# JuliaLinearAlgebra/ArnoldiMethod.jl

Hardware: AMD Instinct MI355X
Metric: arnoldi_iters_per_sec (higher is better)
Workload: dtype f64

## Files before the change

arnoldimethod.jl_amd/_lib.py:

```python
from __future__ import annotations

import ctypes as C
import os

_HERE = os.path.dirname(os.path.abspath(__file__))
LIB_PATH = os.path.join(_HERE, "libkschur_hip.so")

KS_OK, KS_ERR_ARGUMENT, KS_ERR_DIMENSION, KS_ERR_HIP, KS_ERR_RCCL, KS_ERR_QR, KS_ERR_INTERNAL, KS_ERR_NO_DEVICE, KS_ERR_OPERATOR, KS_ERR_COMM = range(10)
KS_F64, KS_C64 = 0, 1
KS_I32, KS_I64 = 0, 1
KS_CSR, KS_CSC = 0, 1
LAYOUTS = {-1: "none", 0: "csr", 1: "csr-vi", 2: "csr-dvi", 3: "sell", 4: "sell-vi", 5: "stencil", 6: "csr-cb"}
PLAN_FACTS = ("ptr64", "ni", "nblk", "nlong", "row_gather", "nslices", "sell_entries", "ncolblocks", "cb_rpt", "cb_ni", "nstencil",
              "nstencil_local", "stencil_mask_bytes", "ndvi", "dvi_unroll")
WHICH = {"LM": 0, "LR": 1, "SR": 2, "LI": 3, "SI": 4}


class ArgumentError(ValueError):
    """Julia's ArgumentError (src/run.jl:111-116,123-124,165-174,185; src/ArnoldiMethod.jl:62-63,87-90)."""


class DimensionMismatch(ValueError):
    """Julia's DimensionMismatch (checksquare, src/run.jl:110)."""


class QRDidNotConverge(RuntimeError):
    """"QR algorithm did not converge" (src/schurfact.jl:406)."""


class HipError(RuntimeError):
    pass


class CommTimeout(HipError):
    """A peer rank did not take part in an exchange within KS_P2P_TIMEOUT_S (peer-to-peer transport)."""


class ks_params(C.Structure):
    _fields_ = [
        ("nev", C.c_int32), ("which", C.c_int32), ("tol", C.c_double), ("mindim", C.c_int32), ("maxdim", C.c_int32),
        ("restarts", C.c_int32), ("start_from", C.c_int32), ("initialize", C.c_int32), ("reserved", C.c_int32),
    ]


class ks_history(C.Structure):
    _fields_ = [
        ("mvproducts", C.c_int32), ("nconverged", C.c_int32), ("converged", C.c_int32), ("nev", C.c_int32),
        ("restarts", C.c_int32), ("reorth", C.c_int32), ("breakdowns", C.c_int32), ("explicit_steps", C.c_int32),
        ("seconds_expand", C.c_double), ("seconds_host", C.c_double), ("seconds_rotate", C.c_double),
    ]


class ks_expand_stats(C.Structure):
    _fields_ = [("steps", C.c_int32), ("reorth", C.c_int32), ("breakdowns", C.c_int32), ("explicit_steps", C.c_int32)]


HOST_APPLY_FN = C.CFUNCTYPE(C.c_int, C.c_void_p, C.c_void_p, C.c_void_p)
DEVICE_APPLY_FN = C.CFUNCTYPE(C.c_int, C.c_void_p, C.c_void_p, C.c_void_p, C.c_void_p)
HOST_ALLREDUCE_FN = C.CFUNCTYPE(C.c_int, C.c_void_p, C.POINTER(C.c_double), C.c_int)
HOST_EXCHANGE_FN = C.CFUNCTYPE(C.c_int, C.c_void_p, C.c_int, C.POINTER(C.c_int32), C.POINTER(C.c_void_p), C.POINTER(C.c_int64),
                               C.POINTER(C.c_void_p), C.POINTER(C.c_int64))

vp, i32, i64, u64, dbl = C.c_void_p, C.c_int, C.c_int64, C.c_uint64, C.c_double
P = C.POINTER
PROTOTYPES = {
    "ks_version": [P(C.c_int), P(C.c_int)],
    "ks_ctx_create": [i32, P(vp)],
    "ks_comm_unique_id": [vp],
    "ks_ctx_create_dist": [i32, i32, i32, vp, P(vp)],
    "ks_ctx_create_hostcomm": [i32, i32, i32, HOST_ALLREDUCE_FN, HOST_EXCHANGE_FN, vp, P(vp)],
    "ks_ctx_create_p2p": [i32, i32, i32, P(vp)],
    "ks_ctx_p2p_handle": [vp, vp],
    "ks_ctx_p2p_attach": [vp, vp],
    "ks_ctx_destroy": [vp],
    "ks_ctx_synchronize": [vp],
    "ks_ctx_rank": [vp, P(C.c_int), P(C.c_int)],
    "ks_ctx_stream": [vp, P(vp)],
    "ks_operator_csr": [vp, i64, i64, i64, vp, vp, vp, i32, i32, i32, i32, P(vp)],
    "ks_operator_csr_dist": [vp, i64, i64, i64, vp, vp, vp, i32, i32, vp, vp, vp, vp, P(vp)],
    "ks_operator_dense": [vp, i64, vp, i64, i32, i32, P(vp)],
    "ks_operator_host_callback": [vp, i64, i32, HOST_APPLY_FN, vp, P(vp)],
    "ks_operator_device_callback": [vp, i64, i32, DEVICE_APPLY_FN, vp, P(vp)],
    "ks_operator_lu": [vp, i64, i32, vp, vp, vp, vp, vp, vp, vp, vp, vp, P(vp)],
    "ks_operator_lu_info": [vp, P(i64), P(i64), P(i64), P(i64)],
    "ks_operator_lu_layout": [vp, i32, P(i64), P(i64), P(i64), P(C.c_int)],
    "ks_operator_destroy": [vp],
    "ks_operator_size": [vp, P(i64), P(i64), P(C.c_int)],
    "ks_operator_format": [vp, P(C.c_double), P(C.c_int), P(C.c_int)],
    "ks_operator_apply_raw": [vp, vp, vp],
    "ks_workspace_create": [vp, i64, i64, i64, i32, i32, P(vp)],
    "ks_workspace_placement": [vp, P(C.c_int), P(C.c_double), P(C.c_double), P(C.c_int)],
    "ks_workspace_passes": [vp, P(C.c_int)],
    "ks_workspace_set_passes": [vp, i32, dbl],
    "ks_workspace_set_sstep": [vp, i32, dbl, dbl],
    "ks_debug_blk_time": [vp, i32, i32, i32, i32, i32, P(C.c_double), P(C.c_int)],
    "ks_workspace_sstep_info": [vp, P(C.c_int), P(C.c_int), P(C.c_int), P(C.c_double)],
    "ks_workspace_relation_info": [vp, P(C.c_int), P(C.c_double)],
    "ks_workspace_relation_probes": [vp, P(C.c_int)],
    "ks_workspace_fused_rotations": [vp, P(C.c_int), P(C.c_int), P(C.c_int)],
    "ks_workspace_split_rotations": [vp, P(C.c_int)],
    "ks_workspace_deflated_blocks": [vp, P(C.c_int), P(C.c_int)],
    "ks_sstep_partition": [C.c_int, C.c_int, C.c_int, C.c_int, P(C.c_int), C.c_int, P(C.c_int)],
    "ks_workspace_assert_arnoldi": [vp, i32],
    "ks_workspace_provenance": [vp, P(C.c_int)],
    "ks_workspace_check_guard": [vp, P(C.c_int)],
    "ks_workspace_destroy": [vp],
    "ks_workspace_dims": [vp, P(i64), P(C.c_int), P(C.c_int), P(i64)],
    "ks_workspace_H": [vp, P(vp), P(C.c_int)],
    "ks_workspace_Q": [vp, P(vp), P(C.c_int)],
    "ks_workspace_col_ptr": [vp, i32, P(vp)],
    "ks_workspace_set_seed": [vp, u64],
    "ks_col_upload": [vp, i32, vp],
    "ks_col_download": [vp, i32, vp],
    "ks_cols_download": [vp, i32, i32, vp, i64],
    "ks_cols_upload": [vp, i32, i32, vp, i64],
    "ks_col_fill_uniform": [vp, i32, u64],
    "ks_col_norm": [vp, i32, P(dbl)],
    "ks_col_div": [vp, i32, dbl],
    "ks_col_copy": [vp, i32, i32],
    "ks_apply": [vp, vp, i32, i32],
    "ks_gemv_t": [vp, i32, i32, vp],
    "ks_gemv_n_sub": [vp, i32, i32, vp],
    "ks_rotate": [vp, i32, i32, i32, vp, i32],
    "ks_basis_times": [vp, i32, i32, vp, i32, i32, vp, i64],
    "ks_orthogonalize": [vp, i32, P(C.c_int)],
    "ks_reinitialize": [vp, i32, vp, P(C.c_int)],
    "ks_iterate_arnoldi": [vp, vp, i32, i32, P(ks_expand_stats)],
    "ks_params_default": [i64, P(ks_params)],
    "ks_partialschur": [vp, vp, P(ks_params), vp, vp, P(ks_history)],
    "ks_restart": [vp, P(ks_params), i32, P(C.c_int), P(C.c_int), P(C.c_int), vp, vp, vp],
    "ks_expand_restart": [vp, vp, P(ks_params), i32, i32, P(C.c_int), P(C.c_int), P(C.c_int), vp, vp, vp, P(ks_expand_stats), vp],
    "ks_profile_enable": [vp, i32],
    "ks_profile_reset": [vp],
    "ks_profile_get": [vp, i32, vp, vp, vp],
    "ks_residual_norms": [vp, vp, i32, P(dbl), P(dbl)],
    "ks_arnoldi_relation": [vp, vp, i32, P(dbl), P(dbl)],
    "ks_host_schurfact": [i32, vp, i32, i32, i32, i32, i32, vp, i32, i32],
    "ks_host_restart_step": [i32, vp, i32, vp, i32, i32, i32, i32, i32, dbl, i32, P(C.c_int), P(C.c_int), P(C.c_int), vp, vp, vp],
    "ks_host_sortschur": [i32, vp, i32, i32, i32, vp, i32, i32, i32, i32],
    "ks_host_givens": [i32, vp, vp, P(dbl), vp, vp],
    "ks_host_csr_plan": [i64, i64, i64, vp, vp, vp, i32, i32, i32, i32, i32, i64, i64, P(C.c_int), P(C.c_int), P(dbl), P(dbl), vp, vp, vp, vp, i64, vp, i32],
    "ks_last_words": [C.c_char_p, i32],
}

_lib = None


def load():
    global _lib
    if _lib is not None:
        return _lib
    if not os.path.exists(LIB_PATH):
        raise ImportError(
            f"{LIB_PATH} is missing: the MI355X HIP library has not been built (run `python __graft_entry__.py build`). "
            "There is no CPU fallback for the product path."
        )
    L = C.CDLL(LIB_PATH)
    L.ks_last_error_string.restype = C.c_char_p
    L.ks_last_error_string.argtypes = []
    for name, args in PROTOTYPES.items():
        fn = getattr(L, name)
        fn.argtypes = args
        fn.restype = C.c_int
    _lib = L
    return L


def check(rc: int):
    if rc == KS_OK:
        return
    msg = load().ks_last_error_string().decode(errors="replace")
    if rc == KS_ERR_ARGUMENT:
        raise ArgumentError(msg)
    if rc == KS_ERR_DIMENSION:
        raise DimensionMismatch(msg)
    if rc == KS_ERR_QR:
        raise QRDidNotConverge(msg)
    if rc == KS_ERR_COMM:
        raise CommTimeout(msg)
    raise HipError(f"libkschur_hip error {rc}: {msg}")
```

arnoldimethod.jl_amd/api.py:

```python
from __future__ import annotations

import ctypes as C
import math
from dataclasses import dataclass

import numpy as np

from . import _lib
from ._lib import ArgumentError, DimensionMismatch, check

EPS = float(np.finfo(np.float64).eps)
DEFAULT_SEED = 20240917


class Target:
    name = "LM"

    def __repr__(self):
        return f"{self.name}()"


class LM(Target):
    name = "LM"

# ... 455 lines not shown
        out = np.empty((self.n, Yf.shape[1]), dtype=ydt, order="F")
        check(_lib.load().ks_basis_times(self._h, c, Yf.shape[1], Yf.ctypes.data, Yf.shape[0], _dtype_code(ydt), out.ctypes.data, self.n))
        return out

    def orthogonalize(self, j: int) -> bool:
        ok = C.c_int()
        check(_lib.load().ks_orthogonalize(self._h, j, C.byref(ok)))
        return bool(ok.value)

    def reinitialize(self, j: int = 0, v1=None) -> bool:
        ok = C.c_int()
        p = None
        if v1 is not None:
            v1 = np.ascontiguousarray(np.asarray(v1, dtype=self.dtype))
            p = v1.ctypes.data
        check(_lib.load().ks_reinitialize(self._h, j, p, C.byref(ok)))
        return bool(ok.value)

    def iterate_arnoldi(self, A: Operator, frm: int, to: int):
        st = _lib.ks_expand_stats()
        _check_op(_lib.load().ks_iterate_arnoldi(A._h, self._h, frm, to, C.byref(st)), A)
        return dict(steps=st.steps, reorth=st.reorth, breakdowns=st.breakdowns, explicit_steps=st.explicit_steps)

    def restart(self, active: int, nev: int, which="LM", tol=None, mindim=None, maxdim=None):
        maxdim = self.maxdim if maxdim is None else maxdim
        mindim = min(max(10, nev), self.n_global) if mindim is None else mindim
        tol = math.sqrt(EPS) if tol is None else tol
        p = _lib.ks_params(nev, _which_code(which), float(tol), mindim, maxdim, 1, 1, 0, 0)
        k, nlock, purge = C.c_int(), C.c_int(), C.c_int()
        lams, rs, groups = np.zeros(2 * maxdim), np.zeros(maxdim), np.zeros(maxdim, dtype=np.int32)
        check(_lib.load().ks_restart(self._h, C.byref(p), active, C.byref(k), C.byref(nlock), C.byref(purge),
                                     lams.ctypes.data, rs.ctypes.data, groups.ctypes.data))
        return dict(k=k.value, nlock=nlock.value, purge=purge.value, eigenvalues=lams[0::2] + 1j * lams[1::2],
                    residuals=rs, groups=groups)

    def expand_restart(self, A: Operator, k: int, active: int, nev: int, which="LM", tol=None, mindim=None, maxdim=None):
        maxdim = self.maxdim if maxdim is None else maxdim
        mindim = min(max(10, nev), self.n_global) if mindim is None else mindim
        tol = math.sqrt(EPS) if tol is None else tol
        p = _lib.ks_params(nev, _which_code(which), float(tol), mindim, maxdim, 1, 1, 0, 0)
        ko, nlock, purge = C.c_int(), C.c_int(), C.c_int()
        lams, rs, groups = np.zeros(2 * maxdim), np.zeros(maxdim), np.zeros(maxdim, dtype=np.int32)
        st = _lib.ks_expand_stats()
        sec = np.zeros(3)
        _check_op(_lib.load().ks_expand_restart(A._h, self._h, C.byref(p), active, k, C.byref(ko), C.byref(nlock), C.byref(purge),
                                                lams.ctypes.data, rs.ctypes.data, groups.ctypes.data, C.byref(st), sec.ctypes.data), A)
        return dict(k=ko.value, nlock=nlock.value, purge=purge.value, eigenvalues=lams[0::2] + 1j * lams[1::2], residuals=rs,
                    groups=groups, steps=st.steps, reorth=st.reorth, breakdowns=st.breakdowns, explicit_steps=st.explicit_steps,
                    seconds=tuple(sec))

    def residual_norms(self, A: Operator, ncols: int):
        r, o = C.c_double(), C.c_double()
        _check_op(_lib.load().ks_residual_norms(A._h, self._h, ncols, C.byref(r), C.byref(o)), A)
        return r.value, o.value

    def arnoldi_relation(self, A: Operator, k: int):
        r, o = C.c_double(), C.c_double()
        _check_op(_lib.load().ks_arnoldi_relation(A._h, self._h, k, C.byref(r), C.byref(o)), A)
        return r.value, o.value

    @property
    def passes(self) -> int:
        k = C.c_int()
        check(_lib.load().ks_workspace_passes(self._h, C.byref(k)))
        return k.value

    def set_passes(self, passes: int, max_ratio: float = float("nan")):
        check(_lib.load().ks_workspace_set_passes(self._h, int(passes), float(max_ratio)))

    def set_sstep(self, s: int, pivot_min: float = float("nan"), gram_dev_max: float = float("nan")):
        check(_lib.load().ks_workspace_set_sstep(self._h, int(s), float(pivot_min), float(gram_dev_max)))

    @property
    def sstep_info(self) -> dict:
        s, b, a = C.c_int(), C.c_int(), C.c_int()
        d = (C.c_double * 3)()
        check(_lib.load().ks_workspace_sstep_info(self._h, C.byref(s), C.byref(b), C.byref(a), d))
        fr, sa, sd = C.c_int(), C.c_int(), C.c_int()
        check(_lib.load().ks_workspace_fused_rotations(self._h, C.byref(fr), C.byref(sa), C.byref(sd)))
        sr = C.c_int()
        check(_lib.load().ks_workspace_split_rotations(self._h, C.byref(sr)))
        db, dc = C.c_int(), C.c_int()
        check(_lib.load().ks_workspace_deflated_blocks(self._h, C.byref(db), C.byref(dc)))
        return dict(s=s.value, blocks=b.value, abandoned=a.value, pivot_stage1=d[0], pivot_stage2=d[1], gram_dev=d[2], fused_rotations=fr.value,
                    split_rotations=sr.value, chains_adopted=sa.value, chains_dropped=sd.value, deflated_blocks=db.value, deflated_columns=dc.value)

    @property
    def relation_info(self) -> dict:
        b, w = C.c_int(), C.c_double()
        check(_lib.load().ks_workspace_relation_info(self._h, C.byref(b), C.byref(w)))
        pr = C.c_int()
        check(_lib.load().ks_workspace_relation_probes(self._h, C.byref(pr)))
        return dict(breaks=b.value, worst_leak=w.value, probes=pr.value)

    def assert_arnoldi(self, k: int):
        check(_lib.load().ks_workspace_assert_arnoldi(self._h, int(k)))

    @property
    def provenance(self) -> int:
        k = C.c_int()
        check(_lib.load().ks_workspace_provenance(self._h, C.byref(k)))
        return k.value

    @property
    def placement(self) -> dict:
        k, b, w, r = C.c_int(), C.c_double(), C.c_double(), C.c_int()
        check(_lib.load().ks_workspace_placement(self._h, C.byref(k), C.byref(b), C.byref(w), C.byref(r)))
        return dict(candidates=k.value, kept_ms=b.value, slowest_ms=w.value, refused=r.value)

    def guard_intact(self) -> bool:
        ok = C.c_int()
        check(_lib.load().ks_workspace_check_guard(self._h, C.byref(ok)))
        return bool(ok.value)

    def close(self):
        if getattr(self, "_h", None) and getattr(self.ctx, "_h", None):
            _lib.load().ks_workspace_destroy(self._h)
        self._h = None

    def __del__(self):
        try:
            self.close()
        except Exception:
            pass


def sstep_partition(dtype, k0: int, count: int, smax: int) -> list:
    if k0 < 1 or count < 1 or smax < 1:
        return []
    cap = 64
    out = (C.c_int * cap)()
    nb = C.c_int(0)
    check(_lib.load().ks_sstep_partition(_dtype_code(dtype), int(k0), int(count), int(smax), out, cap, C.byref(nb)))
    return [int(out[i]) for i in range(min(nb.value, cap))]


class PartialSchur:

    def __init__(self, ws: ArnoldiWorkspace, nconv: int, eigenvalues: np.ndarray):
        self.workspace = ws
        self.nconverged = nconv
        self.R = ws.H[:nconv, :nconv]
        self.eigenvalues = eigenvalues
        self._Q = None

    @property
    def Q(self) -> np.ndarray:
        if self._Q is None:
            self._Q = self.workspace.cols(0, self.nconverged)
        return self._Q

    def __repr__(self):
        return (
            f"PartialSchur decomposition ({'ComplexF64' if self.workspace.dtype.kind == 'c' else 'Float64'}) "
            f"of dimension {self.nconverged}\neigenvalues:\n{self.eigenvalues!r}"
        )


@dataclass
class History:

    mvproducts: int
    nconverged: int
    converged: bool
    nev: int
    restarts: int = 0
    reorth: int = 0
    breakdowns: int = 0
# ... 101 lines not shown
```

arnoldimethod.jl_amd/csrc/ks_backend.hpp:

```cpp
#pragma once
template <class T> struct HipBackend : ks::Backend<T> {
  using D = typename DevT<T>::type;
  ks_operator* op;
  ks_workspace* ws;
  HipBackend(ks_operator* o, ks_workspace* w) : op(o), ws(w) {}

  int64_t n_global() const override { return ws->n_global; }

  void iterate_arnoldi(int from, int to, const ks::Mat<T>& H, ks::ExpandStats& stats) override {
    guarded_expand([&] { iterate_arnoldi_impl(from, to, H, stats, nullptr); });
  }

  bool iterate_arnoldi_early(int from, int to, const ks::Mat<T>& H, ks::ExpandStats& stats, const std::function<void()>& early) override {
    const char* e = std::getenv("KS_EARLY_RESTART");
    const bool on = !(e && e[0] == '0');
    bool done = false;
    guarded_expand([&] { done = iterate_arnoldi_impl(from, to, H, stats, on ? &early : nullptr); });
    return done;
  }

  template <class F> void guarded_expand(F&& f) {
    try {
      f();
    } catch (...) {
      gate_cancel(ws);
      (void)hipStreamSynchronize(ws->ctx->stream);
      try { reset_lazy(ws); } catch (...) {}
      prov_drop(ws);
      ws->rot_pending = ws->rot_fuse = ws->rot_split = false;
      ws->rot_true_start = ws->chain_true = ws->ztrue_valid = false;
      ws->spec_valid = false;
      ws->spec_adopt = 0;
      ws->rp_inflight = false;
      throw;
    }
  }

  bool iterate_arnoldi_impl(int from, int to, const ks::Mat<T>& H, ks::ExpandStats& stats, const std::function<void()>* early) {
    ws->ctx->use();
    bool early_stands = false;
    int j0 = from;
    int explicit_step = -1;
    const bool trusted = prov_ok(ws, from);
    bool no_block = false;
    drift_probe_collect();
    if (trusted && ws->prov_vouched && !ws->t_lazy && ws->sstep_eff >= 2 && op->async_capable && from >= 2 && to - from + 1 >= 2) relation_probe(from, H);
    blk_shifts_from_saved_H();
    while (j0 <= to) {
      const double tb0 = ks::now_s();
      int jend = to;
      if (!op->async_capable) jend = j0;
      if (explicit_step >= 0) jend = j0;
      const bool lazy = use_deferred(ws, jend);
      const bool tpath = lazy && ws->passes == 2 && trusted && explicit_step < 0;
      std::vector<int> blk_sizes;
      ksd::BlkShifts<D> blk_sh{};
      std::vector<std::complex<double>> defl_ex;
      int ndefl = 0;
      if (tpath && !no_block && ws->sstep >= 2 && ws->sstep_eff >= 1 && op->async_capable && jend - j0 + 1 >= 2) {
        ndefl = defl_plan(H, j0, defl_ex, std::min(std::min(ws->sstep, ksd::kBlkSMax), jend - j0 + 1));
        if (ndefl > ws->defl_last && ws->sstep_eff < ws->sstep) { ws->sstep_eff = ws->sstep; ws->blk_clean = 0; }
        ws->defl_last = ndefl;
      }
      if (tpath && !no_block && ws->sstep_eff >= 2 && op->async_capable && jend - j0 + 1 >= 2 &&
          blk_make_shifts<D>(ws, std::min(ws->sstep_eff, ksd::kBlkSMax), blk_sh, ndefl > 0 ? &defl_ex : nullptr))
        blk_sizes = blk_partition(ws->dtype, j0, jend - j0 + 1, std::min(ws->sstep_eff, ksd::kBlkSMax));
      const bool bpath = !blk_sizes.empty();
      if (bpath) {
        int covered = 0;
        for (int sz : blk_sizes) covered += sz;
        jend = std::min(jend, j0 + covered - 1);
      }
      if (ws->rot_pending) {
        const bool fused_ok = bpath && ks_blk_rot_ok(ws->dtype == KS_F64 ? 0 : 1, ws->rot_cin, j0, blk_sizes[0]);
        const bool split_ok = bpath && ws->spec_on && ks_blk_zsrc_ok(ws->dtype == KS_F64 ? 0 : 1, j0, blk_sizes[0]);
        static const int defer_dbg = env_int("KS_DEFER_DEBUG", 0);
        if (defer_dbg)
          std::fprintf(stderr, "[adopt] bpath %d j0 %d out0+rr %d fused_ok %d split_ok %d spec_valid %d blk0 %d spec_ne %d backoff %d\n", (int)bpath, j0, ws->rot_out0 + ws->rot_rr,
                       (int)fused_ok, (int)split_ok, (int)ws->spec_valid, bpath ? blk_sizes[0] : 0, ws->spec_ne, ws->spec_backoff);
        const bool need_true = ws->rot_true_start;
        const bool spec_fits = ws->spec_valid && bpath && blk_sizes[0] >= ws->spec_ne && ws->spec_sh.size() == sizeof(blk_sh) && (!need_true || ws->spec_true);
        if (bpath && ndefl == 0 && j0 == ws->rot_out0 + ws->rot_rr && (fused_ok || split_ok) && ensure_zscratch<D>(ws) &&
            (!need_true || spec_fits || true_start_enqueue<D>(ws))) {
          ws->rot_pending = false;
          ws->rot_true_start = false;
          ws->rot_fuse = true;
          ws->rot_split = !fused_ok;
          ws->chain_true = spec_fits ? ws->spec_true : need_true;
          ws->t_lazy = false;
          ws->t_hi = -1;
          if (spec_fits) {
            std::memcpy(&blk_sh, ws->spec_sh.data(), sizeof(blk_sh));
            ws->spec_adopt = ws->spec_ne;
            ws->spec_used++;
            ws->spec_backoff_len = 1;
            ws->spec_valid = false;
          }
          spec_drop(ws);
        } else {
          rot_flush(ws);
        }
      }
      spec_drop(ws);
      ws->ztrue_valid = false;
      if (tpath && (bpath || ws->blk_tail || !(ws->t_lazy && j0 == ws->t_hi + 1))) {
        materialize(ws);
        ws->ntrue = j0;
      }
      double sigma0 = 1.0;
      if (tpath && ws->t_lazy && j0 - 1 >= ws->ntrue && j0 - 1 <= ws->t_hi) {
        const double binv = reinterpret_cast<const double*>(static_cast<const char*>(ws->Th) + ((size_t)(j0 - 1) + (size_t)(j0 - 1) * ws->ldt) * ws->esz)[0];
        if (binv > 0.0 && std::isfinite(binv)) sigma0 = std::ldexp(1.0, std::ilogb(binv));
      }
      reset_state(ws, tpath, sigma0);
      const bool mb = lazy && ws->use_mbox;
      const bool do_early = early && mb && !tpath && jend == to;
      const uint64_t seq = ++ws->mbox_seq;
      if (bpath) {
        blk_ensure_buffers(ws);
        enqueue_steps_blk<D>(ws, op, j0, blk_sizes, blk_sh, ndefl);
      } else if (tpath) {
        enqueue_steps_t<D>(ws, op, j0, jend);
      } else if (lazy) {
        if (ws->t_lazy) materialize(ws);
        enqueue_steps_deferred<D>(ws, op, j0, jend, do_early ? seq : 0);
      } else {
        materialize(ws);
        for (int j = j0; j <= jend; ++j) {
          op->in_scale = 1.0;
          op->apply(ws->col(j - 1), ws->col(j), ws->st);
          enqueue_orthogonalize<D>(ws, j);
        }
      }
      bool early_ran = false;
      struct EarlyGuard {
        ks_workspace* w; void* Hp; bool armed;
        ~EarlyGuard() { if (armed && !w->Hbackup.empty()) std::memcpy(Hp, w->Hbackup.data(), w->Hbackup.size()); }
      } early_guard{ws, H.p, false};
      static const int dbg = env_int("KS_EARLY_DEBUG", 0);
      double tq0 = dbg ? ks::now_s() : 0.0, tq1 = 0, tq2 = 0;
      if (mb) publish_control(ws, j0, ws->Hstage_dev, 1, seq, tpath);
      else fetch_state_enqueue(ws, j0, tpath);
      if (bpath && jend == to && to == ws->maxdim && j0 >= 2 && !ws->rp_inflight && ++ws->rp_count >= ws->rp_every) {
        ws->rp_count = 0;
        drift_probe_enqueue(j0, H);
      }
      if (bpath && ndefl == 0 && jend == to && to == ws->maxdim &&
          (ks_blk_rot_ok(ws->dtype == KS_F64 ? 0 : 1, ws->maxdim + 1, j0, blk_sizes[0]) || ks_blk_zsrc_ok(ws->dtype == KS_F64 ? 0 : 1, j0, blk_sizes[0]))) {
        static const int defer_dbg2 = env_int("KS_DEFER_DEBUG", 0);
        if (defer_dbg2) std::fprintf(stderr, "[spec] enqueue? backoff %d j0 %d blk0 %d\n", ws->spec_backoff, j0, blk_sizes[0]);
        const bool start_stored = ws->blk_count == 0 || ws->blk_diag[2] <= 1e-12;
        if (ws->spec_backoff > 0) --ws->spec_backoff;
        else spec_enqueue(blk_sh, j0, !start_stored);
      }
      const bool will_defer = ws->rot_defer_on && bpath && ws->sstep_eff >= 8 && to == ws->maxdim;
      if (early && tpath && mb && jend == to && !will_defer) gate_arm(ws);
      if (do_early) {
        mbox_wait(ws, 0, seq);
        if (dbg) tq1 = ks::now_s();
        const DevState* se = reinterpret_cast<const DevState*>(static_cast<const char*>(ws->Hstage_early) + ws->hd_bytes);
        if (se->breakdown < 0) {
          const size_t hb = (size_t)H.ld * H.n * sizeof(T);
          ws->Hbackup.resize(hb);
          std::memcpy(ws->Hbackup.data(), H.p, hb);
          early_guard.armed = true;
          fetch_H_columns<T>(ws, j0, jend, H, false, ws->Hstage_early);
          (*early)();
          early_ran = true;
        }
        if (dbg) tq2 = ks::now_s();
      }
      if (mb) {
        mbox_wait(ws, 1, seq);
        if (ws->ctx->profiling) {
          KS_HIP(hipStreamSynchronize(ws->ctx->stream));
          prof_collect(ws->ctx);
        }
        ws->ctx->check_comm();
      } else {
        fetch_state_wait(ws);
      }
      if (dbg && do_early) {
        const double tq3 = ks::now_s();
        std::fprintf(stderr, "[early] enqueue %.1f us | wait H %.1f us | early host part %.1f us | final wait %.1f us | batch %.1f us\n", 1e6 * (tq0 - tb0), 1e6 * (tq1 - tq0), 1e6 * (tq2 - tq1), 1e6 * (tq3 - tq2), 1e6 * (tq3 - tb0));
      } else if (dbg) {
        const double tq3 = ks::now_s();
        std::fprintf(stderr, "[early off] enqueue %.1f us | wait %.1f us | batch %.1f us\n", 1e6 * (tq0 - tb0), 1e6 * (tq3 - tq0), 1e6 * (tq3 - tb0));
      }
      if (ws->gate_armed && (ws->st_h->breakdown >= 0 || ws->st_h->bail >= 0 || ws->st_h->blk_bail >= 0))
        gate_cancel(ws);
      const int blk_bail = bpath ? ws->st_h->blk_bail : -1;
      const int bail = (tpath && !bpath) ? ws->st_h->bail : -1;
      const int bd = (bail >= 0 || blk_bail >= 0) ? -1 : ws->st_h->breakdown;
      const int last_done = blk_bail >= 0 ? blk_bail - 1 : (bail >= 0 ? bail - 1 : (bd >= 0 ? bd : jend));
      if (bpath) {
        ws->blk_diag[0] = ws->st_h->blk_piv1;
        ws->blk_diag[1] = ws->st_h->blk_piv2;
        ws->blk_diag[2] = ws->st_h->blk_gdev;
        int done = 0, done_blocks = 0;
        for (int sz : blk_sizes) { if (j0 + done + sz - 1 <= last_done) { done += sz; ws->blk_count++; ++done_blocks; } }
        if (blk_bail >= 0) {
          ws->blk_bails++; stats.blk_bails++; no_block = true;
          ws->sstep_eff = ws->sstep_eff >= 4 ? ws->sstep_eff / 2 : (ws->sstep_eff > 2 ? 2 : 1);
          ws->blk_clean = 0;
        } else if (++ws->blk_clean >= 16 && ws->sstep_eff < ws->sstep) {
          int nxt = ws->sstep_eff + 1;
          for (int cand : {2, 3, 4, 5, 8, 10, 20}) if (cand > ws->sstep_eff) { nxt = cand; break; }
          ws->sstep_eff = std::min(ws->sstep, std::max(2, nxt));
          ws->blk_clean = 0;
        }
        stats.blocks += done_blocks;
      } else if (tpath && ws->sstep_eff == 1 && ws->sstep >= 2 && blk_bail < 0 && bail < 0 && bd < 0) {
        if (++ws->blk_clean >= 16) { ws->sstep_eff = 2; ws->blk_clean = 0; }
      }
      if (early_ran && bd >= 0) {
        std::memcpy(H.p, ws->Hbackup.data(), ws->Hbackup.size());
        early_ran = false;
      }
      early_guard.armed = false;
      if (early_ran) {
        const T* hs = static_cast<const T*>(ws->Hstage);
        H(jend, jend - 1) = hs[(size_t)(jend - 1) * (ws->maxdim + 1) + jend];
        lazy_factors_from_stage<T>(ws, j0, jend, ws->Hstage);
        early_stands = true;
      } else {
        fetch_H_columns<T>(ws, j0, last_done, H, lazy && !tpath);
      }
      if (tpath) {
        const int good = blk_bail >= 0 ? blk_bail - 1 : (bail >= 0 ? bail - 1 : (bd >= 0 ? bd - 1 : jend));
        if (good >= ws->ntrue) {
          ws->t_lazy = true;
          ws->t_hi = good;
          ws->blk_tail = bpath;
        }
      }
      stats.steps += last_done - j0 + 1;
      stats.reorth += ws->st_h->n_reorth;
      if (explicit_step >= 0) explicit_step = -1;
      if (bail >= 0) {
        explicit_step = bail;
        stats.explicit_steps++;
      }
      if (lazy && jend > j0) ws->oop_full = 10 * ws->st_h->n_reorth >= 9 * (last_done - j0 + 1);
      if (bd >= 0) {
        if ((int64_t)bd != ws->n_global) {
          reinit_column<D>(ws, bd, nullptr);
          stats.breakdowns++;
        }
      }
      j0 = last_done + 1;
    }
    if (trusted) prov_set(ws, to);
    else prov_drop(ws);
    if (ws->sstep_eff >= 2 && to == ws->maxdim && !early_stands) {
      ws->Hfull.assign(static_cast<const char*>(ws->H), static_cast<const char*>(ws->H) + h_bytes(ws));
      ws->hfull_valid = true;
      ws->ritz_valid = false;
    }
    return early_stands;
  }

  int defl_plan(const ks::Mat<T>& H, int j0, std::vector<std::complex<double>>& ex, int steps) {
    ex.clear();
    static const int dbg = env_int("KS_DEFLATE_DEBUG", 0);
    if (dbg) std::fprintf(stderr, "[deflate] j0 %d on %d dist %d ritz_valid %d nritz %d sstep_eff %d steps %d\n", j0, (int)ws->defl_on, (int)ws->ctx->distributed(), (int)ws->ritz_valid, (int)ws->ritz.size(), ws->sstep_eff, steps);
    if (!ws->defl_on || !ws->ritz_valid || ws->ritz.empty()) return 0;
    static const double ratio = [] { const char* e = std::getenv("KS_DEFLATE_RATIO"); const double v = e ? std::atof(e) : 1.5; return v > 1.0 ? v : 1.5; }();
    int nl = 0;
    for (int j = 1; j <= j0 - 2; ++j)
      if (H(j, j - 1) == T(0)) nl = j;
    if (nl == 0) return 0;
    using C = std::complex<double>;
    std::vector<C> lam(nl);
    std::vector<int> width(nl, 1);
    for (int j = 0; j < nl;) {
      if (j + 1 < nl && H(j + 1, j) != T(0)) {
        const C a = C(H(j, j)), b = C(H(j, j + 1)), c = C(H(j + 1, j)), d = C(H(j + 1, j + 1));
        const C tr2 = 0.5 * (a + d), disc = std::sqrt(tr2 * tr2 - (a * d - b * c));
        lam[j] = tr2 + disc; lam[j + 1] = tr2 - disc;
        width[j] = 2; width[j + 1] = 0;
        j += 2;
      } else {
        lam[j] = C(H(j, j));
        ++j;
      }
    }
    double rest = 0.0;
    for (auto z : ws->ritz) {
      if (!std::isfinite(std::abs(z))) continue;
      bool locked = false;
      for (int j = 0; j < nl; ++j) locked = locked || std::abs(z - lam[j]) <= 1e-6 * std::max(1.0, std::abs(lam[j]));
      if (!locked) rest = std::max(rest, std::abs(z));
    }
    if (dbg) std::fprintf(stderr, "[deflate] locked columns %d, largest other Ritz value %.3g, |lambda_0| %.3g\n", nl, rest, std::abs(lam[0]));
    if (!(rest > 0.0)) return 0;
    int nd = 0;
    for (int j = 0; j < nl;) {
      const int w = width[j] == 2 ? 2 : 1;
      const double mag = w == 2 ? std::max(std::abs(lam[j]), std::abs(lam[j + 1])) : std::abs(lam[j]);
      const double growth = std::pow(mag / rest, std::max(1, steps - 1));
      if (!(mag > ratio * rest) || !(growth > 1e3) || nd + w > ksd::kDeflMax) break;
      for (int q = 0; q < w; ++q) ex.push_back(lam[j + q]);
      nd += w;
      j += w;
    }
    return nd;
  }

  void spec_enqueue(const ksd::BlkShifts<D>& sh, int k_now, bool from_true) {
    if (!ws->spec_on || !ws->rot_defer_on || !ws->gate_allowed || ws->sstep_eff < 8 || !op->async_capable || ws->ctx->hc.allreduce != nullptr) return;
    if (from_true && (!ws->true_start_on || ws->maxdim + 1 > 40)) return;
    const int ne = std::min(10, ws->maxdim - k_now - (sizeof(D) == 8 ? 1 : 0));
    if (ne < 2) return;
    if (!ensure_zscratch<D>(ws)) return;
    if (from_true && !true_start_enqueue<D>(ws)) return;
    char* zs = static_cast<char*>(ws->zscratch);
    op->shift_store_cacheable = true;
    for (int i = 0; i < ne; ++i) {
      op->in_scale = 1.0;
      const void* src = i == 0 ? (from_true ? static_cast<const void*>(ws->ztrue) : ws->col(ws->maxdim)) : static_cast<const void*>(zs + (size_t)(i - 1) * ws->ld * sizeof(D));
      double tre, tim;
      if constexpr (sizeof(D) == 8) { tre = sh.theta[i]; tim = 0.0; }
      else { tre = sh.theta[i].x; tim = sh.theta[i].y; }
      op->apply_shifted(src, zs + (size_t)i * ws->ld * sizeof(D), tre, tim, sh.sigma[i], ws->ld, ws->st);
    }
    ws->spec_sh.assign(reinterpret_cast<const char*>(&sh), reinterpret_cast<const char*>(&sh) + sizeof(sh));
    ws->spec_ne = ne;
    ws->spec_true = from_true;
    ws->spec_valid = true;
  }

  void relation_probe(int from, const ks::Mat<T>& H) {
    const int c = from - 2, nc = from;
    hipStream_t s_ = ws->ctx->stream;
    D* scratch = static_cast<D*>(ws->col(from));
    op->in_scale = 1.0;
    op->apply(ws->col(c), ws->col(from), nullptr);
    if (!ws->probe_dev) {
      KS_HIP(hipMalloc(&ws->probe_dev, 16 + (size_t)(ws->maxdim + 2) * 16));
      KS_HIP(hipHostMalloc(&ws->probe_host, 16 + (size_t)(ws->maxdim + 2) * 16, hipHostMallocCoherent | hipHostMallocMapped));
    }
    double* out = static_cast<double*>(ws->probe_dev);
    D* coef_d = reinterpret_cast<D*>(static_cast<char*>(ws->probe_dev) + 16);
    D* coef_h = reinterpret_cast<D*>(static_cast<char*>(ws->probe_host) + 16);
    double fro2 = 0.0;
    for (int j = 0; j < from - 1; ++j)
      for (int i = 0; i < from; ++i) fro2 += std::norm(std::complex<double>(H(i, j)));
    for (int i = 0; i < nc; ++i) std::memcpy(&coef_h[i], &H(i, c), sizeof(D));
    KS_HIP(hipMemcpyAsync(coef_d, coef_h, (size_t)nc * sizeof(D), hipMemcpyHostToDevice, s_));
    KS_HIP(hipMemsetAsync(out, 0, 2 * sizeof(double), s_));
    const int64_t nchunks = (ws->n + 15) / 16;
    const int64_t stride = std::max<int64_t>(1, std::min<int64_t>(64, nchunks / 16384));
    const int64_t sampled = (nchunks + stride - 1) / stride * 16;
    const int grid = (int)((sampled + kBlock - 1) / kBlock);
    ksd::k_relation_probe<D><<<grid, kBlock, 0, s_>>>(static_cast<const D*>(ws->V), ws->ld, nc, scratch, coef_d, ws->n, stride, out);
    KS_HIP(hipGetLastError());
    if (ws->ctx->distributed()) ws->ctx->allreduce(out, 2);
    double* res = static_cast<double*>(ws->probe_host);
    KS_HIP(hipMemcpyAsync(res, out, 2 * sizeof(double), hipMemcpyDeviceToHost, s_));
    KS_HIP(hipStreamSynchronize(s_));
    ws->ctx->check_comm();
    ws->relation_probes++;
    const double fro = std::sqrt(fro2);
    const double leak = res[1] > 0.0 ? std::sqrt(res[0] * ((double)ws->n_global / res[1])) : 0.0;
    if (!(leak <= 10.0 * ws->relation_tol * fro)) {
      ws->relation_breaks++;
      ws->relation_leak = std::max(ws->relation_leak, fro > 0.0 ? leak / fro : leak);
      ws->sstep_eff = 0;
    }
  }

  void drift_probe_enqueue(int from, const ks::Mat<T>& H) {
    const int c = from - 2, nc = from;
    hipStream_t s_ = ws->ctx->stream;
    if (!ws->probe_dev) {
      KS_HIP(hipMalloc(&ws->probe_dev, 16 + (size_t)(ws->maxdim + 2) * 16));
      KS_HIP(hipHostMalloc(&ws->probe_host, 16 + (size_t)(ws->maxdim + 2) * 16, hipHostMallocCoherent | hipHostMallocMapped));
    }
    if (!ws->probe_col) {
      if (hipMalloc(&ws->probe_col, (size_t)ws->ld * sizeof(D)) != hipSuccess) {
        (void)hipGetLastError();
        ws->probe_col = nullptr;
        return;
      }
      KS_HIP(hipMemsetAsync(ws->probe_col, 0, (size_t)ws->ld * sizeof(D), s_));
    }
    D* scratch = static_cast<D*>(ws->probe_col);
    op->in_scale = 1.0;
    op->apply(ws->col(c), scratch, ws->st);
    if (!ws->ctx->distributed()) {
      if (!ws->watch_acc) {
        KS_HIP(hipMalloc(&ws->watch_acc, 32));
        KS_HIP(hipMemsetAsync(ws->watch_acc, 0, 32, s_));
        KS_HIP(hipHostGetDevicePointer(&ws->probe_host_dev, ws->probe_host, 0));
      }
      ksd::ProbeCoef<D> pc;
      double fro2w = 0.0;
      for (int j = 0; j < from - 1; ++j)
        for (int i = 0; i < from; ++i) fro2w += std::norm(std::complex<double>(H(i, j)));
// ... 328 lines not shown
```

arnoldimethod.jl_amd/csrc/ks_block.hpp:

```cpp
#pragma once



inline bool blk_shape_ok(int dtype, int k, int s) { return ks_blk_shape_ok(dtype == KS_F64 ? 0 : 1, k, s); }
inline std::vector<int> blk_partition(int dtype, int k0, int count, int smax) {
  std::vector<int> out;
  int k = k0;
  while (count > 0) {
    int s = std::min(count, smax);
    while (s > 1 && !blk_shape_ok(dtype, k, s)) --s;
    if (!blk_shape_ok(dtype, k, s)) break;
    out.push_back(s);
    k += s;
    count -= s;
  }
  return out;
}

inline std::vector<std::complex<double>> leja_shifts(const std::vector<std::complex<double>>& ritz, int s, bool real) {
  std::vector<std::complex<double>> pts;
  for (auto z : ritz) {
    if (real) z = std::complex<double>(z.real(), 0.0);
    if (!std::isfinite(z.real()) || !std::isfinite(z.imag())) continue;
    bool dup = false;
    for (auto& q : pts) dup = dup || std::abs(q - z) <= 1e-14 * std::max(1.0, std::abs(z));
    if (!dup) pts.push_back(z);
  }
  std::vector<std::complex<double>> out;
  if (pts.empty()) { out.assign(s, 0.0); return out; }
  std::vector<double> logprod(pts.size(), 0.0);
  std::vector<bool> used(pts.size(), false);
  size_t cur = 0;
  for (size_t i = 1; i < pts.size(); ++i) if (std::abs(pts[i]) > std::abs(pts[cur])) cur = i;
  while (out.size() < pts.size() && (int)out.size() < s) {
    used[cur] = true;
    out.push_back(pts[cur]);
    size_t best = pts.size();
    for (size_t i = 0; i < pts.size(); ++i) {
      if (used[i]) continue;
      logprod[i] += std::log(std::max(std::abs(pts[i] - pts[cur]), 1e-300));
      if (best == pts.size() || logprod[i] > logprod[best]) best = i;
    }
    if (best == pts.size()) break;
    cur = best;
  }
  const size_t have = out.size();
  while ((int)out.size() < s) out.push_back(out[out.size() % have]);
  return out;
}

inline void blk_ensure_buffers(ks_workspace* ws) {
  if (ws->bpart) return;
  const size_t entries = (size_t)ksd::kBlkKMax * ksd::kBlkSMax + ksd::kBlkGram;
  KS_HIP(hipMalloc(&ws->bpart, entries * (size_t)ws->pnb * ws->esz));
  KS_HIP(hipMalloc(&ws->bred, entries * ws->esz));
  const size_t sb = ws->dtype == KS_F64 ? sizeof(ksd::BlkScratch<double>) : sizeof(ksd::BlkScratch<cd>);
  KS_HIP(hipMalloc(&ws->bscr, sb));
  KS_HIP(hipMemset(ws->bscr, 0, sb));
  KS_HIP(hipMalloc(&ws->bzero, 256));
  KS_HIP(hipMemset(ws->bzero, 0, 256));
}

inline int& blk_dbg() { static int v = env_int("KS_BLK_DBG", 0); return v; }
template <class D> int launch_blk(ks_workspace* ws, int which, int k, int s, bool zscratch = false) {
  auto* bs = static_cast<ksd::BlkScratch<D>*>(ws->bscr);
  BlkLaunchArgs a{};
  a.V = ws->V; a.ld = ws->ld; a.dtype = sizeof(D) == 8 ? 0 : 1; a.k = k; a.s = s;
  if (zscratch) { a.zsrc = ws->zscratch; a.ldz = ws->ld; }
  if (which == 2) { a.cin = ws->rot_cin; a.out0 = ws->rot_out0; a.rotm = ws->Qd; }
  a.partial = ws->bpart; a.pnb = ws->pnb; a.coefp = bs->coefp; a.r1inv = bs->r1inv; a.zeros = ws->bzero; a.st = ws->st;
  a.dbg = blk_dbg(); a.nt = ws->v_nt ? 1 : 0; a.num_cu = ws->ctx->num_cu; a.bpc = ws->ctx->bpc; a.stream = ws->ctx->stream;
  try {
    return ks_blk_launch(which, a);
  } catch (const std::runtime_error& e) {
    throw KsError{KS_ERR_INTERNAL, e.what()};
  }
}

template <class D> bool ensure_zscratch(ks_workspace* ws) {
  if (ws->zscratch) return true;
  const size_t zbytes = (size_t)ws->ld * ksd::blk_smax<D>() * sizeof(D);
  if (hipMalloc(&ws->zscratch, zbytes) != hipSuccess) {
    (void)hipGetLastError();
    ws->zscratch = nullptr;
    ws->spec_on = false;
    ws->rot_defer_on = false;
    return false;
  }
  KS_HIP(hipMemsetAsync(ws->zscratch, 0, zbytes, ws->ctx->stream));
  if (env_int("KS_ADDR_DEBUG", 0)) std::fprintf(stderr, "[addr] V %p zscratch %p ld %lld bytes/col %lld\n", ws->V, ws->zscratch, (long long)ws->ld, (long long)(ws->ld * sizeof(D)));
  return true;
}

template <class D> bool true_start_enqueue(ks_workspace* ws) {
  if (ws->ztrue_valid) return true;
  const int cin = ws->maxdim + 1;
  if (cin > 40) return false;
  if (!ws->ztrue) {
    if (hipMalloc(&ws->ztrue, (size_t)ws->ld * sizeof(D)) != hipSuccess) { (void)hipGetLastError(); ws->ztrue = nullptr; return false; }
    KS_HIP(hipMemsetAsync(ws->ztrue, 0, (size_t)ws->ld * sizeof(D), ws->ctx->stream));
  }
  ks_ctx* cx = ws->ctx;
  ProfScope ps(cx, KSP_ROTATE, (double)ws->n * sizeof(D) * (cin + 1));
  const D* Vc = static_cast<const D*>(ws->col(0));
  const D* tcol = static_cast<const D*>(ws->Td) + (size_t)ws->maxdim * ws->ldt;
  D* out = static_cast<D*>(ws->ztrue);
  const size_t smem = (size_t)cin * sizeof(D);
  const int nb = cap_blocks(ws, cx->num_cu * 4, kBlock);
  if (cin <= 8) ksd::k_rotate_valu<D, 8><<<nb, kBlock, smem, cx->stream>>>(Vc, ws->ld, cin, 1, tcol, ws->ldt, out, ws->ld, -1);
  else if (cin <= 16) ksd::k_rotate_valu<D, 16><<<nb, kBlock, smem, cx->stream>>>(Vc, ws->ld, cin, 1, tcol, ws->ldt, out, ws->ld, -1);
  else if (cin <= 24) ksd::k_rotate_valu<D, 24><<<nb, kBlock, smem, cx->stream>>>(Vc, ws->ld, cin, 1, tcol, ws->ldt, out, ws->ld, -1);
  else ksd::k_rotate_valu<D, 40><<<nb, kBlock, smem, cx->stream>>>(Vc, ws->ld, cin, 1, tcol, ws->ldt, out, ws->ld, -1);
  KS_HIP(hipGetLastError());
  ws->ztrue_valid = true;
  ws->true_starts++;
  return true;
}

template <class D>
void enqueue_steps_blk(ks_workspace* ws, ks_operator* op, int from, const std::vector<int>& sizes, const ksd::BlkShifts<D>& sh, int ndefl = 0) {
  ks_ctx* cx = ws->ctx;
  hipStream_t s_ = cx->stream;
  const int ldh = ws->maxdim + 1;
  const double nb8 = (double)ws->n * sizeof(D);
  D* Hd = static_cast<D*>(ws->Hd);
  D* Tm = static_cast<D*>(ws->Td);
  auto* bs = static_cast<ksd::BlkScratch<D>*>(ws->bscr);
  int k = from;
  int first = 1;
  for (int s : sizes) {
    const bool fuse = first && ws->rot_fuse;
    const bool split = fuse && ws->rot_split;
    const bool chain_true = fuse && ws->chain_true;
    ws->rot_fuse = false;
    ws->rot_split = false;
    ws->chain_true = false;
    char* zs = nullptr;
    if (fuse) {
      KS_REQUIRE(ws->zscratch != nullptr, KS_ERR_INTERNAL, "fused rotation without scratch columns (the adoption allocates them)");
      zs = static_cast<char*>(ws->zscratch);
    }
    if (split) {
      rotate_device<D>(ws, 0, ws->rot_cin, ws->rot_rr, ws->rot_out0, -1);
      ws->rot_split_count++;
    }
    auto zcol = [&](int i) -> void* { return fuse ? static_cast<void*>(zs + (size_t)i * ws->ld * sizeof(D)) : ws->col(k + i); };
    op->shift_store_cacheable = s >= 10;
    const int adopted = fuse ? ws->spec_adopt : 0;
    ws->spec_adopt = 0;
    for (int i = adopted; i < s; ++i) {
      double tre, tim;
      if constexpr (sizeof(D) == 8) { tre = sh.theta[i]; tim = 0.0; }
      else { tre = sh.theta[i].x; tim = sh.theta[i].y; }
      op->in_scale = 1.0;
      const void* src = i == 0 ? (fuse ? (chain_true ? static_cast<const void*>(ws->ztrue) : ws->col(ws->maxdim)) : ws->col(k - 1)) : zcol(i - 1);
      op->apply_shifted(src, zcol(i), tre, tim, sh.sigma[i], ws->ld, ws->st);
      if (ndefl > 0) {
        ProfScope ps(cx, KSP_AXPY, nb8 * 2.0 * (ndefl + 1) + nb8);
        if (!ws->defl_part) KS_HIP(hipMalloc(&ws->defl_part, (size_t)ksd::kDeflMax * (1024 + 1) * sizeof(D)));
        const int nbd = (int)std::max<int64_t>(1, std::min<int64_t>(std::min(1024, cx->num_cu * 4), (ws->n + kBlock - 1) / kBlock));
        D* zc = static_cast<D*>(zcol(i));
        const D* U = static_cast<const D*>(ws->col(0));
        D* part = static_cast<D*>(ws->defl_part);
        ksd::k_defl_dots<D><<<nbd, kBlock, 0, s_>>>(U, ws->ld, ndefl, zc, ws->n, part);
        if (!cx->distributed()) {
          ksd::k_defl_apply<D><<<nbd, kBlock, 0, s_>>>(U, ws->ld, ndefl, zc, ws->n, part, nbd, bs->cdefl + (size_t)i * ksd::kDeflMax);
        } else {
          D* red = part + (size_t)ksd::kDeflMax * 1024;
          ksd::k_defl_reduce<D><<<1, kBlock, 0, s_>>>(part, nbd, ndefl, red);
          cx->allreduce(reinterpret_cast<double*>(red), ndefl * (int)(sizeof(D) / 8));
          ksd::k_defl_apply<D><<<nbd, kBlock, 0, s_>>>(U, ws->ld, ndefl, zc, ws->n, red, 1, bs->cdefl + (size_t)i * ksd::kDeflMax);
        }
      }
    }
    if (ndefl > 0) ws->defl_blocks++;
    const int ne = k * s + s * (s + 1) / 2;
    int nb1, nb2;
    auto fin = [&](int stage, int nbp) {
      ProfScope ps(cx, KSP_FIN, 0.0);
      const D* part = static_cast<const D*>(ws->bpart);
      D* red = static_cast<D*>(ws->bred);
      if (!cx->distributed()) {
        ksd::k_fin_blk<D><<<(ne + 3) / 4, kBlock, 0, s_>>>(stage, 0, part, nbp, ws->pnb, k, s, red, Hd, ldh, Tm, ws->ldt, ws->ntrue, bs, sh, first, ws->blk_pivmin,
                                                 ws->blk_gdevmax, ws->st, ws->ctr, ndefl);
      } else {
        ksd::k_fin_blk<D><<<(ne + 3) / 4, kBlock, 0, s_>>>(stage, 1, part, nbp, ws->pnb, k, s, red, Hd, ldh, Tm, ws->ldt, ws->ntrue, bs, sh, first, ws->blk_pivmin,
                                                 ws->blk_gdevmax, ws->st, ws->ctr, ndefl);
        cx->allreduce(reinterpret_cast<double*>(red), ne * (int)(sizeof(D) / 8));
        ksd::k_fin_blk<D><<<1, kBlock, 0, s_>>>(stage, 2, part, nbp, ws->pnb, k, s, red, Hd, ldh, Tm, ws->ldt, ws->ntrue, bs, sh, first, ws->blk_pivmin,
                                                ws->blk_gdevmax, ws->st, ws->ctr, ndefl);
      }
    };
    if (fuse && !split) {
      ProfScope ps(cx, KSP_ROTATE, nb8 * (ws->rot_cin + s + ws->rot_rr));
      nb1 = launch_blk<D>(ws, 2, k, s, true);
      ws->rot_fused_count++;
    } else {
      ProfScope ps(cx, KSP_DOTS, nb8 * (k + s));
      nb1 = launch_blk<D>(ws, 0, k, s, fuse);
    }
    fin(1, nb1);
    {
      ProfScope ps(cx, KSP_FUSED, nb8 * (k + 2 * s));
      nb2 = launch_blk<D>(ws, 1, k, s, fuse);
    }
    fin(2, nb2);
    k += s;
    first = 0;
  }
  KS_HIP(hipGetLastError());
}

template <class D> bool blk_make_shifts(ks_workspace* ws, int smax, ksd::BlkShifts<D>& sh, const std::vector<std::complex<double>>* excluded = nullptr) {
  if (!ws->ritz_valid || ws->ritz.empty()) return false;
  const bool real = sizeof(D) == 8;
  std::vector<std::complex<double>> pool;
  if (excluded && !excluded->empty()) {
    for (auto z : ws->ritz) {
      bool ex = false;
      for (auto q : *excluded) ex = ex || std::abs(z - q) <= 1e-6 * std::max(1.0, std::abs(q));
      if (!ex) pool.push_back(z);
    }
  }
  const std::vector<std::complex<double>>& src = pool.empty() ? ws->ritz : pool;
  const auto th = leja_shifts(src, smax, real);
  double rho = 0.0;
  for (auto z : src)
    if (std::isfinite(std::abs(z))) rho = std::max(rho, std::abs(z));
  if (!(rho > 0.0) || !std::isfinite(rho)) return false;
  const double sigma = std::ldexp(1.0, -(int)std::lround(std::log2(rho)));
  for (int i = 0; i < ksd::kBlkSMax; ++i) {
    const auto z = th[i < (int)th.size() ? i : 0];
    if constexpr (sizeof(D) == 8) sh.theta[i] = z.real();
    else sh.theta[i] = cd{z.real(), z.imag()};
    sh.sigma[i] = sigma;
  }
  return true;
}
```

arnoldimethod.jl_amd/csrc/ks_block_inst.hip:

```cpp
#include <hip/hip_runtime.h>

#include <algorithm>
#include <cstdlib>
#include <stdexcept>
#include <string>

#include "ks_block_kernels.hpp"
#include "ks_block_mfma.hpp"
#include "ks_block_launch.hpp"

#ifndef KS_BLK_PART
#error "compile with -DKS_BLK_PART=0|1|2"
#endif

namespace {
using ksd::cd;
using ksd::kBlock;

inline void hipcheck(hipError_t e, const char* what) {
  if (e != hipSuccess) throw std::runtime_error(std::string("HIP error in ") + what + ": " + hipGetErrorString(e));
}
template <class K> int resident(const BlkLaunchArgs& a, K kernel, int& cache, int threads = kBlock) {
  if (cache < 0) {
    int occ = 0;
// ... 17 lines not shown
  if (stages < 2) throw std::runtime_error("block kernels: ring does not fit the LDS");
  const size_t smem = (size_t)stages * ncol * 1024;
  auto kern = ksd::k_bdots_ring<NCW, S, NW, WB>;
  static bool attr = false;
  if (!attr) {
    hipcheck(hipFuncSetAttribute(reinterpret_cast<const void*>(kern), hipFuncAttributeMaxDynamicSharedMemorySize, 160 * 1024), "dynamic LDS size");
    attr = true;
  }
  const int nb = cap(a, a.num_cu, 64, sizeof(double));
  kern<<<nb, 64 * NW, smem, a.stream>>>(static_cast<const double*>(a.V), a.ld, a.k, stages, static_cast<double*>(a.partial), a.pnb,
                                        static_cast<const ksd::DevState*>(a.st), a.dbg | (a.nt ? 64 : 0), static_cast<const double*>(a.zeros));
  return nb;
}

template <int NCW, int S, int NW, int WB> int go_ring1(const BlkLaunchArgs& a) {
  constexpr int WA = NW / WB, SP = ((S + WB - 1) / WB) * WB;
  const int ncol = a.k + S;
  const size_t fixed = (size_t)(WA * S + S) * 1024 + (size_t)(WA * NCW * SP + S * SP) * 8;
  int stages = (int)std::min<size_t>(3, (158 * 1024 - fixed) / ((size_t)ncol * 1024));
  static const int st_env = [] { const char* e = std::getenv("KS_BLK_RING_STAGES"); return e ? std::atoi(e) : 0; }();
  if (st_env >= 2) stages = (int)std::min<size_t>(st_env, (158 * 1024 - fixed) / ((size_t)ncol * 1024));
  if (stages < 2) throw std::runtime_error("block kernels: ring does not fit the LDS");
  const size_t smem = (size_t)stages * ncol * 1024 + fixed;
  auto kern = ksd::k_bupdate_ring<NCW, S, NW, WB>;
  static bool attr = false;
  if (!attr) {
    hipcheck(hipFuncSetAttribute(reinterpret_cast<const void*>(kern), hipFuncAttributeMaxDynamicSharedMemorySize, 160 * 1024), "dynamic LDS size");
    attr = true;
  }
  const int nb = cap(a, a.num_cu, 64, sizeof(double));
  kern<<<nb, 64 * NW, smem, a.stream>>>(static_cast<double*>(a.V), a.ld, a.k, stages, static_cast<const double*>(a.coefp), a.k,
                                        static_cast<const double*>(a.r1inv), static_cast<double*>(a.partial), a.pnb,
                                        static_cast<const ksd::DevState*>(a.st), a.dbg | (a.nt ? 64 : 0), static_cast<const double*>(a.zeros));
  return nb;
}

template <int NCW4> int go_ringL0(const BlkLaunchArgs& a) {
  const int ncol = a.k + ksd::kBlkL;
  const int stages = std::min(3, (150 * 1024) / (ncol * 1024));
  if (stages < 2) throw std::runtime_error("block kernels: ring does not fit the LDS");
  const size_t smem = (size_t)stages * ncol * 1024;
  auto kern = ksd::k_bdots_ringL<NCW4>;
  static bool attr = false;
  if (!attr) {
    hipcheck(hipFuncSetAttribute(reinterpret_cast<const void*>(kern), hipFuncAttributeMaxDynamicSharedMemorySize, 160 * 1024), "dynamic LDS size");
    attr = true;
  }
  const int nb = cap(a, a.num_cu, 64, sizeof(double));
  kern<<<nb, 512, smem, a.stream>>>(static_cast<const double*>(a.V), a.ld, a.k, stages, static_cast<double*>(a.partial), a.pnb,
                                   static_cast<const ksd::DevState*>(a.st), a.dbg | (a.nt ? 64 : 0), static_cast<const double*>(a.zeros));
  return nb;
}
template <int NCW2> int go_ringL1(const BlkLaunchArgs& a) {
  constexpr int S = ksd::kBlkL;
  const int ncol = a.k + S;
  const size_t fixed = (size_t)(2 * S + S) * 1024 + (size_t)(2 * NCW2 * S + S * S) * 8;
  const int stages = 2;
  const size_t smem = (size_t)stages * ncol * 1024 + fixed;
  if (smem > 160 * 1024) throw std::runtime_error("block kernels: ring does not fit the LDS");
  auto kern = ksd::k_bupdate_ringL<NCW2>;
  static bool attr = false;
  if (!attr) {
    hipcheck(hipFuncSetAttribute(reinterpret_cast<const void*>(kern), hipFuncAttributeMaxDynamicSharedMemorySize, 160 * 1024), "dynamic LDS size");
    attr = true;
  }
  const int nb = cap(a, a.num_cu, 64, sizeof(double));
  kern<<<nb, 512, smem, a.stream>>>(static_cast<double*>(a.V), a.ld, a.k, stages, static_cast<const double*>(a.coefp), a.k,
                                   static_cast<const double*>(a.r1inv), static_cast<double*>(a.partial), a.pnb,
                                   static_cast<const ksd::DevState*>(a.st), a.dbg | (a.nt ? 64 : 0), static_cast<const double*>(a.zeros));
  return nb;
}


inline int mfma_env() { static const int v = [] { const char* e = std::getenv("KS_BLK_MFMA"); return e ? std::atoi(e) : 255; }(); return v; }
inline int mfma_ring_env() { static const int v = [] { const char* e = std::getenv("KS_BLK_MFMA_RING"); return e ? std::atoi(e) : 3; }(); return v; }
template <int NGS, int NT, bool CX = false> int go_mfma(int which, const BlkLaunchArgs& a) {
  using C = ksd::BlkMfma<NGS, NT>;
  int ring = mfma_ring_env();
  while (ring > 2 && C::lds_bytes(ring, CX) > 160 * 1024) --ring;
  const size_t smem = C::lds_bytes(ring, CX);
  if (ring < 2 || smem > 160 * 1024) throw std::runtime_error("block kernels: slab ring does not fit the LDS");
  constexpr int RV = CX ? 2 : 1;
  const int nb = cap(a, a.num_cu, 64, CX ? 16 : 8);
  const int dbg = a.dbg | (a.nt ? 64 : 0);
  double* Vr = static_cast<double*>(a.V);
  const int64_t ldr = a.ld * RV;
  if (which == 0) {
    auto kern = ksd::k_bdots_mfma<NGS, NT, CX>;
    static bool attr = false;
    if (!attr) {
      hipcheck(hipFuncSetAttribute(reinterpret_cast<const void*>(kern), hipFuncAttributeMaxDynamicSharedMemorySize, 160 * 1024), "dynamic LDS size");
      attr = true;
    }
    const double* zb = a.zsrc ? static_cast<const double*>(a.zsrc) : Vr + (int64_t)a.k * ldr;
    kern<<<nb, 512, smem, a.stream>>>(Vr, ldr, a.k, zb, a.zsrc ? a.ldz * RV : ldr, a.s, ring, static_cast<double*>(a.partial), a.pnb,
                                     static_cast<const ksd::DevState*>(a.st), dbg, static_cast<const double*>(a.zeros));
  } else {
    auto kern = ksd::k_bupdate_mfma<NGS, NT, CX>;
    static bool attr = false;
    if (!attr) {
      hipcheck(hipFuncSetAttribute(reinterpret_cast<const void*>(kern), hipFuncAttributeMaxDynamicSharedMemorySize, 160 * 1024), "dynamic LDS size");
      attr = true;
    }
    const double* zb = a.zsrc ? static_cast<const double*>(a.zsrc) : Vr + (int64_t)a.k * ldr;
    kern<<<nb, 512, smem, a.stream>>>(Vr, ldr, a.k, zb, a.zsrc ? a.ldz * RV : ldr, a.s, ring, static_cast<const double*>(a.coefp), a.k,
                                     static_cast<const double*>(a.r1inv), static_cast<double*>(a.partial), a.pnb,
                                     static_cast<const ksd::DevState*>(a.st), dbg, static_cast<const double*>(a.zeros));
  }
  return nb;
}
template <int NT, int MAXG, int G = 1, bool CX = false> int go_mfma_by_k(int which, const BlkLaunchArgs& a) {
  if constexpr (G > MAXG) {
    throw std::runtime_error("block kernels: no matrix-instruction form for this many columns");
  } else {
    if ((a.k + 3) / 4 == G) return go_mfma<G, NT, CX>(which, a);
    return go_mfma_by_k<NT, MAXG, G + 1, CX>(which, a);
  }
}

#if KS_BLK_PART >= 1
template <int NGX, int NTK, int NT, bool CX> int go_rot(const BlkLaunchArgs& a) {
  using C = ksd::BlkRot<NGX, NTK, NT>;
  int ring = mfma_ring_env();
  while (ring > 2 && C::lds_bytes(ring, CX) > 160 * 1024) --ring;
  const size_t smem = C::lds_bytes(ring, CX);
  if (ring < 2 || smem > 160 * 1024) throw std::runtime_error("block kernels: slab ring of the fused rotation does not fit the LDS");
  constexpr int RV = CX ? 2 : 1;
  const int nb = cap(a, a.num_cu, 64, CX ? 16 : 8);
  auto kern = ksd::k_brotdots_mfma<NGX, NTK, NT, CX>;
  static bool attr = false;
  if (!attr) {
    hipcheck(hipFuncSetAttribute(reinterpret_cast<const void*>(kern), hipFuncAttributeMaxDynamicSharedMemorySize, 160 * 1024), "dynamic LDS size");
    attr = true;
  }
  kern<<<nb, 512, smem, a.stream>>>(static_cast<double*>(a.V), a.ld * RV, a.cin, static_cast<const double*>(a.rotm), a.out0, a.k,
                                   static_cast<const double*>(a.zsrc), a.ldz * RV, a.s, ring, static_cast<double*>(a.partial), a.pnb,
                                   a.dbg | (a.nt ? 64 : 0), static_cast<const double*>(a.zeros));
  return nb;
}
#if KS_BLK_PART == 1
#define KS_ROT_SHAPES(X) X(11, 6, 5) X(11, 7, 4) X(11, 7, 3) X(11, 8, 3) X(11, 8, 2) X(6, 3, 3) X(6, 4, 3) X(6, 4, 2)
constexpr bool kRotCX = false;
#else
#define KS_ROT_SHAPES(X) X(6, 3, 3) X(6, 4, 3) X(6, 4, 2) X(11, 6, 3)
constexpr bool kRotCX = true;
#endif
inline bool rot_shape(int cin, int k, int s, int& ngx, int& ntk, int& nt) {
  ngx = (cin + 3) / 4; ntk = (k + 3) / 4;
  const int need = (s + 3) / 4;
  nt = 0;
#define KS_ROT_HAS(A, B, C_) if (ngx == A && ntk == B && need <= C_ && (nt == 0 || C_ < nt)) nt = C_;
  KS_ROT_SHAPES(KS_ROT_HAS)
#undef KS_ROT_HAS
  return nt != 0;
}
inline int go_rot_by_shape(const BlkLaunchArgs& a) {
  int ngx, ntk, nt;
  if (!a.zsrc || !a.rotm || !rot_shape(a.cin, a.k, a.s, ngx, ntk, nt)) throw std::runtime_error("block kernels: no fused rotation for this shape");
#define KS_ROT_GO(A, B, C_) if (ngx == A && ntk == B && nt == C_) return go_rot<A, B, C_, kRotCX>(a);
  KS_ROT_SHAPES(KS_ROT_GO)
#undef KS_ROT_GO
  throw std::runtime_error("block kernels: no fused rotation for this shape");
}
#endif

template <class D, int NCW, int S, int NW = 4, int WB = 1> int go(int which, const BlkLaunchArgs& a) {
  if constexpr (sizeof(D) == 8 && S == 20) {
    if ((mfma_env() >> which) & 1) return go_mfma_by_k<5, 6>(which, a);
  }
  if constexpr (sizeof(D) == 8 && S == 10) {
    if ((mfma_env() >> (which + 2)) & 1) return go_mfma_by_k<3, 8>(which, a);
  }
  if constexpr (sizeof(D) == 8 && S == 8) {
    if ((mfma_env() >> (which + 4)) & 1) return go_mfma_by_k<2, 12>(which, a);
  }
  if constexpr (sizeof(D) == 8 && NW == 8 && S == 20) {
    if (which == 0 && (ring_env() & 1)) return go_ringL0<NCW>(a);
    if (which == 1 && (ring_env() & 2)) {
      if (a.k <= 20) return go_ringL1<10>(a);
      if (a.k <= 22) return go_ringL1<11>(a);
      return go_ringL1<12>(a);
    }
  }
  if constexpr (sizeof(D) == 8 && NW == 8 && S <= 10) {
    if (which == 0 && (ring_env() & 1)) return go_ring0<NCW, S, NW, WB>(a);
    if (which == 1 && (ring_env() & 2)) return go_ring1<NCW, S, NW, WB>(a);
  }
  constexpr int U = ksd::blk_u<D, NCW, S, NW>();
  constexpr int NT_ = 64 * NW;
  const ksd::DevState* st = static_cast<const ksd::DevState*>(a.st);
  D* V = static_cast<D*>(a.V);
  D* part = static_cast<D*>(a.partial);
  if (which == 0) {
    static int cache = -1;
    const int nb = cap(a, resident(a, ksd::k_bdots<D, NCW, S, U, true, NW, WB>, cache, NT_), 64 * U, sizeof(D));
    if (a.nt) ksd::k_bdots<D, NCW, S, U, true, NW, WB><<<nb, NT_, 0, a.stream>>>(V, a.ld, a.k, part, a.pnb, st);
    else ksd::k_bdots<D, NCW, S, U, false, NW, WB><<<nb, NT_, 0, a.stream>>>(V, a.ld, a.k, part, a.pnb, st);
    return nb;
  }
  static int cache = -1;
  const int nb = cap(a, resident(a, ksd::k_bupdate<D, NCW, S, U, true, NW, WB>, cache, NT_), 64 * U, sizeof(D));
  const D* cp = static_cast<const D*>(a.coefp);
  const D* ri = static_cast<const D*>(a.r1inv);
  if (a.nt) ksd::k_bupdate<D, NCW, S, U, true, NW, WB><<<nb, NT_, 0, a.stream>>>(V, a.ld, a.k, cp, a.k, ri, part, a.pnb, st, a.dbg);
  else ksd::k_bupdate<D, NCW, S, U, false, NW, WB><<<nb, NT_, 0, a.stream>>>(V, a.ld, a.k, cp, a.k, ri, part, a.pnb, st, a.dbg);
  return nb;
}

template <class D, int S> int by_ncw(int which, const BlkLaunchArgs& a) {
  const int need = (a.k + 3) / 4;
  if constexpr (sizeof(D) == 8 && S == 20) {
    if (need <= 6) return go<D, 6, S, 8, 2>(which, a);
  } else if constexpr (sizeof(D) == 8 && S == 10) {
    if (need <= 4) return go<D, 4, S, 8, 2>(which, a);
    if (need <= 5) return go<D, 5, S, 8, 2>(which, a);
    if (need <= 6) return go<D, 6, S, 8, 2>(which, a);
    if (need <= 7) return go<D, 7, S, 8, 2>(which, a);
    if (need <= 8) return go<D, 8, S, 8, 2>(which, a);
  } else if constexpr (sizeof(D) == 8) {
    if (need <= 4) return go<D, 4, S>(which, a);
    if (need <= 5) return go<D, 5, S>(which, a);
    if (need <= 6) return go<D, 6, S>(which, a);
    if (need <= 7) return go<D, 7, S>(which, a);
    if (need <= 8) return go<D, 8, S>(which, a);
    if (need <= 9) return go<D, 9, S>(which, a);
    if (need <= 10) return go<D, 10, S>(which, a);
    if (need <= 12) return go<D, 12, S>(which, a);
    if constexpr (S <= 5) return go<D, 16, S>(which, a);
  } else {
    if (need <= 4) return go<D, 4, S>(which, a);
    if (need <= 6) return go<D, 6, S>(which, a);
    if (need <= 8) return go<D, 8, S>(which, a);
  }
  throw std::runtime_error("block kernels: no instantiation for this many columns");
}
}

#if KS_BLK_PART == 0
int ks_blk_launch_part0(int which, const BlkLaunchArgs& a) {
  switch (a.s) {
    case 1: return by_ncw<double, 1>(which, a);
    case 2: return by_ncw<double, 2>(which, a);
    case 3: return by_ncw<double, 3>(which, a);
    case 4: return by_ncw<double, 4>(which, a);
    default: throw std::runtime_error("block kernels: block size not in this part");
  }
}
#elif KS_BLK_PART == 1
int ks_blk_mfma_nt_f64(int k, int s) {
  const int m = mfma_env();
  if (s < 1 || k < 1) return 0;
  if (s <= 8) return (k <= 64 && ((m >> 4) & 3) == 3) ? 2 : 0;
  if (s <= 12) return (k <= 48 && ((m >> 2) & 3) == 3) ? 3 : 0;
  if (s <= 16 && k <= 28 && k > 24) return (m & 3) == 3 ? 4 : 0;
  return (s <= 20 && k <= 24 && (m & 3) == 3) ? 5 : 0;
}
static bool pass2_mfma(int k, int s) {
  const int bit2 = s == 20 ? 1 : (s == 10 ? 3 : (s == 8 ? 5 : -1));
  if (bit2 >= 0 && (s == 20 ? k <= 24 : (s == 10 ? k <= 32 : k <= 48))) return ((mfma_env() >> bit2) & 1) != 0;
  return s > 5 && ks_blk_mfma_nt_f64(k, s) > 0;
}
bool ks_blk_rot_ok_f64(int cin, int k, int s) {
  int a, b, c;
  if (!pass2_mfma(k, s) || !((mfma_env() >> 6) & 1)) return false;
  return k >= 1 && cin >= k && rot_shape(cin, k, s, a, b, c);
}
int ks_blk_launch_part1(int which, const BlkLaunchArgs& a) {
  if (which == 2) return go_rot_by_shape(a);
  const bool wide = (a.s == 8 && a.k > 48) || (a.s == 10 && a.k > 32);
  switch (wide ? 0 : a.s) {
    case 5: return by_ncw<double, 5>(which, a);
    case 8: return by_ncw<double, 8>(which, a);
    case 10: return by_ncw<double, 10>(which, a);
    case 20: return by_ncw<double, 20>(which, a);
    default:
      switch (ks_blk_mfma_nt_f64(a.k, a.s)) {
        case 2: return go_mfma_by_k<2, 16>(which, a);
        case 3: return go_mfma_by_k<3, 12>(which, a);
        case 4: return go_mfma_by_k<4, 7, 7>(which, a);
        case 5: return go_mfma_by_k<5, 6>(which, a);
        default: throw std::runtime_error("block kernels: block size not in this part");
      }
  }
}
#else
int ks_blk_mfma_nt_c64(int k, int s) {
  if (!((mfma_env() >> 7) & 1) || k < 1 || k > 48 || s < 1) return 0;
  if (s <= 8) return 2;
  return (s <= 10 && k <= 32) ? 3 : 0;
}
bool ks_blk_rot_ok_c64(int cin, int k, int s) {
  int a, b, c;
  if (!(s > 5 && ks_blk_mfma_nt_c64(k, s) > 0) || !((mfma_env() >> 6) & 1)) return false;
  return k >= 1 && cin >= k && rot_shape(cin, k, s, a, b, c);
}
int ks_blk_launch_part2(int which, const BlkLaunchArgs& a) {
  if (which == 2) return go_rot_by_shape(a);
  if (a.s > 5 || a.k > 32) {
    const int nt = ks_blk_mfma_nt_c64(a.k, a.s);
    if (nt == 2) return go_mfma_by_k<2, 12, 1, true>(which, a);
    if (nt == 3) return go_mfma_by_k<3, 8, 1, true>(which, a);
  }
  switch (a.s) {
    case 1: return by_ncw<cd, 1>(which, a);
    case 2: return by_ncw<cd, 2>(which, a);
    case 3: return by_ncw<cd, 3>(which, a);
    case 4: return by_ncw<cd, 4>(which, a);
    case 5: return by_ncw<cd, 5>(which, a);
    default: throw std::runtime_error("block kernels: block size not instantiated for ComplexF64");
  }
}
#endif
```

arnoldimethod.jl_amd/csrc/ks_block_launch.hpp:

```cpp
#pragma once

#include <hip/hip_runtime.h>
#include <stdint.h>

struct BlkLaunchArgs {
  void* V;
  int64_t ld;
  int dtype;
  int k, s;
  void* partial;
  int pnb;
  const void* coefp;
  const void* r1inv;
  const void* zeros;
  const void* st;
  int dbg;
  int nt;
  int num_cu, bpc;
  hipStream_t stream;
  const void* zsrc = nullptr;
  int64_t ldz = 0;
  int cin = 0, out0 = 0;
  const void* rotm = nullptr;
};
int ks_blk_launch_part0(int which, const BlkLaunchArgs& a);
int ks_blk_launch_part1(int which, const BlkLaunchArgs& a);
int ks_blk_launch_part2(int which, const BlkLaunchArgs& a);
int ks_blk_mfma_nt_f64(int k, int s);
int ks_blk_mfma_nt_c64(int k, int s);
inline int ks_blk_mfma_nt(int dtype, int k, int s) { return dtype == 0 ? ks_blk_mfma_nt_f64(k, s) : ks_blk_mfma_nt_c64(k, s); }
inline bool ks_blk_zsrc_ok(int dtype, int k, int s) { return s > 5 && ks_blk_mfma_nt(dtype, k, s) > 0; }
bool ks_blk_rot_ok_f64(int cin, int k, int s);
bool ks_blk_rot_ok_c64(int cin, int k, int s);
inline bool ks_blk_rot_ok(int dtype, int cin, int k, int s) { return dtype == 0 ? ks_blk_rot_ok_f64(cin, k, s) : ks_blk_rot_ok_c64(cin, k, s); }
inline int ks_blk_launch(int which, const BlkLaunchArgs& a) {
  if (a.dtype != 0) return ks_blk_launch_part2(which, a);
  return a.s <= 4 ? ks_blk_launch_part0(which, a) : ks_blk_launch_part1(which, a);
}
inline bool ks_blk_shape_ok(int dtype, int k, int s) {
  if (k < 1 || s < 1 || k + s > 65) return false;
  if (dtype != 0) return (s <= 5 && k <= 32) || ks_blk_mfma_nt_c64(k, s) > 0;
  if (s <= 5) return true;
  if ((s == 8 && k <= 48) || (s == 10 && k <= 32) || (s == 20 && k <= 24)) return true;
  return ks_blk_mfma_nt_f64(k, s) > 0;
}
```

arnoldimethod.jl_amd/csrc/ks_block_mfma.hpp:

```cpp
#pragma once

#include "ks_block_kernels.hpp"

namespace ksd {

__device__ __forceinline__ double mfma4(double a, double b, double c) { return __builtin_amdgcn_mfma_f64_4x4x4f64(a, b, c, 0, 0, 0); }
__device__ __forceinline__ void wait_vm(int n) {
#define KS_VMW(N) case N: asm volatile("s_waitcnt vmcnt(" #N ") lgkmcnt(0)" ::: "memory"); break;
  switch (n) {
    KS_VMW(0) KS_VMW(1) KS_VMW(2) KS_VMW(3) KS_VMW(4) KS_VMW(5) KS_VMW(6) KS_VMW(7) KS_VMW(8) KS_VMW(9) KS_VMW(10) KS_VMW(11)
    KS_VMW(12) KS_VMW(13) KS_VMW(14) KS_VMW(15) KS_VMW(16) KS_VMW(17) KS_VMW(18) KS_VMW(19) KS_VMW(20) KS_VMW(21) KS_VMW(22)
    KS_VMW(23) KS_VMW(24) KS_VMW(25) KS_VMW(26) KS_VMW(27) KS_VMW(28) KS_VMW(29) KS_VMW(30) KS_VMW(31) KS_VMW(32) KS_VMW(33)
    KS_VMW(34) KS_VMW(35) KS_VMW(36) KS_VMW(37) KS_VMW(38) KS_VMW(39) KS_VMW(40)
    default: asm volatile("s_waitcnt vmcnt(0) lgkmcnt(0)" ::: "memory"); break;
  }
#undef KS_VMW
}
__device__ __forceinline__ void gst8_nt(double* p, double v) { asm volatile("global_store_dwordx2 %0, %1, off nt" :: "v"(p), "v"(v) : "memory"); }

template <int NGS, int NT> struct BlkMfma {
  static constexpr int NJS = (NGS + 1) / 2, NJZ = (NT + 1) / 2, NJ = NJS + NJZ;
  static constexpr int SLAB = NJ * 1024;
  static constexpr int NTS = NGS * NT, NTG = NT * (NT + 1) / 2, NTILE = NTS + NTG;
  static constexpr int MBYTES = NTILE * 128;
  __host__ __device__ static constexpr int s_off(int g) { return (g / 2) * 1024 + (g % 2) * 512; }
  __host__ __device__ static constexpr int z_off(int t) { return NJS * 1024 + (t / 2) * 1024 + (t % 2) * 512; }
  __host__ __device__ static constexpr int gt(int a, int t) { return t * (t + 1) / 2 + a; }
  static constexpr size_t lds_bytes(int ring, bool cx = false) { return (size_t)8 * ring * SLAB + (cx ? 2 : 1) * (size_t)MBYTES; }
};

template <int NGS, int NT, bool CX = false>
__device__ __forceinline__ void blkm_finish(double* acc, unsigned char* lds, int lane, int wave, int k, int s, double* __restrict__ partial, int pnb) {
  using C = BlkMfma<NGS, NT>;
  constexpr int NA = CX ? 2 * C::NTILE : C::NTILE;
  double* red = reinterpret_cast<double*>(lds);
  __syncthreads();
#pragma unroll
  for (int e = 0; e < NA; ++e) {
    double v = acc[e];
    v += __shfl_xor(v, 4, 64);
    v += __shfl_xor(v, 8, 64);
    if ((lane & 12) == 0) red[(wave * NA + e) * 16 + (lane >> 4) * 4 + (lane & 3)] = v;
  }
  __syncthreads();
  for (int e = threadIdx.x; e < NA * 16; e += 512) {
    double v = 0.0;
#pragma unroll
    for (int w = 0; w < 8; ++w) v += red[w * NA * 16 + e];
    const int part = (e >> 4) / C::NTILE;
    const int tile = (e >> 4) % C::NTILE, ii = (e >> 2) & 3, jj = e & 3;
    int entry = -1;
    if (tile < C::NTS) {
      const int g = tile / NT, t = tile % NT, c = 4 * g + ii, i = 4 * t + jj;
      if (c < k && i < s) entry = i * k + c;
    } else {
      int t = 0, rem = tile - C::NTS;
      while (rem > t) { rem -= t + 1; ++t; }
      const int a = rem, i = 4 * a + ii, i2 = 4 * t + jj;
      if (i <= i2 && i2 < s) entry = k * s + gram_idx(i, i2);
    }
    if (entry >= 0) partial[((int64_t)entry * pnb + blockIdx.x) * (CX ? 2 : 1) + part] = v;
  }
}


template <int NGS, int NT>
__device__ __forceinline__ void blkm_issue(const double* __restrict__ V, int64_t ldv, int k, const double* __restrict__ Zb, int64_t ldz, int s,
                                           int64_t pack0, int64_t pe, int lane, uint32_t slab_lds, const double* __restrict__ zeros, bool nt) {
  using C = BlkMfma<NGS, NT>;
  const int64_t p = pack0 + (lane & 7);
  const bool in = p < pe;
  const int cl = lane >> 3;
#pragma unroll
  for (int j = 0; j < C::NJ; ++j) {
    const int c = j < C::NJS ? 8 * j + cl : 8 * (j - C::NJS) + cl;
    const bool have = in && (j < C::NJS ? c < k : c < s);
    const double* src = have ? (j < C::NJS ? V + (int64_t)c * ldv : Zb + (int64_t)c * ldz) + p * 2 : zeros;
    if (nt) glds16_nt(src, slab_lds + (uint32_t)j * 1024u);
    else glds16(src, slab_lds + (uint32_t)j * 1024u);
  }
}

template <int NGS, int NT, bool CX = false>
__global__ void __launch_bounds__(512, 2)
    k_bdots_mfma(const double* __restrict__ V, int64_t ldv, int k, const double* __restrict__ Zb, int64_t ldz, int s, int ring,
                 double* __restrict__ partial, int pnb, const DevState* __restrict__ st, int dbg, const double* __restrict__ zeros) {
  if (st && st->breakdown >= 0) return;
  using C = BlkMfma<NGS, NT>;
  extern __shared__ __attribute__((aligned(16))) unsigned char lds_raw[];
  const int lane = threadIdx.x & 63;
  const int wave = __builtin_amdgcn_readfirstlane(threadIdx.x >> 6);
  unsigned char* myring = lds_raw + (size_t)wave * ring * C::SLAB;
  const uint32_t ring_lds = (uint32_t)(uintptr_t)myring;
  const int gat = (lane & 3) * 128 + (4 * ((lane >> 2) & 3) + (lane >> 4)) * 8;
  const double psign = ((lane >> 4) & 1) ? -1.0 : 1.0;
  constexpr int NA = CX ? 2 * C::NTILE : C::NTILE;
  double acc[NA];
#pragma unroll
  for (int e = 0; e < NA; ++e) acc[e] = 0.0;
  int64_t pb, pe;
  block_range(ldv / 2, blockIdx.x, gridDim.x, pb, pe);
  const int niter = (int)((pe - pb + 63) / 64);
  const bool nt = (dbg & 64) != 0;
  auto issue = [&](int it, int sl) {
    if (dbg & 32) return;
    blkm_issue<NGS, NT>(V, ldv, k, Zb, ldz, s, pb + (int64_t)it * 64 + wave * 8, pe, lane, ring_lds + (uint32_t)(sl * C::SLAB), zeros, nt);
  };
  for (int it = 0; it < ring - 1; ++it) issue(it, it);
  int sl_cur = 0, sl_new = ring - 1;
  for (int it = 0; it < niter; ++it) {
    wait_vm((ring - 2) * C::NJ);
    issue(it + ring - 1, sl_new);
    const unsigned char* slab = myring + (size_t)sl_cur * C::SLAB;
    sl_new = sl_cur;
    sl_cur = sl_cur + 1 == ring ? 0 : sl_cur + 1;
    if (dbg & 16) continue;
    double a[NGS], z[NT], zp[CX ? NT : 1];
#pragma unroll
    for (int t = 0; t < NT; ++t) z[t] = *reinterpret_cast<const double*>(slab + C::z_off(t) + gat);
    if constexpr (CX) {
#pragma unroll
      for (int t = 0; t < NT; ++t) zp[t] = psign * *reinterpret_cast<const double*>(slab + C::z_off(t) + (gat ^ 8));
    }
#pragma unroll
    for (int g = 0; g < NGS; ++g) a[g] = *reinterpret_cast<const double*>(slab + C::s_off(g) + gat);
#pragma unroll
    for (int t = 0; t < NT; ++t)
#pragma unroll
      for (int q = 0; q <= t; ++q) {
        acc[C::NTS + C::gt(q, t)] = mfma4(z[q], z[t], acc[C::NTS + C::gt(q, t)]);
        if constexpr (CX) acc[C::NTILE + C::NTS + C::gt(q, t)] = mfma4(z[q], zp[t], acc[C::NTILE + C::NTS + C::gt(q, t)]);
      }
#pragma unroll
    for (int g = 0; g < NGS; ++g)
#pragma unroll
      for (int t = 0; t < NT; ++t) {
        acc[g * NT + t] = mfma4(a[g], z[t], acc[g * NT + t]);
        if constexpr (CX) acc[C::NTILE + g * NT + t] = mfma4(a[g], zp[t], acc[C::NTILE + g * NT + t]);
      }
  }
  asm volatile("s_waitcnt vmcnt(0)" ::: "memory");
  blkm_finish<NGS, NT, CX>(acc, lds_raw, lane, wave, k, s, partial, pnb);
}

template <int NGS, int NT, bool CX = false>
__global__ void __launch_bounds__(512, 2)
    k_bupdate_mfma(double* __restrict__ V, int64_t ldv, int k, const double* __restrict__ Zb, int64_t ldz, int s, int ring,
                   const double* __restrict__ coefp, int ldc, const double* __restrict__ r1inv, double* __restrict__ partial, int pnb,
                   const DevState* __restrict__ st, int dbg, const double* __restrict__ zeros) {
  if (st && st->breakdown >= 0) return;
  using C = BlkMfma<NGS, NT>;
  extern __shared__ __attribute__((aligned(16))) unsigned char lds_raw[];
  const int lane = threadIdx.x & 63;
  const int wave = __builtin_amdgcn_readfirstlane(threadIdx.x >> 6);
  unsigned char* myring = lds_raw + (size_t)wave * ring * C::SLAB;
  const uint32_t ring_lds = (uint32_t)(uintptr_t)myring;
  constexpr int CD = CX ? 2 : 1;
  double* mt = reinterpret_cast<double*>(lds_raw + (size_t)8 * ring * C::SLAB);
  for (int e = threadIdx.x; e < CD * C::NTILE * 16; e += 512) {
    const int part = (e >> 4) / C::NTILE;
    const int tile = (e >> 4) % C::NTILE, kk = (e >> 2) & 3, jj = e & 3;
    double v = 0.0;
    if (tile < C::NTS) {
      const int g = tile / NT, t = tile % NT, c = 4 * g + kk, i = 4 * t + jj;
      if (c < k && i < s) v = -coefp[(c + (int64_t)i * ldc) * CD + part];
    } else {
      int t = 0, rem = tile - C::NTS;
      while (rem > t) { rem -= t + 1; ++t; }
      const int l = 4 * rem + kk, i = 4 * t + jj;
      if (l <= i && i < s) v = r1inv[(l + i * s) * CD + part];
    }
    mt[e] = v;
  }
  __syncthreads();
  const int lin = lane * 8;
  const int gat = (lane & 3) * 128 + (4 * ((lane >> 2) & 3) + (lane >> 4)) * 8;
  const double jsign = (lane & 1) ? 1.0 : -1.0;
  const double psign = ((lane >> 4) & 1) ? -1.0 : 1.0;
  const double* mrd = mt + (lane >> 4) * 4 + (lane & 3);
  const double* mri = mrd + C::NTILE * 16;
  constexpr int NA = CX ? 2 * C::NTILE : C::NTILE;
  double acc[NA];
#pragma unroll
  for (int e = 0; e < NA; ++e) acc[e] = 0.0;
  int64_t pb, pe;
  block_range(ldv / 2, blockIdx.x, gridDim.x, pb, pe);
  const int niter = (int)((pe - pb + 63) / 64);
  const bool nt = (dbg & 64) != 0;
  const int nst = (dbg & 1) ? 0 : (s + 3) / 4;
  auto issue = [&](int it, int sl) {
    blkm_issue<NGS, NT>(V, ldv, k, Zb, ldz, s, pb + (int64_t)it * 64 + wave * 8, pe, lane, ring_lds + (uint32_t)(sl * C::SLAB), zeros, nt);
  };
  const int row = 4 * ((lane >> 2) & 3) + (lane >> 4), cj = lane & 3;
  double* zst = V + (int64_t)(k + cj) * ldv + row;
  for (int it = 0; it < ring - 1; ++it) issue(it, it);
  int sl_cur = 0, sl_new = ring - 1;
  for (int it = 0; it < niter; ++it) {
    wait_vm((ring - 2) * C::NJ + (it < ring - 1 ? it : ring - 1) * nst);
    issue(it + ring - 1, sl_new);
    const unsigned char* slab = myring + (size_t)sl_cur * C::SLAB;
    sl_new = sl_cur;
    sl_cur = sl_cur + 1 == ring ? 0 : sl_cur + 1;
    const int64_t pack0 = pb + (int64_t)it * 64 + wave * 8;
    double x[NGS], zx[NT], d[NT];
#pragma unroll
    for (int g = 0; g < NGS; ++g) x[g] = *reinterpret_cast<const double*>(slab + C::s_off(g) + lin);
#pragma unroll
    for (int u = 0; u < NT; ++u) zx[u] = *reinterpret_cast<const double*>(slab + C::z_off(u) + lin);
#pragma unroll
    for (int t = 0; t < NT; ++t) d[t] = 0.0;
#pragma unroll
    for (int g = 0; g < NGS; ++g)
#pragma unroll
      for (int t = 0; t < NT; ++t) d[t] = mfma4(x[g], mrd[(g * NT + t) * 16], d[t]);
#pragma unroll
    for (int u = 0; u < NT; ++u)
#pragma unroll
      for (int t = u; t < NT; ++t) d[t] = mfma4(zx[u], mrd[(C::NTS + C::gt(u, t)) * 16], d[t]);
    if constexpr (CX) {
#pragma unroll
      for (int g = 0; g < NGS; ++g) {
        const double xj = jsign * *reinterpret_cast<const double*>(slab + C::s_off(g) + (lin ^ 8));
#pragma unroll
        for (int t = 0; t < NT; ++t) d[t] = mfma4(xj, mri[(g * NT + t) * 16], d[t]);
      }
#pragma unroll
      for (int u = 0; u < NT; ++u) {
        const double zj = jsign * *reinterpret_cast<const double*>(slab + C::z_off(u) + (lin ^ 8));
#pragma unroll
        for (int t = u; t < NT; ++t) d[t] = mfma4(zj, mri[(C::NTS + C::gt(u, t)) * 16], d[t]);
      }
    }
    if (nst) {
      const bool ok = pack0 + (row >> 1) < pe;
      double* dst = zst + pack0 * 2;
#pragma unroll
      for (int t = 0; t < NT; ++t) {
        if (4 * t < s) {
          if (ok && 4 * t + cj < s) gst8_nt(dst + (int64_t)(4 * t) * ldv, d[t]);
        }
      }
    }
    double a[NGS], dp[CX ? NT : 1];
#pragma unroll
    for (int g = 0; g < NGS; ++g) a[g] = *reinterpret_cast<const double*>(slab + C::s_off(g) + gat);
    if constexpr (CX) {
#pragma unroll
      for (int t = 0; t < NT; ++t) dp[t] = psign * __shfl_xor(d[t], 16, 64);
    }
#pragma unroll
    for (int t = 0; t < NT; ++t)
#pragma unroll
      for (int q = 0; q <= t; ++q) {
        acc[C::NTS + C::gt(q, t)] = mfma4(d[q], d[t], acc[C::NTS + C::gt(q, t)]);
        if constexpr (CX) acc[C::NTILE + C::NTS + C::gt(q, t)] = mfma4(d[q], dp[t], acc[C::NTILE + C::NTS + C::gt(q, t)]);
      }
#pragma unroll
    for (int g = 0; g < NGS; ++g)
#pragma unroll
      for (int t = 0; t < NT; ++t) {
        acc[g * NT + t] = mfma4(a[g], d[t], acc[g * NT + t]);
        if constexpr (CX) acc[C::NTILE + g * NT + t] = mfma4(a[g], dp[t], acc[C::NTILE + g * NT + t]);
      }
  }
  asm volatile("s_waitcnt vmcnt(0)" ::: "memory");
  blkm_finish<NGS, NT, CX>(acc, lds_raw, lane, wave, k, s, partial, pnb);
}


template <int NGX, int NTK, int NT> struct BlkRot {
  static constexpr int NJX = (NGX + 1) / 2, NJZ = (NT + 1) / 2, NJ = NJX + NJZ;
  static constexpr int SLAB = NJ * 1024;
  static constexpr int NTM = NGX * NTK;
  static constexpr int NTS = NTK * NT, NTG = NT * (NT + 1) / 2, NTILE = NTS + NTG;
  __host__ __device__ static constexpr int x_off(int g) { return (g / 2) * 1024 + (g % 2) * 512; }
  __host__ __device__ static constexpr int z_off(int t) { return NJX * 1024 + (t / 2) * 1024 + (t % 2) * 512; }
  __host__ __device__ static constexpr int gt(int a, int t) { return t * (t + 1) / 2 + a; }
  static constexpr size_t lds_bytes(int ring, bool cx = false) { return (size_t)8 * ring * SLAB + (cx ? 2 : 1) * (size_t)NTM * 128; }
};

template <int NGX, int NTK, int NT, bool CX = false>
__global__ void __launch_bounds__(512, 2)
    k_brotdots_mfma(double* __restrict__ V, int64_t ldv, int cin, const double* __restrict__ M, int out0, int knew,
                    const double* __restrict__ Zb, int64_t ldz, int s, int ring, double* __restrict__ partial, int pnb, int dbg,
                    const double* __restrict__ zeros) {
  using C = BlkRot<NGX, NTK, NT>;
  extern __shared__ __attribute__((aligned(16))) unsigned char lds_raw[];
  const int lane = threadIdx.x & 63;
  const int wave = __builtin_amdgcn_readfirstlane(threadIdx.x >> 6);
  unsigned char* myring = lds_raw + (size_t)wave * ring * C::SLAB;
  const uint32_t ring_lds = (uint32_t)(uintptr_t)myring;
  constexpr int CD = CX ? 2 : 1;
  double* mt = reinterpret_cast<double*>(lds_raw + (size_t)8 * ring * C::SLAB);
  for (int e = threadIdx.x; e < CD * C::NTM * 16; e += 512) {
    const int part = (e >> 4) / C::NTM;
    const int tile = (e >> 4) % C::NTM, kk = (e >> 2) & 3, jj = e & 3;
    const int g = tile / NTK, t = tile % NTK, c = 4 * g + kk, j = 4 * t + jj;
    double v = 0.0;
    if (c < cin && j < knew) v = j < out0 ? ((c == j && part == 0) ? 1.0 : 0.0) : M[(c + (int64_t)(j - out0) * cin) * CD + part];
    mt[e] = v;
  }
  __syncthreads();
  const int lin = lane * 8;
  const int gat = (lane & 3) * 128 + (4 * ((lane >> 2) & 3) + (lane >> 4)) * 8;
  const double jsign = (lane & 1) ? 1.0 : -1.0;
  const double psign = ((lane >> 4) & 1) ? -1.0 : 1.0;
  const double* mrd = mt + (lane >> 4) * 4 + (lane & 3);
  const double* mri = mrd + C::NTM * 16;
  constexpr int NA = CX ? 2 * C::NTILE : C::NTILE;
  double acc[NA];
#pragma unroll
  for (int e = 0; e < NA; ++e) acc[e] = 0.0;
  int64_t pb, pe;
  block_range(ldv / 2, blockIdx.x, gridDim.x, pb, pe);
  const int niter = (int)((pe - pb + 63) / 64);
  const bool nt = (dbg & 64) != 0;
  const int t_lo = out0 >> 2, t_hi = (knew - 1) >> 2;
  const int nst = (dbg & 1) ? 0 : (t_hi - t_lo + 1);
  auto issue = [&](int it, int sl) {
    const int64_t p = pb + (int64_t)it * 64 + wave * 8 + (lane & 7);
    const bool in = p < pe;
    const int cl = lane >> 3;
    const uint32_t slab_lds = ring_lds + (uint32_t)(sl * C::SLAB);
#pragma unroll
    for (int j = 0; j < C::NJ; ++j) {
      const int c = j < C::NJX ? 8 * j + cl : 8 * (j - C::NJX) + cl;
      const bool have = in && (j < C::NJX ? c < cin : c < s);
      const double* src = have ? (j < C::NJX ? V + (int64_t)c * ldv : Zb + (int64_t)c * ldz) + p * 2 : zeros;
      if (nt) glds16_nt(src, slab_lds + (uint32_t)j * 1024u);
      else glds16(src, slab_lds + (uint32_t)j * 1024u);
    }
  };
  const int row = 4 * ((lane >> 2) & 3) + (lane >> 4), cj = lane & 3;
  double* vst = V + (int64_t)cj * ldv + row;
  for (int it = 0; it < ring - 1; ++it) issue(it, it);
  int sl_cur = 0, sl_new = ring - 1;
  for (int it = 0; it < niter; ++it) {
    wait_vm((ring - 2) * C::NJ + (it < ring - 1 ? it : ring - 1) * nst);
    issue(it + ring - 1, sl_new);
    const unsigned char* slab = myring + (size_t)sl_cur * C::SLAB;
    sl_new = sl_cur;
    sl_cur = sl_cur + 1 == ring ? 0 : sl_cur + 1;
    const int64_t pack0 = pb + (int64_t)it * 64 + wave * 8;
    double x[NGX], d[NTK], z[NT], zp[CX ? NT : 1];
#pragma unroll
    for (int g = 0; g < NGX; ++g) x[g] = *reinterpret_cast<const double*>(slab + C::x_off(g) + lin);
#pragma unroll
    for (int u = 0; u < NT; ++u) z[u] = *reinterpret_cast<const double*>(slab + C::z_off(u) + gat);
    if constexpr (CX) {
#pragma unroll
      for (int u = 0; u < NT; ++u) zp[u] = psign * *reinterpret_cast<const double*>(slab + C::z_off(u) + (gat ^ 8));
    }
#pragma unroll
    for (int t = 0; t < NTK; ++t) d[t] = 0.0;
#pragma unroll
    for (int g = 0; g < NGX; ++g)
#pragma unroll
      for (int t = 0; t < NTK; ++t) d[t] = mfma4(x[g], mrd[(g * NTK + t) * 16], d[t]);
    if constexpr (CX) {
#pragma unroll
      for (int g = 0; g < NGX; ++g) {
        const double xj = jsign * *reinterpret_cast<const double*>(slab + C::x_off(g) + (lin ^ 8));
#pragma unroll
        for (int t = 0; t < NTK; ++t) d[t] = mfma4(xj, mri[(g * NTK + t) * 16], d[t]);
      }
    }
    if (nst) {
      const bool ok = pack0 + (row >> 1) < pe;
      double* dst = vst + pack0 * 2;
#pragma unroll
      for (int t = 0; t < NTK; ++t) {
        if (t >= t_lo && t <= t_hi) {
          const int j = 4 * t + cj;
          if (ok && j >= out0 && j < knew) gst8_nt(dst + (int64_t)(4 * t) * ldv, d[t]);
        }
      }
    }
#pragma unroll
    for (int u = 0; u < NT; ++u)
#pragma unroll
      for (int q = 0; q <= u; ++q) {
        acc[C::NTS + C::gt(q, u)] = mfma4(z[q], z[u], acc[C::NTS + C::gt(q, u)]);
        if constexpr (CX) acc[C::NTILE + C::NTS + C::gt(q, u)] = mfma4(z[q], zp[u], acc[C::NTILE + C::NTS + C::gt(q, u)]);
      }
#pragma unroll
    for (int t = 0; t < NTK; ++t)
#pragma unroll
      for (int u = 0; u < NT; ++u) {
        acc[t * NT + u] = mfma4(d[t], z[u], acc[t * NT + u]);
        if constexpr (CX) acc[C::NTILE + t * NT + u] = mfma4(d[t], zp[u], acc[C::NTILE + t * NT + u]);
      }
  }
  asm volatile("s_waitcnt vmcnt(0)" ::: "memory");
  blkm_finish<NTK, NT, CX>(acc, lds_raw, lane, wave, knew, s, partial, pnb);
}

}
```

arnoldimethod.jl_amd/csrc/ks_hip.hip:

```cpp
#include <hip/hip_runtime.h>
#include <rccl/rccl.h>

#include <signal.h>
#include <unistd.h>

#include <algorithm>
#include <chrono>
#include <cmath>
#include <cstdio>
#include <cstdlib>
#include <cstring>
#include <memory>
#include <stdexcept>
#include <string>
#include <thread>
#include <unordered_map>
#include <vector>

#include "../../include/kschur.h"
#include "ks_driver.hpp"
#include "ks_kernels.hpp"
#include "ks_spmv_march.hpp"
#include "ks_block_kernels.hpp"
#include "ks_block_launch.hpp"
// ... 497 lines not shown
    w->pstride = (int)round_up(maxdim + 2, 8);
    w->esz = dtype == KS_F64 ? 8 : 16;
    w->pnb = ctx->nblocks();
    w->nb = cap_blocks(w.get(), w->pnb, 2 * kBlock);
    const size_t esz = w->esz;
    const size_t vbytes = (size_t)w->ld * (maxdim + 1) * esz;
    w->vbytes = vbytes;
    {
      const int nt_env = env_int("KS_V_NT", -1);
      w->v_nt = nt_env >= 0 ? nt_env != 0 : vbytes > ((size_t)env_int("KS_V_NT_MB", 352) << 20);
    }
    if (env_int("KS_GUARD", 0)) {
      w->guard = (size_t)1 << 20;
      KS_HIP(hipMalloc(&w->Vbase, vbytes + 2 * w->guard));
      KS_HIP(hipMemsetAsync(w->Vbase, 0xA5, vbytes + 2 * w->guard, ctx->stream));
      w->V = static_cast<char*>(w->Vbase) + w->guard;
    } else {
      KS_HIP(hipMalloc(&w->V, vbytes));
      w->Vbase = w->V;
    }
    KS_HIP(hipMemsetAsync(w->V, 0, vbytes, ctx->stream));
    if (env_int("KS_ZS_EARLY", 0)) {
      const size_t zbytes = (size_t)w->ld * (dtype == KS_F64 ? ksd::kBlkSMax : 10) * esz;
      if (hipMalloc(&w->zscratch, zbytes) == hipSuccess) KS_HIP(hipMemsetAsync(w->zscratch, 0, zbytes, ctx->stream));
      else { (void)hipGetLastError(); w->zscratch = nullptr; }
    }
    const size_t hbytes = (size_t)(maxdim + 1) * maxdim * esz, qbytes = (size_t)maxdim * maxdim * esz;
    const size_t qxbytes = (size_t)(maxdim + 1) * (maxdim + 1) * esz;
    KS_HIP(hipHostMalloc(&w->H, hbytes));
    KS_HIP(hipHostMalloc(&w->Q, qbytes));
    w->hd_bytes = (size_t)round_up((int64_t)hbytes, 64);
    w->ldt = maxdim + 1;
    w->off_T = (size_t)round_up((int64_t)(w->hd_bytes + kCtlStateSlot + (size_t)(maxdim + 2) * 8), 64);
    w->off_g = w->off_T + (size_t)w->ldt * w->ldt * esz;
    w->ctl_bytes = (size_t)round_up((int64_t)(w->off_g + (size_t)w->ldt * esz), 64);
    const size_t ctl_bytes = w->ctl_bytes;
    static_assert(sizeof(DevState) <= kCtlStateSlot, "DevState must fit its slot of the control block");
    const unsigned coh = hipHostMallocCoherent | hipHostMallocMapped;
    KS_HIP(hipHostMalloc(&w->Hstage, ctl_bytes, coh));
    KS_HIP(hipHostMalloc(&w->Qstage, qxbytes, coh));
    KS_HIP(hipHostMalloc(&w->Hstage_early, ctl_bytes, coh));
    std::memset(w->Hstage_early, 0, ctl_bytes);
    KS_HIP(hipHostMalloc(reinterpret_cast<void**>(&w->mbox), 128, coh));
    std::memset(w->mbox, 0, 128);
    if (hipHostMalloc(reinterpret_cast<void**>(&w->gate_h), sizeof(ksd::RotGate), coh) == hipSuccess) {
      std::memset(w->gate_h, 0, sizeof(ksd::RotGate));
      if (hipHostGetDevicePointer(reinterpret_cast<void**>(&w->gate_hd), w->gate_h, 0) != hipSuccess ||
          hipHostGetDevicePointer(&w->Qstage_dev, w->Qstage, 0) != hipSuccess || hipMalloc(reinterpret_cast<void**>(&w->gate_d), sizeof(ksd::RotGate)) != hipSuccess) {
        (void)hipGetLastError();
        (void)hipHostFree(w->gate_h);
        w->gate_h = nullptr;
      } else {
        KS_HIP(hipMemset(w->gate_d, 0, sizeof(ksd::RotGate)));
      }
    } else {
      (void)hipGetLastError();
      w->gate_h = nullptr;
    }
    w->use_mbox = env_int("KS_MAILBOX", 1) != 0;
    if (hipHostGetDevicePointer(reinterpret_cast<void**>(&w->mbox_dev), w->mbox, 0) != hipSuccess ||
        hipHostGetDevicePointer(&w->Hstage_dev, w->Hstage, 0) != hipSuccess ||
        hipHostGetDevicePointer(&w->Hstage_early_dev, w->Hstage_early, 0) != hipSuccess) {
      (void)hipGetLastError();
      w->use_mbox = false;
    }
    std::memset(w->H, 0, hbytes);
    std::memset(w->Q, 0, qbytes);
    std::memset(w->Hstage, 0, ctl_bytes);
    KS_HIP(hipMalloc(&w->Hd, ctl_bytes));
    KS_HIP(hipMemsetAsync(w->Hd, 0, ctl_bytes, ctx->stream));
    w->st = reinterpret_cast<DevState*>(static_cast<char*>(w->Hd) + w->hd_bytes);
    w->st_h = reinterpret_cast<DevState*>(static_cast<char*>(w->Hstage) + w->hd_bytes);
    w->colscale = reinterpret_cast<double*>(static_cast<char*>(w->Hd) + w->hd_bytes + kCtlStateSlot);
    w->cs_h = reinterpret_cast<double*>(static_cast<char*>(w->Hstage) + w->hd_bytes + kCtlStateSlot);
    w->Td = static_cast<char*>(w->Hd) + w->off_T;
    w->gd = static_cast<char*>(w->Hd) + w->off_g;
    w->Th = static_cast<char*>(w->Hstage) + w->off_T;
    KS_HIP(hipMalloc(reinterpret_cast<void**>(&w->ctr), 64));
    KS_HIP(hipMemsetAsync(w->ctr, 0, 64, ctx->stream));
    w->passes = env_int("KS_PASSES", 2) == 3 ? 3 : 2;
    w->sstep = std::max(0, std::min(env_int("KS_SSTEP", 20), ksd::kBlkSMax));
    w->sstep_eff = w->sstep;
    w->rot_defer_on = env_int("KS_ROT_DEFER", 1) != 0;
    w->spec_on = env_int("KS_SPEC_CHAIN", 1) != 0;
    w->defl_on = env_int("KS_CHAIN_DEFLATE", 1) != 0;
    w->true_start_on = env_int("KS_TRUE_START", 0) != 0;
    if (const char* e = std::getenv("KS_SSTEP_GDEV_MAX")) w->blk_gdevmax = std::atof(e);
    if (const char* e = std::getenv("KS_SSTEP_PIVOT_MIN")) w->blk_pivmin = std::atof(e);
    if (const char* mr = std::getenv("KS_IMPLICIT_MAX_RATIO")) w->max_ratio = std::atof(mr);
    KS_HIP(hipMalloc(&w->Hscratch, (size_t)(maxdim + 2) * esz));
    KS_HIP(hipMalloc(&w->partial, (size_t)w->pnb * w->pstride * esz));
    KS_HIP(hipMalloc(&w->partial_s, (size_t)w->pnb * w->pstride * esz));
    KS_HIP(hipMalloc(&w->partial2, (size_t)std::max(w->pnb, ctx->num_cu * 8) * 8));
    KS_HIP(hipMalloc(&w->coef, (size_t)(w->pstride + 136) * esz));
    KS_HIP(hipMemsetAsync(w->coef, 0, (size_t)(w->pstride + 136) * esz, ctx->stream));
    KS_HIP(hipMalloc(&w->red, (size_t)(2 * w->pstride + 8) * esz));
    KS_HIP(hipMalloc(&w->scal, 64));
    KS_HIP(hipHostMalloc(&w->scal_h, 64));
    KS_HIP(hipHostMalloc(&w->coef_h, (size_t)w->pstride * esz));
    KS_HIP(hipMalloc(&w->Qd, std::max<size_t>(qxbytes, 16)));
    w->oop_mode = env_int("KS_OOP", 2);
    if (w->oop_mode == 1 || w->oop_mode == 2) {
      const size_t ob = (size_t)(w->oop_mode == 1 ? 2 : 1) * w->ld * esz;
      KS_HIP(hipMalloc(&w->oop, ob));
      KS_HIP(hipMemsetAsync(w->oop, 0, ob, ctx->stream));
    }
    w->hostscale.assign(maxdim + 2, 1.0);
    w->ones.assign(maxdim + 2, 1.0);
    w->colscale_dirty = true;
    reset_state(w.get());
    KS_HIP(hipStreamSynchronize(ctx->stream));
    if (dtype == KS_F64) tune_placement<double>(w.get(), vbytes);
    else tune_placement<cd>(w.get(), vbytes);
    reset_state(w.get());
    KS_HIP(hipStreamSynchronize(ctx->stream));
    *out = w.release();
  });
}

int ks_workspace_passes(const ks_workspace* ws, int* passes) {
  return guarded([&] {
    KS_REQUIRE(ws && passes, KS_ERR_ARGUMENT, "null argument");
    *passes = ws->passes;
  });
}

int ks_workspace_set_passes(ks_workspace* ws, int passes, double max_ratio) {
  return guarded([&] {
    KS_REQUIRE(ws, KS_ERR_ARGUMENT, "null workspace");
    KS_REQUIRE(passes == 2 || passes == 3, KS_ERR_ARGUMENT, "passes must be 2 (implicit second pass) or 3 (explicit)");
    ws->ctx->use();
    materialize(ws);
    ws->passes = passes;
    if (!std::isnan(max_ratio)) ws->max_ratio = max_ratio;
  });
}

int ks_workspace_set_sstep(ks_workspace* ws, int s, double pivot_min, double gram_dev_max) {
  return guarded([&] {
    KS_REQUIRE(ws, KS_ERR_ARGUMENT, "null workspace");
    KS_REQUIRE(s >= 0 && s <= ksd::kBlkSMax, KS_ERR_ARGUMENT, "block size must be 0 (off) .. 20");
    ws->ctx->use();
    materialize(ws);
    ws->sstep = s;
    ws->sstep_eff = s;
    ws->blk_clean = 0;
    if (!std::isnan(pivot_min)) ws->blk_pivmin = pivot_min;
    if (!std::isnan(gram_dev_max)) ws->blk_gdevmax = gram_dev_max;
  });
}

int ks_workspace_sstep_info(const ks_workspace* ws, int* s, int* blocks, int* abandoned, double* diag3) {
  return guarded([&] {
    KS_REQUIRE(ws, KS_ERR_ARGUMENT, "null workspace");
    if (s) *s = ws->sstep_eff;
    if (blocks) *blocks = ws->blk_count;
    if (abandoned) *abandoned = ws->blk_bails;
    if (diag3) { diag3[0] = ws->blk_diag[0]; diag3[1] = ws->blk_diag[1]; diag3[2] = ws->blk_diag[2]; }
  });
}

int ks_workspace_relation_info(const ks_workspace* ws, int* breaks, double* worst_leak) {
  return guarded([&] {
    KS_REQUIRE(ws, KS_ERR_ARGUMENT, "null workspace");
    if (breaks) *breaks = ws->relation_breaks;
    if (worst_leak) *worst_leak = ws->relation_leak;
  });
}

int ks_workspace_relation_probes(const ks_workspace* ws, int* probes) {
  return guarded([&] {
    KS_REQUIRE(ws && probes, KS_ERR_ARGUMENT, "null argument");
    *probes = ws->relation_probes;
  });
}

int ks_workspace_fused_rotations(const ks_workspace* ws, int* count, int* spec_adopted, int* spec_dropped) {
  return guarded([&] {
    KS_REQUIRE(ws, KS_ERR_ARGUMENT, "null workspace");
    if (count) *count = ws->rot_fused_count;
    if (spec_adopted) *spec_adopted = ws->spec_used;
    if (spec_dropped) *spec_dropped = ws->spec_wasted;
  });
}

int ks_workspace_split_rotations(const ks_workspace* ws, int* count) {
  return guarded([&] {
    KS_REQUIRE(ws && count, KS_ERR_ARGUMENT, "null argument");
    *count = ws->rot_split_count;
  });
}

int ks_workspace_deflated_blocks(const ks_workspace* ws, int* blocks, int* columns) {
  return guarded([&] {
    KS_REQUIRE(ws != nullptr, KS_ERR_ARGUMENT, "null argument");
    if (blocks) *blocks = ws->defl_blocks;
    if (columns) *columns = ws->defl_last;
  });
}

int ks_sstep_partition(int dtype, int k0, int count, int smax, int* out, int cap, int* nblocks) {
  return guarded([&] {
    KS_REQUIRE(nblocks && (out || cap == 0), KS_ERR_ARGUMENT, "null argument");
    KS_REQUIRE(dtype == KS_F64 || dtype == KS_C64, KS_ERR_ARGUMENT, "dtype");
    *nblocks = 0;
    if (k0 < 1 || count < 1 || smax < 1) return;
    const auto sizes = blk_partition(dtype, k0, count, std::min(smax, dtype == KS_F64 ? ksd::kBlkSMax : ksd::blk_smax<cd>()));
    *nblocks = (int)sizes.size();
    for (int i = 0; i < (int)sizes.size() && i < cap; ++i) out[i] = sizes[i];
  });
}

int ks_debug_blk_time(ks_workspace* ws, int k, int s, int which, int reps, int dbg, double* ms_per_launch, int* grid) {
  return guarded([&] {
    KS_REQUIRE(ws && ms_per_launch, KS_ERR_ARGUMENT, "null argument");
    KS_REQUIRE(blk_shape_ok(ws->dtype, k, s) && k + s <= ws->maxdim + 1, KS_ERR_ARGUMENT, "no block kernel for this shape");
    KS_REQUIRE(reps >= 1 && (which == 0 || which == 1), KS_ERR_ARGUMENT, "bad reps / which");
    ws->ctx->use();
    materialize(ws);
    prov_drop(ws);
    blk_ensure_buffers(ws);
    reset_state(ws);
    const bool zs = (dbg & 256) != 0, reroll = (dbg & 512) != 0;
    dbg &= 255;
    if (zs) {
      void* old = reroll ? ws->zscratch : nullptr;
      if (reroll) ws->zscratch = nullptr;
      bool ok = false;
      if (ws->dtype == KS_F64) ok = ensure_zscratch<double>(ws);
      else ok = ensure_zscratch<cd>(ws);
      if (old) { KS_HIP(hipStreamSynchronize(ws->ctx->stream)); (void)hipFree(old); }
      KS_REQUIRE(ok, KS_ERR_INTERNAL, "no room for the scratch columns");
    }
    const int saved = blk_dbg();
    blk_dbg() = dbg;
    hipEvent_t a, b;
    KS_HIP(hipEventCreate(&a));
    KS_HIP(hipEventCreate(&b));
    int nb = 0;
    auto run = [&](int n) {
      for (int i = 0; i < n; ++i) {
        if (ws->dtype == KS_F64) nb = launch_blk<double>(ws, which, k, s, zs);
        else nb = launch_blk<cd>(ws, which, k, s, zs);
      }
    };
    run(2);
    KS_HIP(hipEventRecord(a, ws->ctx->stream));
    run(reps);
    KS_HIP(hipEventRecord(b, ws->ctx->stream));
    KS_HIP(hipEventSynchronize(b));
    float ms = 0.f;
    KS_HIP(hipEventElapsedTime(&ms, a, b));
    (void)hipEventDestroy(a);
    (void)hipEventDestroy(b);
    blk_dbg() = saved;
    *ms_per_launch = (double)ms / reps;
    if (grid) *grid = nb;
  });
}

int ks_workspace_assert_arnoldi(ks_workspace* ws, int k) {
  return guarded([&] {
    KS_REQUIRE(ws, KS_ERR_ARGUMENT, "null workspace");
    KS_REQUIRE(k >= -1 && k <= ws->maxdim, KS_ERR_ARGUMENT, "k out of range");
    if (k < 0) prov_drop(ws);
    else { prov_set(ws, k); ws->prov_vouched = true; }
  });
}

int ks_workspace_provenance(const ks_workspace* ws, int* k) {
  return guarded([&] {
    KS_REQUIRE(ws && k, KS_ERR_ARGUMENT, "null argument");
    *k = ws->prov_k;
  });
}

int ks_workspace_placement(const ks_workspace* ws, int* candidates, double* best_ms, double* worst_ms, int* refused) {
  return guarded([&] {
    KS_REQUIRE(ws, KS_ERR_ARGUMENT, "null workspace");
    if (refused) *refused = ws->place_failed;
    if (candidates) *candidates = ws->place_candidates;
    if (best_ms) *best_ms = ws->place_best_ms;
    if (worst_ms) *worst_ms = ws->place_worst_ms;
  });
}

int ks_workspace_check_guard(ks_workspace* ws, int* intact) {
  return guarded([&] {
    KS_REQUIRE(ws && intact, KS_ERR_ARGUMENT, "null argument");
    *intact = 1;
    if (!ws->guard) return;
    ws->ctx->use();
    KS_HIP(hipStreamSynchronize(ws->ctx->stream));
    std::vector<unsigned char> h(ws->guard);
    for (int side = 0; side < 2; ++side) {
      const char* src = static_cast<const char*>(ws->Vbase) + (side ? ws->guard + ws->vbytes : 0);
      KS_HIP(hipMemcpy(h.data(), src, ws->guard, hipMemcpyDeviceToHost));
      for (unsigned char b : h)
        if (b != 0xA5) { *intact = 0; return; }
    }
  });
}

int ks_workspace_destroy(ks_workspace* ws) {
  return guarded([&] {
    if (!ws) return;
    (void)hipSetDevice(ws->ctx->device);
    gate_cancel(ws);
    (void)hipStreamSynchronize(ws->ctx->stream);
    delete ws;
  });
}

int ks_workspace_dims(const ks_workspace* ws, int64_t* n_local, int* maxdim, int* dtype, int64_t* ldv) {
  return guarded([&] {
    KS_REQUIRE(ws, KS_ERR_ARGUMENT, "null workspace");
    if (n_local) *n_local = ws->n;
    if (maxdim) *maxdim = ws->maxdim;
    if (dtype) *dtype = ws->dtype;
    if (ldv) *ldv = ws->ld;
  });
}

int ks_workspace_H(ks_workspace* ws, void** H, int* ldh) {
  return guarded([&] {
    KS_REQUIRE(ws && H, KS_ERR_ARGUMENT, "null argument");
// ... 610 lines not shown
```

arnoldimethod.jl_amd/csrc/ks_workspace.hpp:

```cpp
#pragma once
constexpr size_t kCtlStateSlot = 128;

struct ks_workspace {
  ks_ctx* ctx = nullptr;
  int dtype = KS_F64;
  int64_t n = 0, n_global = 0, row_begin = 0, ld = 0;
  int maxdim = 0;
  size_t esz = 8;
  void* V = nullptr;
  void* Vbase = nullptr;
  size_t guard = 0, vbytes = 0;
  bool v_nt = true;
  int place_failed = 0;
  int place_candidates = 0;
  double place_best_ms = 0.0, place_worst_ms = 0.0;
  void* H = nullptr;
  void* Q = nullptr;
  void* Hd = nullptr;
  void* Hstage = nullptr;
  void* Hscratch = nullptr;
  void* partial = nullptr;
  void* partial_s = nullptr;
  double* partial2 = nullptr;
  void* coef = nullptr;
  void* red = nullptr;
  double* scal = nullptr;
  double* scal_h = nullptr;
  void* coef_h = nullptr;
  size_t hd_bytes = 0;
  DevState* st = nullptr;
  DevState* st_h = nullptr;
  double* cs_h = nullptr;
  bool colscale_dirty = false;
  void* Hstage_early = nullptr;
  std::vector<char> Hbackup;
  uint64_t* mbox = nullptr;
  uint64_t* mbox_dev = nullptr;
  void* Hstage_dev = nullptr;
  void* Hstage_early_dev = nullptr;
  uint64_t mbox_seq = 0;
  bool use_mbox = true;
  int passes = 2;
  double max_ratio = 1e-3;
  int prov_k = -1;
  bool prov_vouched = false;
  int relation_probes = 0;
  bool rot_defer_on = true, spec_on = true;
  bool rot_pending = false, rot_fuse = false;
  bool rot_split = false;
  int rot_split_count = 0;
  int rot_cin = 0, rot_rr = 0, rot_out0 = 0;
  int rot_fused_count = 0;
  bool rot_defer_ok = false;
  void* zscratch = nullptr;
  bool defl_on = true;
  void* defl_part = nullptr;
  int defl_blocks = 0;
  int defl_last = 0;
  void* ztrue = nullptr;
  bool true_start_on = false;
  bool ztrue_valid = false;
  bool rot_true_start = false;
  bool spec_true = false;
  bool chain_true = false;
  int true_starts = 0;
  bool spec_valid = false;
  int spec_ne = 0;
  std::vector<char> spec_sh;
  int spec_backoff = 0;
  int spec_backoff_len = 1;
  int spec_adopt = 0;
  int spec_used = 0, spec_wasted = 0;
  int mindim_hint = 0;
  void* probe_dev = nullptr;
  void* probe_host = nullptr;
  void* probe_col = nullptr;
  void* watch_acc = nullptr;
  void* probe_host_dev = nullptr;
  int rp_every = 1, rp_count = 0, rp_done = 0;
  hipEvent_t qstage_evt = nullptr;
  bool qstage_marked = false;
  hipEvent_t rp_event = nullptr;
  bool rp_inflight = false;
  double rp_fro = 0.0, rp_last = 0.0, rp_seq = 0.0;
  double watch_tol = 0.0;
  std::vector<char> Hshadow;
  size_t off_T = 0, off_g = 0, ctl_bytes = 0;
  int ldt = 0;
  void* Td = nullptr;
  void* gd = nullptr;
  void* Th = nullptr;
  unsigned* ctr = nullptr;
  bool t_lazy = false;
  int ntrue = 0, t_hi = -1;
  void* Qd = nullptr;
  void* Qstage = nullptr;
  void* oop = nullptr;
  bool oop_full = false;
  int oop_mode = 2;
  void* tmp = nullptr;
  size_t tmp_bytes = 0;
  void* tmp2 = nullptr;
  size_t tmp2_bytes = 0;
  int pstride = 0;
  double* colscale = nullptr;
  std::vector<double> hostscale;
  std::vector<double> ones;
  int lazy_lo = 1 << 30, lazy_hi = -1;
  bool has_lazy() const { return lazy_hi >= lazy_lo || t_lazy; }
  int sstep = 0;
  double blk_pivmin = 1e-6;
  double blk_gdevmax = 1e-8;
  int sstep_eff = 0;
  int blk_clean = 0;
  std::vector<std::complex<double>> ritz;
  bool ritz_valid = false;
  std::vector<char> Hfull;
  bool hfull_valid = false;
  void* bpart = nullptr;
  void* bred = nullptr;
  void* bscr = nullptr;
  void* bzero = nullptr;
  bool blk_tail = false;
  double blk_diag[3] = {1.0, 1.0, 0.0};
  int blk_count = 0, blk_bails = 0;
  int relation_breaks = 0;
  double relation_leak = 0.0;
  double relation_tol = 1e-12;
  ksd::RotGate* gate_h = nullptr;
  ksd::RotGate* gate_hd = nullptr;
  ksd::RotGate* gate_d = nullptr;
  void* Qstage_dev = nullptr;
  bool gate_allowed = false;
  bool gate_armed = false;
  uint64_t gate_seq = 0;
  int gate_cin = 0, gate_rmax = 0;
  int nb = 0;
  int pnb = 0;
  uint64_t seed = 20240917ull;
  uint64_t rng_count = 0;

  void* col(int j) const { return static_cast<char*>(V) + (size_t)j * ld * esz; }
  void* ensure_tmp(size_t bytes) {
    if (bytes > tmp_bytes) {
      (void)hipFree(tmp);
      tmp = nullptr;
      KS_HIP(hipMalloc(&tmp, bytes));
      tmp_bytes = bytes;
    }
    return tmp;
  }
  void* ensure_tmp2(size_t bytes) {
    if (bytes > tmp2_bytes) {
      (void)hipFree(tmp2);
      tmp2 = nullptr;
      KS_HIP(hipMalloc(&tmp2, bytes));
      tmp2_bytes = bytes;
    }
    return tmp2;
  }
  ~ks_workspace() {
    if (gate_armed && gate_h) {
      __atomic_store_n(&gate_h->flag, (gate_seq << 1) | 1u, __ATOMIC_RELEASE);
      gate_armed = false;
      (void)hipStreamSynchronize(ctx->stream);
    }
    (void)hipFree(Vbase ? Vbase : V); (void)hipHostFree(H); (void)hipHostFree(Q); (void)hipFree(Hd); (void)hipHostFree(Hstage);
    (void)hipFree(Hscratch); (void)hipFree(partial); (void)hipFree(partial_s); (void)hipFree(partial2); (void)hipFree(coef); (void)hipFree(red);
    (void)hipFree(scal); (void)hipHostFree(scal_h); (void)hipHostFree(coef_h);
    if (zscratch) (void)hipFree(zscratch);
    if (ztrue) (void)hipFree(ztrue);
    if (defl_part) (void)hipFree(defl_part);
    if (rp_event) (void)hipEventDestroy(rp_event);
    if (qstage_evt) (void)hipEventDestroy(qstage_evt);
    if (probe_col) (void)hipFree(probe_col);
    if (watch_acc) (void)hipFree(watch_acc);
    if (probe_dev) (void)hipFree(probe_dev);
    if (probe_host) (void)hipHostFree(probe_host);
    (void)hipFree(Qd); (void)hipHostFree(Qstage); (void)hipFree(tmp); (void)hipFree(tmp2); (void)hipFree(oop);
    (void)hipHostFree(Hstage_early); (void)hipHostFree(mbox); (void)hipFree(ctr);
    (void)hipFree(bpart); (void)hipFree(bred); (void)hipFree(bscr); (void)hipFree(bzero);
    (void)hipHostFree(gate_h); (void)hipFree(gate_d);
  }
};

namespace {

inline void gate_cancel(ks_workspace* ws);

inline int cap_blocks(const ks_workspace* ws, int nb, int packs_per_iter) {
  const int64_t npacks = ws->ld * (int64_t)ws->esz / 16;
  const int64_t want = std::max<int64_t>(1, npacks / (2 * (int64_t)packs_per_iter));
  return (int)std::min<int64_t>(nb, want);
}

uint64_t next_seed(ks_workspace* ws) {
  const uint64_t s = ws->seed + ws->rng_count * 0x9E3779B97F4A7C15ull;
  ws->rng_count++;
  return s;
}

template <class K> int resident_blocks(ks_ctx* ctx, K kernel, size_t smem, int& cache) {
  if (cache < 0) {
    int occ = 0;
    KS_HIP(hipOccupancyMaxActiveBlocksPerMultiprocessor(&occ, kernel, kBlock, smem));
    cache = std::max(1, std::min(occ, ctx->bpc));
  }
  return ctx->num_cu * cache;
}

template <class D, int NC4> int dots_blocks(ks_workspace* ws) {
  static int cache = -1;
  return resident_blocks(ws->ctx, ksd::k_dots<D, NC4, 1, true>, 0, cache);
}

template <class D> int dots_blocks_for(ks_workspace* ws, int nc4) {
  switch (nc4) {
    case 1: return dots_blocks<D, 1>(ws);
    case 2: return dots_blocks<D, 2>(ws);
    case 3: return dots_blocks<D, 3>(ws);
    case 4: return dots_blocks<D, 4>(ws);
    case 5: return dots_blocks<D, 5>(ws);
    case 6: return dots_blocks<D, 6>(ws);
    case 7: return dots_blocks<D, 7>(ws);
    case 8: return dots_blocks<D, 8>(ws);
    case 9: return dots_blocks<D, 9>(ws);
    default: return dots_blocks<D, 10>(ws);
  }
}

template <class D, int NC4>
void launch_dots_nc(ks_workspace* ws, int nb, const D* V, int jc, const D* w, D* partial, int norm_slot, int pass,
                    const DevState* st) {
  if (ws->v_nt) ksd::k_dots<D, NC4, 1, true><<<nb, kBlock, 0, ws->ctx->stream>>>(V, ws->ld, jc, w, partial, ws->pnb, norm_slot, pass, st);
  else ksd::k_dots<D, NC4, 1, false><<<nb, kBlock, 0, ws->ctx->stream>>>(V, ws->ld, jc, w, partial, ws->pnb, norm_slot, pass, st);
}

template <class D> int launch_dots(ks_workspace* ws, int j, const D* w, int pass, const DevState* st, D* partial_out = nullptr) {
  const D* V = static_cast<const D*>(ws->V);
  D* partial = partial_out ? partial_out : static_cast<D*>(ws->partial);
  const int nb = cap_blocks(ws, dots_blocks_for<D>(ws, (std::min(j, 40) + 3) / 4), kBlock);
  for (int c0 = 0; c0 < j; c0 += 40) {
    const int jc = std::min(40, j - c0);
    const int norm_slot = (c0 + 40 >= j) ? (j - c0) : -1;
    const D* Vc = V + (size_t)c0 * ws->ld;
    D* pc = partial + (size_t)c0 * ws->pnb;
    switch ((jc + 3) / 4) {
      case 1: launch_dots_nc<D, 1>(ws, nb, Vc, jc, w, pc, norm_slot, pass, st); break;
      case 2: launch_dots_nc<D, 2>(ws, nb, Vc, jc, w, pc, norm_slot, pass, st); break;
      case 3: launch_dots_nc<D, 3>(ws, nb, Vc, jc, w, pc, norm_slot, pass, st); break;
      case 4: launch_dots_nc<D, 4>(ws, nb, Vc, jc, w, pc, norm_slot, pass, st); break;
      case 5: launch_dots_nc<D, 5>(ws, nb, Vc, jc, w, pc, norm_slot, pass, st); break;
      case 6: launch_dots_nc<D, 6>(ws, nb, Vc, jc, w, pc, norm_slot, pass, st); break;
// ... 64 lines not shown
      case 2: return launch_axpy_dots_nc<D, 2, 4, 8>(ws, j, w, defer, wdst);
      case 3: return launch_axpy_dots_nc<D, 3, 4, 8>(ws, j, w, defer, wdst);
      case 4: return launch_axpy_dots_nc<D, 4, 4, 8>(ws, j, w, defer, wdst);
      case 5: return launch_axpy_dots_nc<D, 5, 4, 8>(ws, j, w, defer, wdst);
      case 6: return launch_axpy_dots_nc<D, 6, 4, 8>(ws, j, w, defer, wdst);
      case 7: return launch_axpy_dots_nc<D, 7, 4, 8>(ws, j, w, defer, wdst);
      case 8: return launch_axpy_dots_nc<D, 8, 4, 8>(ws, j, w, defer, wdst);
      case 9: return launch_axpy_dots_nc<D, 9, 4, 8>(ws, j, w, defer, wdst);
      case 10: return launch_axpy_dots_nc<D, 10, 4, 8>(ws, j, w, defer, wdst);
      case 11: return launch_axpy_dots_nc<D, 11, 2, 8>(ws, j, w, defer, wdst);
      case 12: return launch_axpy_dots_nc<D, 12, 2, 8>(ws, j, w, defer, wdst);
      case 13: return launch_axpy_dots_nc<D, 13, 2, 8>(ws, j, w, defer, wdst);
      case 14: return launch_axpy_dots_nc<D, 14, 2, 8>(ws, j, w, defer, wdst);
      case 15: return launch_axpy_dots_nc<D, 15, 2, 8>(ws, j, w, defer, wdst);
      default: return launch_axpy_dots_nc<D, 16, 2, 8>(ws, j, w, defer, wdst);
    }
  }
  switch ((j + 3) / 4) {
    case 1: return launch_axpy_dots_nc<D, 1, 4, 24>(ws, j, w, defer, wdst);
    case 2: return launch_axpy_dots_nc<D, 2, 4, 24>(ws, j, w, defer, wdst);
    case 3: return launch_axpy_dots_nc<D, 3, 4, 24>(ws, j, w, defer, wdst);
    case 4: return launch_axpy_dots_nc<D, 4, 4, 24>(ws, j, w, defer, wdst);
    case 5: return launch_axpy_dots_nc<D, 5, 4, 24>(ws, j, w, defer, wdst);
    case 6: return launch_axpy_dots_nc<D, 6, 4, 24>(ws, j, w, defer, wdst);
    case 7: return launch_axpy_dots_nc<D, 7, 4, 24>(ws, j, w, defer, wdst);
    case 8: return launch_axpy_dots_nc<D, 8, 4, 24>(ws, j, w, defer, wdst);
    case 9: return launch_axpy_dots_nc<D, 9, 4, 24>(ws, j, w, defer, wdst);
    case 10: return launch_axpy_dots_nc<D, 10, 4, 24>(ws, j, w, defer, wdst);
    case 11: return launch_axpy_dots_nc<D, 11, 2, 48>(ws, j, w, defer, wdst);
    case 12: return launch_axpy_dots_nc<D, 12, 2, 48>(ws, j, w, defer, wdst);
    case 13: return launch_axpy_dots_nc<D, 13, 2, 48>(ws, j, w, defer, wdst);
    case 14: return launch_axpy_dots_nc<D, 14, 2, 48>(ws, j, w, defer, wdst);
    case 15: return launch_axpy_dots_nc<D, 15, 2, 48>(ws, j, w, defer, wdst);
    default: return launch_axpy_dots_nc<D, 16, 2, 48>(ws, j, w, defer, wdst);
  }
}

template <class D> void enqueue_orthogonalize(ks_workspace* ws, int j) {
  hipStream_t s = ws->ctx->stream;
  D* w = static_cast<D*>(ws->col(j));
  D* Hd = static_cast<D*>(ws->Hd);
  const int ldh = ws->maxdim + 1;
  D* Hcol = Hd + (size_t)(j - 1) * ldh;
  const D* V = static_cast<const D*>(ws->V);
  const double nb8 = (double)ws->n * sizeof(D);
  for (int pass = 1; pass <= 2; ++pass) {
    int nbd;
    {
      ProfScope ps(ws->ctx, KSP_DOTS, nb8 * (j + 1));
      nbd = launch_dots<D>(ws, j, w, pass, ws->st);
    }
    {
      ProfScope ps(ws->ctx, KSP_FIN, 0.0);
      launch_fin_dots<D>(ws, nbd, j, Hcol, pass, ws->st);
    }
    {
      ProfScope ps(ws->ctx, KSP_AXPY, nb8 * (j + 2));
      ksd::k_axpy<D><<<ws->nb, kBlock, 0, s>>>(V, ws->ld, j, w, static_cast<const D*>(ws->coef), ws->partial2, pass, ws->st);
    }
    {
      ProfScope ps(ws->ctx, KSP_FIN, 0.0);
      launch_fin_norm<D>(ws, ws->nb, j, Hcol + j, pass, ws->st);
    }
  }
  {
    ProfScope ps(ws->ctx, KSP_SCALE, nb8 * 2);
    ksd::k_scale<D><<<ws->nb, kBlock, 0, s>>>(w, ws->ld, 0.0, ws->st);
  }
  KS_HIP(hipGetLastError());
}

inline void reset_lazy(ks_workspace* ws) {
  ws->t_lazy = false;
  ws->t_hi = -1;
  ws->blk_tail = false;
  if (!(ws->lazy_hi >= ws->lazy_lo)) return;
  for (int c = ws->lazy_lo; c <= ws->lazy_hi; ++c) ws->hostscale[c] = 1.0;
  ws->colscale_dirty = true;
  ws->lazy_lo = 1 << 30;
  ws->lazy_hi = -1;
}
template <class D> void materialize_t(ks_workspace* ws);
inline void rot_flush(ks_workspace* ws);
inline void materialize(ks_workspace* ws) {
  gate_cancel(ws);
  rot_flush(ws);
  if (ws->t_lazy) {
    if (ws->dtype == KS_F64) materialize_t<double>(ws);
    else materialize_t<cd>(ws);
  }
  if (!(ws->lazy_hi >= ws->lazy_lo)) return;
  for (int c = ws->lazy_lo; c <= ws->lazy_hi; ++c)
    if (ws->hostscale[c] != 1.0) {
      if (ws->dtype == KS_F64) ksd::k_scale<double><<<ws->nb, kBlock, 0, ws->ctx->stream>>>(static_cast<double*>(ws->col(c)), ws->ld, ws->hostscale[c], nullptr);
      else ksd::k_scale<cd><<<ws->nb, kBlock, 0, ws->ctx->stream>>>(static_cast<cd*>(ws->col(c)), ws->ld, ws->hostscale[c], nullptr);
    }
  KS_HIP(hipGetLastError());
  reset_lazy(ws);
}

inline size_t control_end(const ks_workspace* ws, bool with_T) {
  return with_T ? ws->off_g : ws->hd_bytes + sizeof(DevState);
}
inline void publish_control(ks_workspace* ws, int from, void* image_dev, int slot, uint64_t seq, bool with_T = false) {
  const size_t off = from >= 1 ? (size_t)(from - 1) * (ws->maxdim + 1) * ws->esz : ws->hd_bytes;
  const int nwords = (int)((control_end(ws, with_T) - off) / 8);
  ksd::k_publish<<<1, kBlock, 0, ws->ctx->stream>>>(reinterpret_cast<const uint64_t*>(static_cast<const char*>(ws->Hd) + off),
                                                     reinterpret_cast<uint64_t*>(static_cast<char*>(image_dev) + off), nwords,
                                                     ws->mbox_dev + 8 * slot, seq);
  KS_HIP(hipGetLastError());
}
inline void mbox_wait(ks_workspace* ws, int slot, uint64_t seq) {
  const uint64_t* f = ws->mbox + 8 * slot;
  unsigned spins = 0;
  while (__atomic_load_n(f, __ATOMIC_ACQUIRE) != seq) {
#if defined(__x86_64__) || defined(__i386__)
    __builtin_ia32_pause();
#else
    std::this_thread::yield();
#endif
    if ((++spins & 0xFFFu) == 0) {
      const hipError_t q = hipStreamQuery(ws->ctx->stream);
      if (q == hipSuccess) {
        if (__atomic_load_n(f, __ATOMIC_ACQUIRE) == seq) break;
        throw KsError{KS_ERR_HIP, "the stream drained without publishing the control block"};
      }
      if (q != hipErrorNotReady) KS_HIP(q);
    }
  }
}

template <class D> void enqueue_steps_deferred(ks_workspace* ws, ks_operator* op, int from, int to, uint64_t early_seq = 0) {
  ks_ctx* cx = ws->ctx;
  hipStream_t s = cx->stream;
  const int ldh = ws->maxdim + 1;
  D* Hd = static_cast<D*>(ws->Hd);
  const D* V = static_cast<const D*>(ws->V);
  D* red = static_cast<D*>(ws->red);
  D* coef = static_cast<D*>(ws->coef);
  const D* part = static_cast<const D*>(ws->partial);
  double* redd = reinterpret_cast<double*>(ws->red);
  constexpr int dpe = (int)(sizeof(D) / 8);
  const double nb8 = (double)ws->n * sizeof(D);
  const bool dist = cx->distributed();
  static const int no_fold = env_int("KS_P2P_NO_FOLD", 0);
  const bool p2p = cx->p2p.attached && !no_fold;
  const ksd::P2pDev pd = cx->p2p.dev;
  D* S0 = (op && ws->oop) ? static_cast<D*>(ws->oop) : nullptr;
  D* S1 = (S0 && ws->oop_full && ws->oop_mode == 1) ? S0 + ws->ld : nullptr;
  for (int j = from; j <= to; ++j) {
    D* w = static_cast<D*>(ws->col(j));
    D* y = S0 ? S0 : w;
    D* w1 = S1 ? S1 : w;
    D* Hcol = Hd + (size_t)(j - 1) * ldh;
    D* Hsub_prev = (j >= 2) ? Hd + (size_t)(j - 2) * ldh + (j - 1) : Hcol;
    if (op) {
      op->in_scale = op->async_capable ? 1.0 : ws->hostscale[j - 1];
      op->apply(ws->col(j - 1), y, ws->st);
    }
    int nbd;
    {
      ProfScope ps(cx, KSP_DOTS, nb8 * (j + 1));
      nbd = launch_dots<D>(ws, j, y, 1, ws->st);
    }
    {
      ProfScope ps(cx, KSP_FIN, 0.0);
      if (!dist || p2p) {
        ksd::k_fin_dots_def<D><<<j + 1, kBlock, 0, s>>>(part, nbd, ws->pnb, ws->partial2, ws->nb, j, red, Hcol, Hsub_prev, coef, ws->colscale, p2p ? 3 : 0, ws->st, pd);
// ... 387 lines not shown
  ws->gate_cin = cin;
  ws->gate_rmax = cin;
  rotate_device<double>(ws, 0, cin, cin, 0, -1, true);
  KS_HIP(hipGetLastError());
  ws->gate_armed = true;
  return true;
}

inline void qstage_wait(ks_workspace* ws) {
  static const int evt_on = env_int("KS_QSTAGE_EVENT", 1);
  if (evt_on && ws->ctx->hc.allreduce == nullptr && ws->qstage_marked) {
    KS_HIP(hipEventSynchronize(ws->qstage_evt));
    return;
  }
  KS_HIP(hipStreamSynchronize(ws->ctx->stream));
}
inline void qstage_mark(ks_workspace* ws) {
  if (!ws->qstage_evt) KS_HIP(hipEventCreateWithFlags(&ws->qstage_evt, hipEventDisableTiming));
  KS_HIP(hipEventRecord(ws->qstage_evt, ws->ctx->stream));
  ws->qstage_marked = true;
}

template <class T> void rotate_tfold(ks_workspace* ws, int c0, int c, int r, const T* Qh, int ldq, int out0, int src, int dst) {
  using D = typename DevT<T>::type;
  ws->ctx->use();
  rot_flush(ws);
  const bool gated = ws->gate_armed;
  if (!gated) qstage_wait(ws);
  const int rr = r + (src >= 0 ? 1 : 0);
  const int cin = std::max(c0 + c, src + 1);
  KS_REQUIRE(cin <= ws->maxdim + 1 && rr <= ws->maxdim + 1, KS_ERR_INTERNAL, "T-folded rotation out of range");
  T* qs = static_cast<T*>(ws->Qstage);
  const bool tl = ws->t_lazy;
  const int tlo = ws->ntrue, thi = ws->t_hi;
  const T* Th = static_cast<const T*>(ws->Th);
  const size_t ldt = (size_t)ws->ldt;
  std::fill(qs, qs + (size_t)cin * rr, T(0));
  for (int jj = 0; jj < r; ++jj) {
    T* __restrict__ out = qs + (size_t)jj * cin;
    for (int i = c0; i < c0 + c; ++i) {
      const T q = Qh[(i - c0) + (size_t)jj * ldq];
      if (tl && i >= tlo && i <= thi) {
        const T* __restrict__ tc = Th + (size_t)i * ldt;
        for (int k = 0; k <= i; ++k) out[k] += tc[k] * q;
      } else {
        out[i] += q;
      }
    }
  }
  if (src >= 0) {
    T* __restrict__ out = qs + (size_t)r * cin;
    if (tl && src >= tlo && src <= thi) {
      const T* __restrict__ tc = Th + (size_t)src * ldt;
      for (int k = 0; k <= src; ++k) out[k] = tc[k];
    } else {
      out[src] = T(1);
    }
  }
  const bool extra_elsewhere = src >= 0 && dst != out0 + r;
  {
    const bool true_start_on = ws->true_start_on;
    const bool start_stored = ws->blk_diag[2] <= 1e-12;
    const bool start_true = !start_stored && true_start_on && cin <= 40 && ws->blk_diag[2] <= ws->blk_gdevmax;
    const bool start_ok = start_stored || start_true;
    static const int defer_dbg = env_int("KS_DEFER_DEBUG", 0);
    if (defer_dbg)
      std::fprintf(stderr, "[defer] on %d ok %d src %d extra %d cin %d sstep_eff %d blk_tail %d tl %d thi %d gdev %.2e\n", (int)ws->rot_defer_on, (int)ws->rot_defer_ok,
                   src, (int)extra_elsewhere, cin, ws->sstep_eff, (int)ws->blk_tail, (int)tl, thi, ws->blk_diag[2]);
    if (ws->rot_defer_on && ws->rot_defer_ok && src == ws->maxdim && !extra_elsewhere && cin == ws->maxdim + 1 && ws->sstep_eff >= 8 && ws->blk_tail && tl && thi == ws->maxdim &&
        start_ok && ws->defl_last == 0) {
      gate_cancel(ws);
      KS_HIP(hipMemcpyAsync(ws->Qd, qs, (size_t)cin * rr * sizeof(T), hipMemcpyHostToDevice, ws->ctx->stream));
      qstage_mark(ws);
      ws->rot_pending = true;
      ws->rot_true_start = start_true;
      ws->rot_cin = cin; ws->rot_rr = rr; ws->rot_out0 = out0;
      ws->t_lazy = true;
      ws->ntrue = out0 + rr;
      ws->t_hi = out0 + rr - 1;
      ws->blk_tail = false;
      return;
    }
  }
  if (gated) {
    if constexpr (sizeof(T) == 8) {
      if (cin == ws->gate_cin && rr <= ws->gate_rmax && __atomic_load_n(&ws->gate_h->timed_out, __ATOMIC_ACQUIRE) != ws->gate_seq) {
        ksd::RotGate* g = ws->gate_h;
        g->c = cin; g->r = rr; g->out0 = out0; g->extra_out = extra_elsewhere ? dst : -1; g->ldq = cin; g->nq = cin * rr; g->cancel = 0;
        __atomic_store_n(&g->flag, ws->gate_seq << 1, __ATOMIC_RELEASE);
        ws->gate_armed = false;
        bool took = true;
        const double t_ack = ks::now_s();
        for (;;) {
          const uint64_t a = __atomic_load_n(&g->taken, __ATOMIC_ACQUIRE);
          if ((a >> 1) == ws->gate_seq) { took = (a & 1u) == 0; break; }
          if (ks::now_s() - t_ack > 2e-3) break;
        }
        if (took) {
          ws->t_lazy = false;
          ws->t_hi = -1;
          ws->blk_tail = false;
          return;
        }
      }
    }
    gate_cancel(ws);
    KS_HIP(hipStreamSynchronize(ws->ctx->stream));
  }
  KS_HIP(hipMemcpyAsync(ws->Qd, qs, (size_t)cin * rr * sizeof(T), hipMemcpyHostToDevice, ws->ctx->stream));
  qstage_mark(ws);
  rotate_device<D>(ws, 0, cin, rr, out0, extra_elsewhere ? dst : -1);
  ws->t_lazy = false;
  ws->t_hi = -1;
  ws->blk_tail = false;
}

inline void spec_drop(ks_workspace* ws) {
  if (ws->spec_valid) { ws->spec_valid = false; ws->spec_wasted++; ws->spec_backoff = ws->spec_backoff_len; ws->spec_backoff_len = std::min(8, 2 * ws->spec_backoff_len); }
}
inline void rot_flush(ks_workspace* ws) {
  if (!ws->rot_pending) return;
  spec_drop(ws);
  ws->rot_pending = false;
  ws->rot_true_start = false;
  ws->ztrue_valid = false;
  ws->t_lazy = false;
  ws->t_hi = -1;
  if (ws->dtype == KS_F64) rotate_device<double>(ws, 0, ws->rot_cin, ws->rot_rr, ws->rot_out0, -1);
  else rotate_device<cd>(ws, 0, ws->rot_cin, ws->rot_rr, ws->rot_out0, -1);
}

template <class D> void materialize_t(ks_workspace* ws) {
  using T = typename HostT<D>::type;
  if (!ws->t_lazy) return;
  const int lo = ws->ntrue, hi = ws->t_hi;
  if (hi < lo) { ws->t_lazy = false; return; }
  const int c = hi - lo + 1;
  std::vector<T> I((size_t)c * c, T(0));
  for (int i = 0; i < c; ++i) I[i + (size_t)i * c] = T(1);
  rotate_tfold<T>(ws, lo, c, c, I.data(), c, lo, -1, -1);
}

template <class T> void rotate_lazy(ks_workspace* ws, int c0, int c, int r, const T* Qh, int ldq, bool update_device_factors = true) {
  using D = typename DevT<T>::type;
  if (c <= 0 || r <= 0) return;
  ws->ctx->use();
  gate_cancel(ws);
  if (ws->t_lazy) materialize(ws);
  KS_HIP(hipStreamSynchronize(ws->ctx->stream));
  if (ws->has_lazy() && ws->lazy_lo < c0) materialize(ws);
  T* qs = static_cast<T*>(ws->Qstage);
  for (int jj = 0; jj < r; ++jj)
    for (int ii = 0; ii < c; ++ii) qs[ii + (size_t)jj * c] = Qh[ii + (size_t)jj * ldq] * ws->hostscale[c0 + ii];
  KS_HIP(hipMemcpyAsync(ws->Qd, qs, (size_t)c * r * sizeof(T), hipMemcpyHostToDevice, ws->ctx->stream));
  qstage_mark(ws);
  rotate_device<D>(ws, c0, c, r);
  bool any = false;
  for (int ii = 0; ii < r; ++ii) {
    any = any || ws->hostscale[c0 + ii] != 1.0;
    ws->hostscale[c0 + ii] = 1.0;
  }
  if (any) ws->colscale_dirty = true;
  (void)update_device_factors;
}

template <class D> void col_copy_lazy(ks_workspace* ws, int dst, int src) {
  ws->ctx->use();
  if (ws->t_lazy) materialize(ws);
  const double f = ws->hostscale[src];
  if (dst == src) {
    if (f != 1.0) ksd::k_scale<D><<<ws->nb, kBlock, 0, ws->ctx->stream>>>(static_cast<D*>(ws->col(src)), ws->ld, f, nullptr);
  } else {
    ksd::k_copy<D><<<ws->nb, kBlock, 0, ws->ctx->stream>>>(static_cast<const D*>(ws->col(src)), static_cast<D*>(ws->col(dst)), ws->ld, f);
  }
  KS_HIP(hipGetLastError());
  if (ws->hostscale[dst] != 1.0 || (dst == src && f != 1.0)) {
    ws->hostscale[dst] = 1.0;
    ws->colscale_dirty = true;
  }
}
```

include/kschur.h:

```cpp
#ifndef KSCHUR_H
#define KSCHUR_H

#include <stddef.h>
#include <stdint.h>

#ifdef __cplusplus
extern "C" {
#endif

#define KS_VERSION_MAJOR 0
#define KS_VERSION_MINOR 1

enum {
  KS_OK = 0,
  KS_ERR_ARGUMENT = 1,
  KS_ERR_DIMENSION = 2,
  KS_ERR_HIP = 3,
  KS_ERR_RCCL = 4,
  KS_ERR_QR = 5,
  KS_ERR_INTERNAL = 6,
  KS_ERR_NO_DEVICE = 7,
  KS_ERR_OPERATOR = 8,
  KS_ERR_COMM = 9
};

enum { KS_F64 = 0, KS_C64 = 1 };
enum { KS_I32 = 0, KS_I64 = 1 };
enum { KS_CSR = 0, KS_CSC = 1 };
enum { KS_LM = 0, KS_LR = 1, KS_SR = 2, KS_LI = 3, KS_SI = 4 };

typedef struct ks_ctx ks_ctx;
typedef struct ks_operator ks_operator;
typedef struct ks_workspace ks_workspace;

const char* ks_last_error_string(void);
int ks_version(int* major, int* minor);

int ks_ctx_create(int device, ks_ctx** out);
int ks_comm_unique_id(void* out128);
int ks_ctx_create_dist(int device, int rank, int nranks, const void* unique_id128, ks_ctx** out);
int ks_ctx_create_p2p(int device, int rank, int nranks, ks_ctx** out);
int ks_ctx_p2p_handle(ks_ctx* ctx, void* out64);
int ks_ctx_p2p_attach(ks_ctx* ctx, const void* handles);
typedef int (*ks_host_allreduce_fn)(void* user, double* buf, int count);
typedef int (*ks_host_exchange_fn)(void* user, int npeers, const int32_t* peers, const void* const* sendbufs,
                                   const int64_t* send_bytes, void* const* recvbufs, const int64_t* recv_bytes);
int ks_ctx_create_hostcomm(int device, int rank, int nranks, ks_host_allreduce_fn allreduce,
                           ks_host_exchange_fn exchange, void* user, ks_ctx** out);
int ks_ctx_destroy(ks_ctx* ctx);
int ks_ctx_synchronize(ks_ctx* ctx);
int ks_ctx_rank(const ks_ctx* ctx, int* rank, int* nranks);
int ks_ctx_stream(ks_ctx* ctx, void** hip_stream);

int ks_operator_csr(ks_ctx* ctx, int64_t nrows_local, int64_t ncols, int64_t nnz,
                    const void* ptr, const void* idx, const void* val, int layout, int index_base,
                    int index_type, int dtype, ks_operator** out);
int ks_operator_csr_dist(ks_ctx* ctx, int64_t nrows_local, int64_t nghost, int64_t nnz,
                         const int64_t* rowptr, const int32_t* colidx, const void* val, int dtype,
                         int nneigh, const int32_t* neigh, const int64_t* send_ptr,
                         const int32_t* send_idx, const int64_t* recv_cnt, ks_operator** out);
#define KS_ROW_MAJOR 0
#define KS_COL_MAJOR 1
int ks_operator_dense(ks_ctx* ctx, int64_t n, const void* a, int64_t ld, int layout, int dtype,
                      ks_operator** out);
typedef int (*ks_host_apply_fn)(void* user, const void* x_host, void* y_host);
int ks_operator_host_callback(ks_ctx* ctx, int64_t n_local, int dtype, ks_host_apply_fn apply,
                              void* user, ks_operator** out);
typedef int (*ks_device_apply_fn)(void* user, const void* x_dev, void* y_dev, void* hip_stream);
int ks_operator_device_callback(ks_ctx* ctx, int64_t n_local, int dtype, ks_device_apply_fn apply,
                                void* user, ks_operator** out);
int ks_operator_lu(ks_ctx* ctx, int64_t n, int dtype, const int64_t* l_rowptr, const int32_t* l_colind, const void* l_val,
                   const int64_t* u_rowptr, const int32_t* u_colind, const void* u_val, const int32_t* perm_in,
                   const int32_t* perm_out, const double* scale, ks_operator** out);
int ks_operator_lu_info(const ks_operator* op, int64_t* nnz_l, int64_t* nnz_u, int64_t* levels_l, int64_t* levels_u);
int ks_operator_lu_layout(const ks_operator* op, int upper, int64_t* rows, int64_t* run_rows, int64_t* top_rows, int* ngroups);
int ks_operator_destroy(ks_operator* op);
int ks_operator_size(const ks_operator* op, int64_t* n_local, int64_t* nnz, int* dtype);
enum { KS_LAYOUT_CSR = 0, KS_LAYOUT_CSR_VI = 1, KS_LAYOUT_DVI = 2, KS_LAYOUT_SELL = 3, KS_LAYOUT_SELL_VI = 4, KS_LAYOUT_STENCIL = 5, KS_LAYOUT_CSR_CB = 6 };
int ks_operator_format(const ks_operator* op, double* bytes_per_nnz, int* ndict, int* layout);
int ks_operator_apply_raw(ks_operator* op, const void* x_dev, void* y_dev);

int ks_workspace_create(ks_ctx* ctx, int64_t n_local, int64_t n_global, int64_t row_begin,
                        int maxdim, int dtype, ks_workspace** out);
int ks_workspace_destroy(ks_workspace* ws);
int ks_workspace_placement(const ks_workspace* ws, int* candidates, double* best_ms, double* worst_ms, int* refused);
int ks_workspace_passes(const ks_workspace* ws, int* passes);
int ks_workspace_set_passes(ks_workspace* ws, int passes, double max_ratio);
int ks_workspace_set_sstep(ks_workspace* ws, int s, double pivot_min, double gram_dev_max);
int ks_workspace_sstep_info(const ks_workspace* ws, int* s, int* blocks, int* abandoned, double* diag3);
int ks_sstep_partition(int dtype, int k0, int count, int smax, int* out, int cap, int* nblocks);
int ks_workspace_relation_info(const ks_workspace* ws, int* breaks, double* worst_leak);
int ks_workspace_relation_probes(const ks_workspace* ws, int* probes);
int ks_workspace_fused_rotations(const ks_workspace* ws, int* count, int* spec_adopted, int* spec_dropped);
int ks_workspace_split_rotations(const ks_workspace* ws, int* count);
int ks_workspace_deflated_blocks(const ks_workspace* ws, int* blocks, int* columns);
int ks_debug_blk_time(ks_workspace* ws, int k, int s, int which, int reps, int dbg, double* ms_per_launch, int* grid);
int ks_workspace_assert_arnoldi(ks_workspace* ws, int k);
int ks_workspace_provenance(const ks_workspace* ws, int* k);
int ks_workspace_check_guard(ks_workspace* ws, int* intact);
int ks_workspace_dims(const ks_workspace* ws, int64_t* n_local, int* maxdim, int* dtype, int64_t* ldv);
int ks_workspace_H(ks_workspace* ws, void** H, int* ldh);
int ks_workspace_Q(ks_workspace* ws, void** Q, int* ldq);
int ks_workspace_col_ptr(ks_workspace* ws, int j, void** dev_ptr);
int ks_workspace_set_seed(ks_workspace* ws, uint64_t seed);

int ks_col_upload(ks_workspace* ws, int j, const void* host);
int ks_col_download(ks_workspace* ws, int j, void* host);
int ks_cols_download(ks_workspace* ws, int j0, int ncols, void* host, int64_t ldhost);
int ks_cols_upload(ks_workspace* ws, int j0, int ncols, const void* host, int64_t ldhost);
int ks_col_fill_uniform(ks_workspace* ws, int j, uint64_t seed);
int ks_col_norm(ks_workspace* ws, int j, double* out);
int ks_col_div(ks_workspace* ws, int j, double s);
int ks_col_copy(ks_workspace* ws, int dst, int src);
int ks_apply(ks_operator* A, ks_workspace* ws, int jsrc, int jdst);
int ks_gemv_t(ks_workspace* ws, int j, int jv, void* h_host);
int ks_gemv_n_sub(ks_workspace* ws, int j, int jv, const void* h_host);
int ks_rotate(ks_workspace* ws, int c0, int c, int r, const void* Q_host, int ldq);
int ks_basis_times(ks_workspace* ws, int c, int r, const void* Y_host, int ldy, int ydtype,
                   void* out_host, int64_t ldout);

int ks_orthogonalize(ks_workspace* ws, int j, int* ok);
int ks_reinitialize(ks_workspace* ws, int j, const void* v1_host, int* ok);
typedef struct ks_expand_stats {
  int32_t steps;
  int32_t reorth;
  int32_t breakdowns;
  int32_t explicit_steps;
} ks_expand_stats;
int ks_iterate_arnoldi(ks_operator* A, ks_workspace* ws, int from, int to, ks_expand_stats* stats);

typedef struct ks_params {
  int32_t nev;
  int32_t which;
  double tol;
  int32_t mindim;
  int32_t maxdim;
  int32_t restarts;
  int32_t start_from;
  int32_t initialize;
  int32_t reserved;
} ks_params;
typedef struct ks_history {
  int32_t mvproducts;
  int32_t nconverged;
  int32_t converged;
  int32_t nev;
  int32_t restarts;
  int32_t reorth;
  int32_t breakdowns;
  int32_t explicit_steps;
  double seconds_expand;
  double seconds_host;
  double seconds_rotate;
} ks_history;
int ks_params_default(int64_t n, ks_params* p);
int ks_partialschur(ks_operator* A, ks_workspace* ws, const ks_params* p, const void* v1_host,
                    double* eigenvalues_c64, ks_history* history);

int ks_restart(ks_workspace* ws, const ks_params* p, int active, int* k, int* nlock, int* purge,
               double* lams_c64, double* rs, int32_t* groups);

int ks_expand_restart(ks_operator* A, ks_workspace* ws, const ks_params* p, int active, int k_in, int* k, int* nlock,
                      int* purge, double* eigenvalues_c64, double* residuals, int32_t* groups, ks_expand_stats* stats,
                      double* seconds);

int ks_profile_enable(ks_ctx* ctx, int on);
int ks_profile_reset(ks_ctx* ctx);
int ks_profile_get(ks_ctx* ctx, int nclass, double* ms, double* bytes, int64_t* counts);

int ks_residual_norms(ks_operator* A, ks_workspace* ws, int ncols, double* resid, double* orth);
int ks_arnoldi_relation(ks_operator* A, ks_workspace* ws, int k, double* resid, double* orth);

int ks_host_schurfact(int dtype, void* H, int m, int n, int ldh, int start, int to, void* Q, int nq,
                      int ldq);
int ks_host_restart_step(int dtype, void* H, int ldh, void* Q, int ldq, int maxdim, int mindim,
                         int nev, int which, double tol, int active, int* k, int* nlock, int* purge,
// ... 20 lines not shown
```

Before: 4823.

## Fold last block's basis write into the next fused restart rotation

When the final s-step block fills the Krylov basis, the second pass now writes only the last column and leaves the rest of the block's columns in scratch. The following fused rotation kernel reconstructs those columns from the old scratch set and folds them into the rotation, so the basis block is never written and re-read. This needs a second double-buffered scratch column set and flush calls on every path that would otherwise read the unwritten columns. The risks are extra memory, a narrow set of shapes where the fold is legal, and correctness if a flush is missed.

```diff
diff --git a/arnoldimethod.jl_amd/_lib.py b/arnoldimethod.jl_amd/_lib.py
--- a/arnoldimethod.jl_amd/_lib.py
+++ b/arnoldimethod.jl_amd/_lib.py
@@ -99,6 +99,7 @@
     "ks_workspace_relation_probes": [vp, P(C.c_int)],
     "ks_workspace_fused_rotations": [vp, P(C.c_int), P(C.c_int), P(C.c_int)],
     "ks_workspace_split_rotations": [vp, P(C.c_int)],
+    "ks_workspace_block_folds": [vp, P(C.c_int), P(C.c_int)],
     "ks_workspace_deflated_blocks": [vp, P(C.c_int), P(C.c_int)],
     "ks_sstep_partition": [C.c_int, C.c_int, C.c_int, C.c_int, P(C.c_int), C.c_int, P(C.c_int)],
     "ks_workspace_assert_arnoldi": [vp, i32],
diff --git a/arnoldimethod.jl_amd/api.py b/arnoldimethod.jl_amd/api.py
--- a/arnoldimethod.jl_amd/api.py
+++ b/arnoldimethod.jl_amd/api.py
@@ -561,8 +561,10 @@
         check(_lib.load().ks_workspace_split_rotations(self._h, C.byref(sr)))
         db, dc = C.c_int(), C.c_int()
         check(_lib.load().ks_workspace_deflated_blocks(self._h, C.byref(db), C.byref(dc)))
+        fb, ff = C.c_int(), C.c_int()
+        check(_lib.load().ks_workspace_block_folds(self._h, C.byref(fb), C.byref(ff)))
         return dict(s=s.value, blocks=b.value, abandoned=a.value, pivot_stage1=d[0], pivot_stage2=d[1], gram_dev=d[2], fused_rotations=fr.value,
-                    split_rotations=sr.value, chains_adopted=sa.value, chains_dropped=sd.value, deflated_blocks=db.value, deflated_columns=dc.value)
+                    folded_blocks=fb.value, fold_flushes=ff.value, split_rotations=sr.value, chains_adopted=sa.value, chains_dropped=sd.value, deflated_blocks=db.value, deflated_columns=dc.value)
 
     @property
     def relation_info(self) -> dict:
diff --git a/arnoldimethod.jl_amd/csrc/ks_backend.hpp b/arnoldimethod.jl_amd/csrc/ks_backend.hpp
--- a/arnoldimethod.jl_amd/csrc/ks_backend.hpp
+++ b/arnoldimethod.jl_amd/csrc/ks_backend.hpp
@@ -27,6 +27,10 @@
       (void)hipStreamSynchronize(ws->ctx->stream);
       try { reset_lazy(ws); } catch (...) {}
       prov_drop(ws);
+      if (ws->rot_fold) ws->blk_unwritten = true;
+      ws->rot_fold = false;
+      try { blk_flush(ws); } catch (...) {}
+      ws->blk_unwritten = false;
       ws->rot_pending = ws->rot_fuse = ws->rot_split = false;
       ws->rot_true_start = ws->chain_true = ws->ztrue_valid = false;
       ws->spec_valid = false;
@@ -86,6 +90,11 @@
           ws->rot_true_start = false;
           ws->rot_fuse = true;
           ws->rot_split = !fused_ok;
+          bool fold_ok = false;
+          if constexpr (sizeof(D) == 8)
+            fold_ok = ws->blk_unwritten && fused_ok && ws->zscratch2 && ws->rot_cin == ws->fold_k + ws->fold_s && ks_blk_fold_ok_f64(ws->fold_k, ws->fold_s, j0, blk_sizes[0]);
+          if (fold_ok) { ws->rot_fold = true; ws->blk_unwritten = false; }
+          else blk_flush(ws);
           ws->chain_true = spec_fits ? ws->spec_true : need_true;
           ws->t_lazy = false;
           ws->t_hi = -1;
@@ -193,6 +202,7 @@
       const int bail = (tpath && !bpath) ? ws->st_h->bail : -1;
       const int bd = (bail >= 0 || blk_bail >= 0) ? -1 : ws->st_h->breakdown;
       const int last_done = blk_bail >= 0 ? blk_bail - 1 : (bail >= 0 ? bail - 1 : (bd >= 0 ? bd : jend));
+      if (last_done != jend || blk_bail >= 0 || bd >= 0) blk_flush(ws);
       if (bpath) {
         ws->blk_diag[0] = ws->st_h->blk_piv1;
         ws->blk_diag[1] = ws->st_h->blk_piv2;
@@ -314,7 +324,7 @@
     if (ne < 2) return;
     if (!ensure_zscratch<D>(ws)) return;
     if (from_true && !true_start_enqueue<D>(ws)) return;
-    char* zs = static_cast<char*>(ws->zscratch);
+    char* zs = static_cast<char*>(ws->zset(ws->znext()));
     op->shift_store_cacheable = true;
     for (int i = 0; i < ne; ++i) {
       op->in_scale = 1.0;
diff --git a/arnoldimethod.jl_amd/csrc/ks_block.hpp b/arnoldimethod.jl_amd/csrc/ks_block.hpp
--- a/arnoldimethod.jl_amd/csrc/ks_block.hpp
+++ b/arnoldimethod.jl_amd/csrc/ks_block.hpp
@@ -62,12 +62,15 @@
 }
 
 inline int& blk_dbg() { static int v = env_int("KS_BLK_DBG", 0); return v; }
-template <class D> int launch_blk(ks_workspace* ws, int which, int k, int s, bool zscratch = false) {
+constexpr int kP2LastOnly = 1, kP2Flush = 2;
+template <class D> int launch_blk(ks_workspace* ws, int which, int k, int s, const void* zsrc = nullptr, int mode = 0, const void* zold = nullptr) {
   auto* bs = static_cast<ksd::BlkScratch<D>*>(ws->bscr);
   BlkLaunchArgs a{};
   a.V = ws->V; a.ld = ws->ld; a.dtype = sizeof(D) == 8 ? 0 : 1; a.k = k; a.s = s;
-  if (zscratch) { a.zsrc = ws->zscratch; a.ldz = ws->ld; }
-  if (which == 2) { a.cin = ws->rot_cin; a.out0 = ws->rot_out0; a.rotm = ws->Qd; }
+  if (zsrc) { a.zsrc = zsrc; a.ldz = ws->ld; }
+  if (which >= 2) { a.cin = ws->rot_cin; a.out0 = ws->rot_out0; a.rotm = ws->Qd; }
+  if (which == 3) { a.zold = zold; a.ldzo = ws->ld; a.fold_k = ws->fold_k; a.fold_s = ws->fold_s; }
+  a.last_only = mode == kP2LastOnly; a.no_sums = mode == kP2Flush;
   a.partial = ws->bpart; a.pnb = ws->pnb; a.coefp = bs->coefp; a.r1inv = bs->r1inv; a.zeros = ws->bzero; a.st = ws->st;
   a.dbg = blk_dbg(); a.nt = ws->v_nt ? 1 : 0; a.num_cu = ws->ctx->num_cu; a.bpc = ws->ctx->bpc; a.stream = ws->ctx->stream;
   try {
@@ -91,11 +94,33 @@
   if (env_int("KS_ADDR_DEBUG", 0)) std::fprintf(stderr, "[addr] V %p zscratch %p ld %lld bytes/col %lld\n", ws->V, ws->zscratch, (long long)ws->ld, (long long)(ws->ld * sizeof(D)));
   return true;
 }
+inline bool ensure_zscratch2(ks_workspace* ws) {
+  if (ws->zscratch2) return true;
+  if (!ws->blk_fold_on || !ws->zscratch || ws->dtype != KS_F64) return false;
+  const size_t zbytes = (size_t)ws->ld * ksd::blk_smax<double>() * sizeof(double);
+  if (hipMalloc(&ws->zscratch2, zbytes) != hipSuccess) {
+    (void)hipGetLastError();
+    ws->zscratch2 = nullptr;
+    ws->blk_fold_on = false;
+    return false;
+  }
+  KS_HIP(hipMemsetAsync(ws->zscratch2, 0, zbytes, ws->ctx->stream));
+  return true;
+}
+
+void blk_flush(ks_workspace* ws) {
+  if (!ws->blk_unwritten) return;
+  ws->blk_unwritten = false;
+  ws->fold_flushes++;
+  ProfScope ps(ws->ctx, KSP_FUSED, (double)ws->n * sizeof(double) * (ws->fold_k + 2 * ws->fold_s));
+  launch_blk<double>(ws, 1, ws->fold_k, ws->fold_s, ws->zset(ws->zcur), kP2Flush);
+}
 
 template <class D> bool true_start_enqueue(ks_workspace* ws) {
   if (ws->ztrue_valid) return true;
   const int cin = ws->maxdim + 1;
   if (cin > 40) return false;
+  blk_flush(ws);
   if (!ws->ztrue) {
     if (hipMalloc(&ws->ztrue, (size_t)ws->ld * sizeof(D)) != hipSuccess) { (void)hipGetLastError(); ws->ztrue = nullptr; return false; }
     KS_HIP(hipMemsetAsync(ws->ztrue, 0, (size_t)ws->ld * sizeof(D), ws->ctx->stream));
@@ -135,10 +160,21 @@
     ws->rot_fuse = false;
     ws->rot_split = false;
     ws->chain_true = false;
+    const bool fold_in = fuse && ws->rot_fold;
+    ws->rot_fold = false;
     char* zs = nullptr;
+    const void* zold = nullptr;
     if (fuse) {
       KS_REQUIRE(ws->zscratch != nullptr, KS_ERR_INTERNAL, "fused rotation without scratch columns (the adoption allocates them)");
-      zs = static_cast<char*>(ws->zscratch);
+      KS_REQUIRE(!fold_in || (!split && ws->zscratch2 != nullptr), KS_ERR_INTERNAL, "folded rotation without its second set of scratch columns");
+      zold = ws->zset(ws->zcur);
+      ws->zcur = ws->znext();
+      zs = static_cast<char*>(ws->zset(ws->zcur));
+    }
+    bool fold_out = false;
+    if constexpr (sizeof(D) == 8) {
+      fold_out = fuse && ws->blk_fold_on && ndefl == 0 && k + s == ws->maxdim + 1 && ws->rot_defer_on && ws->sstep_eff >= 8 && ks_blk_fold_src_ok_f64(k, s) &&
+                 (blk_dbg() & ~4) == 0 && ensure_zscratch2(ws);
     }
     if (split) {
       rotate_device<D>(ws, 0, ws->rot_cin, ws->rot_rr, ws->rot_out0, -1);
@@ -193,18 +229,20 @@
     };
     if (fuse && !split) {
       ProfScope ps(cx, KSP_ROTATE, nb8 * (ws->rot_cin + s + ws->rot_rr));
-      nb1 = launch_blk<D>(ws, 2, k, s, true);
+      nb1 = launch_blk<D>(ws, fold_in ? 3 : 2, k, s, zs, 0, zold);
       ws->rot_fused_count++;
+      if (fold_in) ws->folded_blocks++;
     } else {
       ProfScope ps(cx, KSP_DOTS, nb8 * (k + s));
-      nb1 = launch_blk<D>(ws, 0, k, s, fuse);
+      nb1 = launch_blk<D>(ws, 0, k, s, zs);
     }
     fin(1, nb1);
     {
-      ProfScope ps(cx, KSP_FUSED, nb8 * (k + 2 * s));
-      nb2 = launch_blk<D>(ws, 1, k, s, fuse);
+      ProfScope ps(cx, KSP_FUSED, nb8 * (fold_out ? k + s + 1 : k + 2 * s));
+      nb2 = launch_blk<D>(ws, 1, k, s, zs, fold_out ? kP2LastOnly : 0);
     }
     fin(2, nb2);
+    if (fold_out) { ws->blk_unwritten = true; ws->fold_k = k; ws->fold_s = s; }
     k += s;
     first = 0;
   }
diff --git a/arnoldimethod.jl_amd/csrc/ks_block_inst.hip b/arnoldimethod.jl_amd/csrc/ks_block_inst.hip
--- a/arnoldimethod.jl_amd/csrc/ks_block_inst.hip
+++ b/arnoldimethod.jl_amd/csrc/ks_block_inst.hip
@@ -123,7 +123,7 @@
   if (ring < 2 || smem > 160 * 1024) throw std::runtime_error("block kernels: slab ring does not fit the LDS");
   constexpr int RV = CX ? 2 : 1;
   const int nb = cap(a, a.num_cu, 64, CX ? 16 : 8);
-  const int dbg = a.dbg | (a.nt ? 64 : 0);
+  const int dbg = a.dbg | (a.nt ? 64 : 0) | (a.no_sums ? ksd::kBlkNoSums : 0);
   double* Vr = static_cast<double*>(a.V);
   const int64_t ldr = a.ld * RV;
   if (which == 0) {
@@ -136,6 +136,21 @@
     const double* zb = a.zsrc ? static_cast<const double*>(a.zsrc) : Vr + (int64_t)a.k * ldr;
     kern<<<nb, 512, smem, a.stream>>>(Vr, ldr, a.k, zb, a.zsrc ? a.ldz * RV : ldr, a.s, ring, static_cast<double*>(a.partial), a.pnb,
                                      static_cast<const ksd::DevState*>(a.st), dbg, static_cast<const double*>(a.zeros));
+  } else if (a.last_only) {
+    if constexpr (!CX && NT == 5) {
+      auto kern = ksd::k_bupdate_mfma<NGS, NT, false, true>;
+      static bool attr = false;
+      if (!attr) {
+        hipcheck(hipFuncSetAttribute(reinterpret_cast<const void*>(kern), hipFuncAttributeMaxDynamicSharedMemorySize, 160 * 1024), "dynamic LDS size");
+        attr = true;
+      }
+      if (!a.zsrc) throw std::runtime_error("block kernels: a block is left unwritten only with its chain in scratch columns");
+      kern<<<nb, 512, smem, a.stream>>>(Vr, ldr, a.k, static_cast<const double*>(a.zsrc), a.ldz, a.s, ring, static_cast<const double*>(a.coefp), a.k,
+                                       static_cast<const double*>(a.r1inv), static_cast<double*>(a.partial), a.pnb,
+                                       static_cast<const ksd::DevState*>(a.st), dbg, static_cast<const double*>(a.zeros));
+    } else {
+      throw std::runtime_error("block kernels: no last-column form of the second pass for this shape");
+    }
   } else {
     auto kern = ksd::k_bupdate_mfma<NGS, NT, CX>;
     static bool attr = false;
@@ -180,6 +195,31 @@
   return nb;
 }
 #if KS_BLK_PART == 1
+inline bool fold_shape(int fold_k, int fold_s, int k, int s) {
+  const int cin = fold_k + fold_s;
+  return fold_k >= 1 && fold_k <= 24 && fold_s >= 1 && fold_s <= 20 && cin >= 41 && cin <= 44 && k >= 1 && k <= 24 && k <= cin && s >= 1 && s <= 20;
+}
+inline int go_rotfold(const BlkLaunchArgs& a) {
+  using C = ksd::BlkFold;
+  if (!a.zsrc || !a.rotm || !a.zold || a.cin != a.fold_k + a.fold_s || !fold_shape(a.fold_k, a.fold_s, a.k, a.s))
+    throw std::runtime_error("block kernels: no folded fused rotation for this shape");
+  int ring = mfma_ring_env();
+  while (ring > 2 && C::lds_bytes(ring) > 160 * 1024) --ring;
+  const size_t smem = C::lds_bytes(ring);
+  if (ring < 2 || smem > 160 * 1024) throw std::runtime_error("block kernels: slab ring of the folded rotation does not fit the LDS");
+  const int nb = cap(a, a.num_cu, 64, 8);
+  auto kern = ksd::k_brotfold_mfma<C>;
+  static bool attr = false;
+  if (!attr) {
+    hipcheck(hipFuncSetAttribute(reinterpret_cast<const void*>(kern), hipFuncAttributeMaxDynamicSharedMemorySize, 160 * 1024), "dynamic LDS size");
+    attr = true;
+  }
+  kern<<<nb, 512, smem, a.stream>>>(static_cast<double*>(a.V), a.ld, a.fold_k, static_cast<const double*>(a.zold), a.ldzo, a.fold_s,
+                                   static_cast<const double*>(a.coefp), static_cast<const double*>(a.r1inv), static_cast<const double*>(a.rotm),
+                                   a.out0, a.k, static_cast<const double*>(a.zsrc), a.ldz, a.s, ring, static_cast<double*>(a.partial), a.pnb,
+                                   a.dbg | (a.nt ? 64 : 0), static_cast<const double*>(a.zeros));
+  return nb;
+}
 #define KS_ROT_SHAPES(X) X(11, 6, 5) X(11, 7, 4) X(11, 7, 3) X(11, 8, 3) X(11, 8, 2) X(6, 3, 3) X(6, 4, 3) X(6, 4, 2)
 constexpr bool kRotCX = false;
 #else
@@ -306,7 +346,12 @@
   if (!pass2_mfma(k, s) || !((mfma_env() >> 6) & 1)) return false;
   return k >= 1 && cin >= k && rot_shape(cin, k, s, a, b, c);
 }
+bool ks_blk_fold_src_ok_f64(int k, int s) { return ((mfma_env() >> 6) & 1) && pass2_mfma(k, s) && ks_blk_mfma_nt_f64(k, s) == 5 && fold_shape(k, s, 1, 1); }
+bool ks_blk_fold_ok_f64(int fold_k, int fold_s, int k, int s) {
+  return ks_blk_fold_src_ok_f64(fold_k, fold_s) && pass2_mfma(k, s) && s > 5 && fold_shape(fold_k, fold_s, k, s);
+}
 int ks_blk_launch_part1(int which, const BlkLaunchArgs& a) {
+  if (which == 3) return go_rotfold(a);
   if (which == 2) return go_rot_by_shape(a);
   const bool wide = (a.s == 8 && a.k > 48) || (a.s == 10 && a.k > 32);
   switch (wide ? 0 : a.s) {
diff --git a/arnoldimethod.jl_amd/csrc/ks_block_launch.hpp b/arnoldimethod.jl_amd/csrc/ks_block_launch.hpp
--- a/arnoldimethod.jl_amd/csrc/ks_block_launch.hpp
+++ b/arnoldimethod.jl_amd/csrc/ks_block_launch.hpp
@@ -22,6 +22,10 @@
   int64_t ldz = 0;
   int cin = 0, out0 = 0;
   const void* rotm = nullptr;
+  bool last_only = false, no_sums = false;
+  const void* zold = nullptr;
+  int64_t ldzo = 0;
+  int fold_k = 0, fold_s = 0;
 };
 int ks_blk_launch_part0(int which, const BlkLaunchArgs& a);
 int ks_blk_launch_part1(int which, const BlkLaunchArgs& a);
@@ -33,6 +37,8 @@
 bool ks_blk_rot_ok_f64(int cin, int k, int s);
 bool ks_blk_rot_ok_c64(int cin, int k, int s);
 inline bool ks_blk_rot_ok(int dtype, int cin, int k, int s) { return dtype == 0 ? ks_blk_rot_ok_f64(cin, k, s) : ks_blk_rot_ok_c64(cin, k, s); }
+bool ks_blk_fold_ok_f64(int fold_k, int fold_s, int k, int s);
+bool ks_blk_fold_src_ok_f64(int k, int s);
 inline int ks_blk_launch(int which, const BlkLaunchArgs& a) {
   if (a.dtype != 0) return ks_blk_launch_part2(which, a);
   return a.s <= 4 ? ks_blk_launch_part0(which, a) : ks_blk_launch_part1(which, a);
diff --git a/arnoldimethod.jl_amd/csrc/ks_block_mfma.hpp b/arnoldimethod.jl_amd/csrc/ks_block_mfma.hpp
--- a/arnoldimethod.jl_amd/csrc/ks_block_mfma.hpp
+++ b/arnoldimethod.jl_amd/csrc/ks_block_mfma.hpp
@@ -3,6 +3,8 @@
 #include "ks_block_kernels.hpp"
 
 namespace ksd {
+
+constexpr int kBlkNoSums = 1 << 11;
 
 __device__ __forceinline__ double mfma4(double a, double b, double c) { return __builtin_amdgcn_mfma_f64_4x4x4f64(a, b, c, 0, 0, 0); }
 __device__ __forceinline__ void wait_vm(int n) {
@@ -17,6 +19,7 @@
 #undef KS_VMW
 }
 __device__ __forceinline__ void gst8_nt(double* p, double v) { asm volatile("global_store_dwordx2 %0, %1, off nt" :: "v"(p), "v"(v) : "memory"); }
+__device__ __forceinline__ void gst8(double* p, double v) { asm volatile("global_store_dwordx2 %0, %1, off" :: "v"(p), "v"(v) : "memory"); }
 
 template <int NGS, int NT> struct BlkMfma {
   static constexpr int NJS = (NGS + 1) / 2, NJZ = (NT + 1) / 2, NJ = NJS + NJZ;
@@ -143,7 +146,7 @@
   blkm_finish<NGS, NT, CX>(acc, lds_raw, lane, wave, k, s, partial, pnb);
 }
 
-template <int NGS, int NT, bool CX = false>
+template <int NGS, int NT, bool CX = false, bool LAST = false>
 __global__ void __launch_bounds__(512, 2)
     k_bupdate_mfma(double* __restrict__ V, int64_t ldv, int k, const double* __restrict__ Zb, int64_t ldz, int s, int ring,
                    const double* __restrict__ coefp, int ldc, const double* __restrict__ r1inv, double* __restrict__ partial, int pnb,
@@ -187,7 +190,8 @@
   block_range(ldv / 2, blockIdx.x, gridDim.x, pb, pe);
   const int niter = (int)((pe - pb + 63) / 64);
   const bool nt = (dbg & 64) != 0;
-  const int nst = (dbg & 1) ? 0 : (s + 3) / 4;
+  const int t_last = (s - 1) >> 2;
+  const int nst = (dbg & 1) ? 0 : (LAST ? 1 : (s + 3) / 4);
   auto issue = [&](int it, int sl) {
     blkm_issue<NGS, NT>(V, ldv, k, Zb, ldz, s, pb + (int64_t)it * 64 + wave * 8, pe, lane, ring_lds + (uint32_t)(sl * C::SLAB), zeros, nt);
   };
@@ -236,7 +240,12 @@
       double* dst = zst + pack0 * 2;
 #pragma unroll
       for (int t = 0; t < NT; ++t) {
-        if (4 * t < s) {
+        if constexpr (LAST) {
+          if (t == t_last && ok && 4 * t + cj == s - 1) {
+            if (dbg & 4) gst8(dst + (int64_t)(4 * t) * ldv, d[t]);
+            else gst8_nt(dst + (int64_t)(4 * t) * ldv, d[t]);
+          }
+        } else if (4 * t < s) {
           if (ok && 4 * t + cj < s) gst8_nt(dst + (int64_t)(4 * t) * ldv, d[t]);
         }
       }
@@ -264,6 +273,7 @@
       }
   }
   asm volatile("s_waitcnt vmcnt(0)" ::: "memory");
+  if (dbg & kBlkNoSums) return;
   blkm_finish<NGS, NT, CX>(acc, lds_raw, lane, wave, k, s, partial, pnb);
 }
 
@@ -395,4 +405,148 @@
   blkm_finish<NTK, NT, CX>(acc, lds_raw, lane, wave, knew, s, partial, pnb);
 }
 
-}
+struct BlkFold {
+  static constexpr int NGS = 6, NTQ = 5, NTK = 6, NT = 5;
+  static constexpr int NJ = 9, SLAB = NJ * 1024;
+  using P2 = BlkMfma<NGS, NTQ>;
+  static constexpr int NTM = (NGS + NTQ) * NTK;
+  static constexpr int NTS = NTK * NT, NTG = NT * (NT + 1) / 2, NTILE = NTS + NTG;
+  __host__ __device__ static constexpr int off(int region, int g) { return region * 3072 + (g / 2) * 1024 + (g % 2) * 512; }
+  __host__ __device__ static constexpr int gt(int a, int t) { return t * (t + 1) / 2 + a; }
+  static constexpr size_t lds_bytes(int ring) { return (size_t)8 * ring * SLAB + (size_t)(P2::NTILE + NTM) * 128; }
+};
+
+template <class C = BlkFold>
+__global__ void __launch_bounds__(512, 1)
+    k_brotfold_mfma(double* __restrict__ V, int64_t ldv, int kold, const double* __restrict__ Zo, int64_t ldzo, int so,
+                    const double* __restrict__ coefp, const double* __restrict__ r1inv, const double* __restrict__ M, int out0, int knew,
+                    const double* __restrict__ Zb, int64_t ldz, int s, int ring, double* __restrict__ partial, int pnb, int dbg,
+                    const double* __restrict__ zeros) {
+  extern __shared__ __attribute__((aligned(16))) unsigned char lds_raw[];
+  const int lane = threadIdx.x & 63;
+  const int wave = __builtin_amdgcn_readfirstlane(threadIdx.x >> 6);
+  unsigned char* myring = lds_raw + (size_t)wave * ring * C::SLAB;
+  const uint32_t ring_lds = (uint32_t)(uintptr_t)myring;
+  double* mq = reinterpret_cast<double*>(lds_raw + (size_t)8 * ring * C::SLAB);
+  double* mt = mq + C::P2::NTILE * 16;
+  const int cin = kold + so;
+  for (int e = threadIdx.x; e < C::P2::NTILE * 16; e += 512) {
+    const int tile = e >> 4, kk = (e >> 2) & 3, jj = e & 3;
+    double v = 0.0;
+    if (tile < C::P2::NTS) {
+      const int g = tile / C::NTQ, t = tile % C::NTQ, c = 4 * g + kk, i = 4 * t + jj;
+      if (c < kold && i < so) v = -coefp[c + (int64_t)i * kold];
+    } else {
+      int t = 0, rem = tile - C::P2::NTS;
+      while (rem > t) { rem -= t + 1; ++t; }
+      const int l = 4 * rem + kk, i = 4 * t + jj;
+      if (l <= i && i < so) v = r1inv[l + i * so];
+    }
+    mq[e] = v;
+  }
+  for (int e = threadIdx.x; e < C::NTM * 16; e += 512) {
+    const int tile = e >> 4, kk = (e >> 2) & 3, jj = e & 3;
+    const int g = tile / C::NTK, t = tile % C::NTK, j = 4 * t + jj;
+    int c = 4 * g + kk;
+    if (g < C::NGS) c = c < kold ? c : -1;
+    else c = (c - 4 * C::NGS) < so ? kold + (c - 4 * C::NGS) : -1;
+    double v = 0.0;
+    if (c >= 0 && j < knew) v = j < out0 ? (c == j ? 1.0 : 0.0) : M[c + (int64_t)(j - out0) * cin];
+    mt[e] = v;
+  }
+  __syncthreads();
+  const int lin = lane * 8;
+  const int gat = (lane & 3) * 128 + (4 * ((lane >> 2) & 3) + (lane >> 4)) * 8;
+  const int swp = 16 * (lane & 3) + (lane & 12) + (lane >> 4);
+  const double* mqd = mq + (lane >> 4) * 4 + (lane & 3);
+  const double* mrd = mt + (lane >> 4) * 4 + (lane & 3);
+  double acc[C::NTILE];
+#pragma unroll
+  for (int e = 0; e < C::NTILE; ++e) acc[e] = 0.0;
+  int64_t pb, pe;
+  block_range(ldv / 2, blockIdx.x, gridDim.x, pb, pe);
+  const int niter = (int)((pe - pb + 63) / 64);
+  const bool nt = (dbg & 64) != 0;
+  const int t_lo = out0 >> 2, t_hi = (knew - 1) >> 2;
+  const int nst = (dbg & 1) ? 0 : (t_hi - t_lo + 1);
+  auto issue = [&](int it, int sl) {
+    const int64_t p = pb + (int64_t)it * 64 + wave * 8 + (lane & 7);
+    const bool in = p < pe;
+    const int cl = lane >> 3;
+    const uint32_t slab_lds = ring_lds + (uint32_t)(sl * C::SLAB);
+#pragma unroll
+    for (int j = 0; j < C::NJ; ++j) {
+      const int c = 8 * (j % 3) + cl;
+      const double* src = zeros;
+      if (j < 3) { if (in && c < kold) src = V + (int64_t)c * ldv + p * 2; }
+      else if (j < 6) { if (in && c < so) src = Zo + (int64_t)c * ldzo + p * 2; }
+      else { if (in && c < s) src = Zb + (int64_t)c * ldz + p * 2; }
+      if (nt) glds16_nt(src, slab_lds + (uint32_t)j * 1024u);
+      else glds16(src, slab_lds + (uint32_t)j * 1024u);
+    }
+  };
+  const int row = 4 * ((lane >> 2) & 3) + (lane >> 4), cj = lane & 3;
+  double* vst = V + (int64_t)cj * ldv + row;
+  for (int it = 0; it < ring - 1; ++it) issue(it, it);
+  int sl_cur = 0, sl_new = ring - 1;
+  for (int it = 0; it < niter; ++it) {
+    wait_vm((ring - 2) * C::NJ + (it < ring - 1 ? it : ring - 1) * nst);
+    issue(it + ring - 1, sl_new);
+    const unsigned char* slab = myring + (size_t)sl_cur * C::SLAB;
+    sl_new = sl_cur;
+    sl_cur = sl_cur + 1 == ring ? 0 : sl_cur + 1;
+    const int64_t pack0 = pb + (int64_t)it * 64 + wave * 8;
+    double x[C::NGS], zo[C::NTQ], q[C::NTQ], d[C::NTK], z[C::NT];
+#pragma unroll
+    for (int g = 0; g < C::NGS; ++g) x[g] = *reinterpret_cast<const double*>(slab + C::off(0, g) + lin);
+#pragma unroll
+    for (int u = 0; u < C::NTQ; ++u) zo[u] = *reinterpret_cast<const double*>(slab + C::off(1, u) + lin);
+#pragma unroll
+    for (int u = 0; u < C::NT; ++u) z[u] = *reinterpret_cast<const double*>(slab + C::off(2, u) + gat);
+#pragma unroll
+    for (int t = 0; t < C::NTQ; ++t) q[t] = 0.0;
+#pragma unroll
+    for (int g = 0; g < C::NGS; ++g)
+#pragma unroll
+      for (int t = 0; t < C::NTQ; ++t) q[t] = mfma4(x[g], mqd[(g * C::NTQ + t) * 16], q[t]);
+#pragma unroll
+    for (int u = 0; u < C::NTQ; ++u)
+#pragma unroll
+      for (int t = u; t < C::NTQ; ++t) q[t] = mfma4(zo[u], mqd[(C::P2::NTS + C::gt(u, t)) * 16], q[t]);
+#pragma unroll
+    for (int t = 0; t < C::NTQ; ++t) q[t] = __shfl(q[t], swp, 64);
+#pragma unroll
+    for (int t = 0; t < C::NTK; ++t) d[t] = 0.0;
+#pragma unroll
+    for (int g = 0; g < C::NGS; ++g)
+#pragma unroll
+      for (int t = 0; t < C::NTK; ++t) d[t] = mfma4(x[g], mrd[(g * C::NTK + t) * 16], d[t]);
+#pragma unroll
+    for (int u = 0; u < C::NTQ; ++u)
+#pragma unroll
+      for (int t = 0; t < C::NTK; ++t) d[t] = mfma4(q[u], mrd[((C::NGS + u) * C::NTK + t) * 16], d[t]);
+    if (nst) {
+      const bool ok = pack0 + (row >> 1) < pe;
+      double* dst = vst + pack0 * 2;
+#pragma unroll
+      for (int t = 0; t < C::NTK; ++t) {
+        if (t >= t_lo && t <= t_hi) {
+          const int j = 4 * t + cj;
+          if (ok && j >= out0 && j < knew) gst8_nt(dst + (int64_t)(4 * t) * ldv, d[t]);
+        }
+      }
+    }
+#pragma unroll
+    for (int u = 0; u < C::NT; ++u)
+#pragma unroll
+      for (int qq = 0; qq <= u; ++qq) acc[C::NTS + C::gt(qq, u)] = mfma4(z[qq], z[u], acc[C::NTS + C::gt(qq, u)]);
+#pragma unroll
+    for (int t = 0; t < C::NTK; ++t)
+#pragma unroll
+      for (int u = 0; u < C::NT; ++u) acc[t * C::NT + u] = mfma4(d[t], z[u], acc[t * C::NT + u]);
+  }
+  asm volatile("s_waitcnt vmcnt(0)" ::: "memory");
+  blkm_finish<C::NTK, C::NT>(acc, lds_raw, lane, wave, knew, s, partial, pnb);
+}
+
+}
diff --git a/arnoldimethod.jl_amd/csrc/ks_hip.hip b/arnoldimethod.jl_amd/csrc/ks_hip.hip
--- a/arnoldimethod.jl_amd/csrc/ks_hip.hip
+++ b/arnoldimethod.jl_amd/csrc/ks_hip.hip
@@ -603,6 +603,7 @@
     w->sstep = std::max(0, std::min(env_int("KS_SSTEP", 20), ksd::kBlkSMax));
     w->sstep_eff = w->sstep;
     w->rot_defer_on = env_int("KS_ROT_DEFER", 1) != 0;
+    w->blk_fold_on = env_int("KS_BLK_FOLD", 1) != 0 && dtype == KS_F64;
     w->spec_on = env_int("KS_SPEC_CHAIN", 1) != 0;
     w->defl_on = env_int("KS_CHAIN_DEFLATE", 1) != 0;
     w->true_start_on = env_int("KS_TRUE_START", 0) != 0;
@@ -705,6 +706,14 @@
   });
 }
 
+int ks_workspace_block_folds(const ks_workspace* ws, int* folded_blocks, int* fold_flushes) {
+  return guarded([&] {
+    KS_REQUIRE(ws, KS_ERR_ARGUMENT, "null workspace");
+    if (folded_blocks) *folded_blocks = ws->folded_blocks;
+    if (fold_flushes) *fold_flushes = ws->fold_flushes;
+  });
+}
+
 int ks_workspace_split_rotations(const ks_workspace* ws, int* count) {
   return guarded([&] {
     KS_REQUIRE(ws && count, KS_ERR_ARGUMENT, "null argument");
@@ -736,13 +745,15 @@
   return guarded([&] {
     KS_REQUIRE(ws && ms_per_launch, KS_ERR_ARGUMENT, "null argument");
     KS_REQUIRE(blk_shape_ok(ws->dtype, k, s) && k + s <= ws->maxdim + 1, KS_ERR_ARGUMENT, "no block kernel for this shape");
-    KS_REQUIRE(reps >= 1 && (which == 0 || which == 1), KS_ERR_ARGUMENT, "bad reps / which");
+    KS_REQUIRE(reps >= 1 && which >= 0 && which <= 3, KS_ERR_ARGUMENT, "bad reps / which");
+    KS_REQUIRE(which < 2 || (ws->dtype == KS_F64 && ks_blk_rot_ok_f64(k + s, k, s)), KS_ERR_ARGUMENT, "no fused rotation for this shape");
+    KS_REQUIRE(which < 3 || ks_blk_fold_ok_f64(k, s, k, s), KS_ERR_ARGUMENT, "no folded rotation for this shape");
     ws->ctx->use();
     materialize(ws);
     prov_drop(ws);
     blk_ensure_buffers(ws);
     reset_state(ws);
-    const bool zs = (dbg & 256) != 0, reroll = (dbg & 512) != 0;
+    const bool zs = (dbg & 256) != 0 || which >= 2, reroll = (dbg & 512) != 0, last_only = (dbg & 1024) != 0 && which == 1;
     dbg &= 255;
     if (zs) {
       void* old = reroll ? ws->zscratch : nullptr;
@@ -753,6 +764,11 @@
       if (old) { KS_HIP(hipStreamSynchronize(ws->ctx->stream)); (void)hipFree(old); }
       KS_REQUIRE(ok, KS_ERR_INTERNAL, "no room for the scratch columns");
     }
+    if (which >= 2) {
+      ws->rot_cin = k + s; ws->rot_out0 = 0; ws->rot_rr = k;
+      ws->fold_k = k; ws->fold_s = s;
+      if (which == 3) KS_REQUIRE(ensure_zscratch2(ws), KS_ERR_INTERNAL, "no room for the second set of scratch columns");
+    }
     const int saved = blk_dbg();
     blk_dbg() = dbg;
     hipEvent_t a, b;
@@ -761,8 +777,9 @@
     int nb = 0;
     auto run = [&](int n) {
       for (int i = 0; i < n; ++i) {
-        if (ws->dtype == KS_F64) nb = launch_blk<double>(ws, which, k, s, zs);
-        else nb = launch_blk<cd>(ws, which, k, s, zs);
+        const void* zp = zs ? ws->zscratch : nullptr;
+        if (ws->dtype == KS_F64) nb = launch_blk<double>(ws, which, k, s, zp, last_only ? kP2LastOnly : 0, ws->zscratch2);
+        else nb = launch_blk<cd>(ws, which, k, s, zp);
       }
     };
     run(2);
diff --git a/arnoldimethod.jl_amd/csrc/ks_workspace.hpp b/arnoldimethod.jl_amd/csrc/ks_workspace.hpp
--- a/arnoldimethod.jl_amd/csrc/ks_workspace.hpp
+++ b/arnoldimethod.jl_amd/csrc/ks_workspace.hpp
@@ -53,6 +53,15 @@
   int rot_fused_count = 0;
   bool rot_defer_ok = false;
   void* zscratch = nullptr;
+  bool blk_fold_on = true;
+  void* zscratch2 = nullptr;
+  int zcur = 0;
+  bool blk_unwritten = false;
+  int fold_k = 0, fold_s = 0;
+  bool rot_fold = false;
+  int folded_blocks = 0, fold_flushes = 0;
+  void* zset(int i) const { return (i & 1) && zscratch2 ? zscratch2 : zscratch; }
+  int znext() const { return zscratch2 ? (zcur ^ 1) : 0; }
   bool defl_on = true;
   void* defl_part = nullptr;
   int defl_blocks = 0;
@@ -169,6 +178,7 @@
     (void)hipFree(Hscratch); (void)hipFree(partial); (void)hipFree(partial_s); (void)hipFree(partial2); (void)hipFree(coef); (void)hipFree(red);
     (void)hipFree(scal); (void)hipHostFree(scal_h); (void)hipHostFree(coef_h);
     if (zscratch) (void)hipFree(zscratch);
+    if (zscratch2) (void)hipFree(zscratch2);
     if (ztrue) (void)hipFree(ztrue);
     if (defl_part) (void)hipFree(defl_part);
     if (rp_event) (void)hipEventDestroy(rp_event);
@@ -399,8 +409,10 @@
 }
 template <class D> void materialize_t(ks_workspace* ws);
 inline void rot_flush(ks_workspace* ws);
+void blk_flush(ks_workspace* ws);
 inline void materialize(ks_workspace* ws) {
   gate_cancel(ws);
+  blk_flush(ws);
   rot_flush(ws);
   if (ws->t_lazy) {
     if (ws->dtype == KS_F64) materialize_t<double>(ws);
@@ -954,6 +966,7 @@
       return;
     }
   }
+  blk_flush(ws);
   if (gated) {
     if constexpr (sizeof(T) == 8) {
       if (cin == ws->gate_cin && rr <= ws->gate_rmax && __atomic_load_n(&ws->gate_h->timed_out, __ATOMIC_ACQUIRE) != ws->gate_seq) {
@@ -992,6 +1005,7 @@
 }
 inline void rot_flush(ks_workspace* ws) {
   if (!ws->rot_pending) return;
+  blk_flush(ws);
   spec_drop(ws);
   ws->rot_pending = false;
   ws->rot_true_start = false;
diff --git a/include/kschur.h b/include/kschur.h
--- a/include/kschur.h
+++ b/include/kschur.h
@@ -92,6 +92,7 @@
 int ks_workspace_relation_info(const ks_workspace* ws, int* breaks, double* worst_leak);
 int ks_workspace_relation_probes(const ks_workspace* ws, int* probes);
 int ks_workspace_fused_rotations(const ks_workspace* ws, int* count, int* spec_adopted, int* spec_dropped);
+int ks_workspace_block_folds(const ks_workspace* ws, int* folded_blocks, int* fold_flushes);
 int ks_workspace_split_rotations(const ks_workspace* ws, int* count);
 int ks_workspace_deflated_blocks(const ks_workspace* ws, int* blocks, int* columns);
 int ks_debug_blk_time(ks_workspace* ws, int k, int s, int which, int reps, int dbg, double* ms_per_launch, int* grid);
```

Result: no change. 4858, median of 6 (+0.7%).
